# forsaken628/katib

Hardware: AMD Instinct MI355X
Metric: darts_cifar10_search_wall_clock_s (lower is better)
Workload: dtype fp32; 1 GPU; model=darts-cnn-cifar10 supernet (b5: C=4, L=2, N=3, stem x1, 6 primitives + none), global_batch=128, per_gpu_batch=128, parallelism=dp1, epochs=2, steps_per_epoch=196, ops=hip, hip_graph=True, sync_bn=False, hessian=concurrent

## Files before the change

### katib_amd/csrc/hip/darts_bind.cpp

```cpp
#include <torch/extension.h>
#include <c10/hip/HIPStream.h>

#include "darts_ops.h"
#include "darts_plane_layout.h"

using namespace katib_hip;
using at::Tensor;
using OptT = c10::optional<Tensor>;

namespace {

hipStream_t cur_stream() { return c10::hip::getCurrentHIPStream().stream(); }

void check_f32(const Tensor& t, const char* name) {
  TORCH_CHECK(t.is_cuda(), name, " must be a GPU tensor");
  TORCH_CHECK(t.scalar_type() == at::kFloat, name, " must be float32");
  TORCH_CHECK(t.is_contiguous(), name, " must be contiguous");
}

constexpr at::ScalarType kZType = kZbf16 ? at::kBFloat16 : at::kFloat;

void check_z(const Tensor& t, const char* name) {
  TORCH_CHECK(t.is_cuda(), name, " must be a GPU tensor");
  TORCH_CHECK(t.scalar_type() == kZType, name, " must be ", kZbf16 ? "bfloat16" : "float32",
              " (the per-op intermediates' storage type of this build)");
  TORCH_CHECK(t.is_contiguous(), name, " must be contiguous");
}

zt* zptr(const Tensor& t) { return reinterpret_cast<zt*>(t.data_ptr()); }

template <typename T>
T* ptr_or_null(const OptT& t) {
  return t.has_value() && t->defined() ? t->data_ptr<T>() : nullptr;
}

BNRef make_bn(const py::tuple& b, int C) {
  BNRef r{};
  TORCH_CHECK(b.size() == 8, "bn tuple has 8 fields");
  OptT sums = b[0].cast<OptT>(), rm = b[1].cast<OptT>(), rv = b[2].cast<OptT>();
  r.rep = b[6].cast<int>();
  r.rstride = b[7].cast<int>();
  TORCH_CHECK(r.rep >= 1 && r.rep <= kRep && r.rstride >= 2 * C, "bn replica layout");
  if (sums.has_value() && sums->defined()) {
    TORCH_CHECK(sums->scalar_type() == at::kDouble && sums->is_contiguous() &&
                    sums->numel() >= (int64_t)(r.rep - 1) * r.rstride + 2 * C,
                "bn sums must be f64 with rep x rstride doubles");
  }
  r.sums = ptr_or_null<double>(sums);
  r.rmean = ptr_or_null<float>(rm);
  r.rvar = ptr_or_null<float>(rv);
  r.inv_count = b[3].cast<float>();
  r.eval = b[4].cast<bool>() ? 1 : 0;
  r.eps = b[5].cast<float>();
  r.C = C;
  TORCH_CHECK(r.eval ? (r.rmean && r.rvar) : (r.sums != nullptr), "bn reference lacks its statistics");
  return r;
}

int64_t storage_doubles_after(const Tensor& t) {
  return (int64_t)(t.storage().nbytes() / sizeof(double)) - t.storage_offset();
}

int64_t gs_numel(const py::tuple& t) {
  return t[1].cast<Tensor>().numel();
}

GradSrc make_gs(const py::tuple& t, int C) {
  GradSrc g{};
  TORCH_CHECK(t.size() == 9, "grad-source tuple has 9 fields");
  Tensor gt = t[0].cast<Tensor>(), zt = t[1].cast<Tensor>();
  check_f32(gt, "g");
  check_z(zt, "z");
  g.g = gt.data_ptr<float>();
  g.z = zptr(zt);
  OptT s1 = t[2].cast<OptT>(), s2 = t[3].cast<OptT>();
  g.S1 = ptr_or_null<double>(s1);
  g.S2 = ptr_or_null<double>(s2);
  g.bn = make_bn(t[4].cast<py::tuple>(), C);
  g.eval = g.bn.eval;
  TORCH_CHECK(g.eval || (g.S1 && g.S2), "training-mode BN backward needs S1/S2 reductions");
  OptT w = t[5].cast<OptT>();
  g.w = ptr_or_null<float>(w);
  g.widx = t[6].cast<int>();
  g.rep = t[7].cast<int>();
  g.rstride = t[8].cast<int>();
  TORCH_CHECK(g.rep >= 1 && g.rep <= kRep, "replicas");
  if (!g.eval) {
    for (int k = 2; k <= 3; ++k) {
      Tensor sv = *t[k].cast<OptT>();
      TORCH_CHECK(sv.scalar_type() == at::kDouble &&
                      storage_doubles_after(sv) >= (int64_t)(g.rep - 1) * g.rstride + C,
                  "S1/S2 replicas exceed their buffer");
    }
  }
  return g;
}

struct CtrRing {
  unsigned* base = nullptr;
  int size = 0;
  int cursor = 0;
};
CtrRing g_ring[64];
bool g_selffold = false;

void set_selffold(bool on) { g_selffold = on; }

int cur_device() {
  int d = 0;
  TORCH_CHECK(hipGetDevice(&d) == hipSuccess, "hipGetDevice");
  return d;
}

void set_fold_counters(Tensor t) {
  TORCH_CHECK(t.is_cuda() && t.scalar_type() == at::kInt && t.is_contiguous() && t.numel() >= 4 * kFoldCtrSlot,
              "fold counters: contiguous int32 GPU tensor of >= 4 launch slots");
  const int d = t.get_device();
  TORCH_CHECK(d >= 0 && d < 64, "device index");
  g_ring[d] = CtrRing{reinterpret_cast<unsigned*>(t.data_ptr<int>()), (int)(t.numel() / kFoldCtrSlot), 0};
}

bool selffold_ready() { return g_selffold && g_ring[cur_device()].base != nullptr; }

void tail_begin(FoldTail& t) {
  t.nseg = 0;
  t.ctr = nullptr;
  if (!g_selffold) return;
  CtrRing& r = g_ring[cur_device()];
  if (!r.base) return;
  t.ctr = r.base + (size_t)r.cursor * kFoldCtrSlot;
  r.cursor = (r.cursor + 1) % r.size;
}

void tail_add(FoldTail& t, double* p, int n, int rs) {
  if (!t.ctr || !p) return;
  for (int s = 0; s < t.nseg; ++s)
    if (t.p[s] == p) {
      t.n[s] = std::max(t.n[s], n);
      return;
    }
  TORCH_CHECK(t.nseg < kTailSeg, "self-fold: too many reduction segments in one launch");
  t.p[t.nseg] = p;
  t.n[t.nseg] = n;
  t.rs[t.nseg] = rs;
  ++t.nseg;
}

void tail_close(FoldTail& t) {
  if (t.nseg == 0) t.ctr = nullptr;
}

int pick_chunk(int C, int per_channel_floats, int fixed_floats) {
  const int budget = 16384 - fixed_floats;
  int ch = C;
  while (ch > 1 && ch * per_channel_floats > budget) ch = (ch + 1) / 2;
  return std::max(ch, 1);
}

template <typename Bt>
void check_batch(const std::vector<py::tuple>& calls) {
  TORCH_CHECK(!calls.empty() && (int)calls.size() <= Bt::kCap, "batch of 1..", Bt::kCap, " edges");
}

#define SAME_SHAPE(b, fld) TORCH_CHECK(b.e[i].fld == b.e[0].fld, "edges in a batch must share " #fld)

static bool fill_dwpw(const py::tuple& t, DwPwFwdArgs& a, int64_t K, int64_t dil, int64_t S, int64_t pad, int nentries,
                      bool use_mfma) {
  Tensor x = t[0].cast<Tensor>(), dw = t[1].cast<Tensor>(), pw = t[2].cast<Tensor>();
  auto inbn = t[3].cast<c10::optional<py::tuple>>();
  Tensor d = t[4].cast<Tensor>(), z = t[5].cast<Tensor>();
  OptT stats = t[6].cast<OptT>();
  const bool has_inbn = t[3].cast<c10::optional<py::tuple>>().has_value();
  if (has_inbn) check_z(x, "x (previous stage z)");
  else check_f32(x, "x");
  check_f32(dw, "dw"); check_f32(pw, "pw"); check_z(d, "d"); check_z(z, "z");
  TORCH_CHECK(x.dim() == 4, "x must be NCHW");
  TORCH_CHECK((K == 3 || K == 5) && (dil == 1 || dil == 2) && (S == 1 || S == 2), "K in {3,5}, dil, S in {1,2}");
  const int N = x.size(0), C = x.size(1), H = x.size(2), W = x.size(3);
  const int Ho = z.size(2), Wo = z.size(3);
  TORCH_CHECK(dw.numel() == C * K * K && pw.numel() == C * C, "weight shapes");
  TORCH_CHECK(z.size(0) == N && z.size(1) == C && d.sizes() == z.sizes(), "output shapes");
  TORCH_CHECK(C == 4 || C == 8 || C == 16 || (64 % Wo == 0 && Ho % (64 / Wo) == 0),
              "tile constraint: 64 % Wo == 0 and Ho % (64/Wo) == 0");
  TORCH_CHECK(C <= kMaxC, "C too large");
  TORCH_CHECK(Ho == (H + 2 * pad - dil * (K - 1) - 1) / S + 1, "output height mismatch");
  a.x = x.data_ptr(); a.dw = dw.data_ptr<float>(); a.pw = pw.data_ptr<float>();
  a.d = zptr(d); a.z = zptr(z); a.stats = ptr_or_null<double>(stats);
  if (a.stats) TORCH_CHECK(stats->scalar_type() == at::kDouble && stats->numel() >= kRep * 2 * C, "stats f64 [kRep][2C]");
  a.N = N; a.C = C; a.H = H; a.W = W; a.Ho = Ho; a.Wo = Wo; a.pad = pad;
  const int TR = 64 / Wo;
  const int IR = (TR - 1) * S + (K - 1) * dil + 1, IW = (Wo - 1) * S + (K - 1) * dil + 1;
  a.chunk = pick_chunk(C, IR * IW, C * 64 + 4 * C);
  if (C == 4 || C == 8 || C == 16) {
    int nb = std::max(1, std::min(Ho / 4, 2048 / std::max(N * nentries, 1)));
    auto band_bytes = [&](int b) {
      const int BR = (Ho + b - 1) / b;
      return (size_t)C * ((BR - 1) * S + (K - 1) * dil + 1) * plane_pitch(W + 2 * pad, S) * sizeof(float);
    };
    while (band_bytes(nb) > 65536 && nb < Ho) ++nb;
    a.chunk = nb;
  }
  a.use_mfma = (use_mfma && C % 16 == 0) ? 1 : 0;
  const bool prebn = inbn.has_value();
  if (prebn) a.inbn = make_bn(*inbn, C);
  a.variant = (((K == 5) * 4 + (dil == 2) * 2 + (S == 2)) * 4) + (prebn ? 2 : 0);
  return prebn;
}

void dwpw_fwd(std::vector<py::tuple> calls, int64_t K, int64_t dil, int64_t S, int64_t pad, bool use_mfma) {
  check_batch<DwPwFwdBatch>(calls);
  DwPwFwdBatch bt{};
  bt.n = calls.size();
  bool prebn = false;
  for (int i = 0; i < bt.n; ++i) {
    const bool pb = fill_dwpw(calls[i], bt.e[i], K, dil, S, pad, bt.n, use_mfma);
    if (i == 0) prebn = pb;
    TORCH_CHECK(pb == prebn, "edges in a batch must agree on the input BN");
    SAME_SHAPE(bt, N); SAME_SHAPE(bt, C); SAME_SHAPE(bt, H); SAME_SHAPE(bt, W);
  }
  tail_begin(bt.tail);
  for (int i = 0; i < bt.n; ++i) tail_add(bt.tail, bt.e[i].stats, 2 * bt.e[i].C, 2 * bt.e[i].C);
  tail_close(bt.tail);
  launch_dwpw_fwd(bt, K, dil, S, prebn, cur_stream());
}

static void fill_dwpw_multi(const std::vector<py::tuple>& calls, DwPwMultiBatch& bt, int64_t* kk, int64_t* dd,
                            int64_t* ss, int64_t* pp, bool* pre) {
  TORCH_CHECK(!calls.empty() && (int)calls.size() <= DwPwMultiBatch::kCap, "1..", DwPwMultiBatch::kCap, " entries");
  bt.n = calls.size();
  for (int i = 0; i < bt.n; ++i) {
    const py::tuple& t = calls[i];
    TORCH_CHECK(t.size() == 11, "dwpw_fwd_multi entry: (x, dw, pw, inbn, d, z, stats, K, dil, S, pad)");
    kk[i] = t[7].cast<int64_t>(); dd[i] = t[8].cast<int64_t>(); ss[i] = t[9].cast<int64_t>(); pp[i] = t[10].cast<int64_t>();
    pre[i] = fill_dwpw(t, bt.e[i], kk[i], dd[i], ss[i], pp[i], bt.n, true);
    SAME_SHAPE(bt, N); SAME_SHAPE(bt, C); SAME_SHAPE(bt, Ho); SAME_SHAPE(bt, Wo);
  }
  tail_begin(bt.tail);
  for (int i = 0; i < bt.n; ++i) tail_add(bt.tail, bt.e[i].stats, 2 * bt.e[i].C, 2 * bt.e[i].C);
  tail_close(bt.tail);
}

void dwpw_fwd_multi(std::vector<py::tuple> calls) {
  DwPwMultiBatch bt{};
  int64_t kk[DwPwMultiBatch::kCap], dd[DwPwMultiBatch::kCap], ss[DwPwMultiBatch::kCap], pp[DwPwMultiBatch::kCap];
  bool pre[DwPwMultiBatch::kCap];
  fill_dwpw_multi(calls, bt, kk, dd, ss, pp, pre);
  if (launch_dwpw_multi(bt, cur_stream())) return;
  for (int i = 0; i < bt.n; ++i) {
    DwPwFwdBatch one{};
    one.n = 1;
    one.tail = bt.tail;
    fill_dwpw(calls[i], one.e[0], kk[i], dd[i], ss[i], pp[i], 1, true);
    launch_dwpw_fwd(one, kk[i], dd[i], ss[i], pre[i], cur_stream());
  }
}

void pw_fwd(std::vector<py::tuple> calls, int64_t S) {
  check_batch<PwFwdBatch>(calls);
  PwFwdBatch bt{};
  bt.n = calls.size();
  for (int i = 0; i < bt.n; ++i) {
    const py::tuple& t = calls[i];
    Tensor x = t[0].cast<Tensor>(), pw = t[1].cast<Tensor>(), z = t[2].cast<Tensor>();
    OptT stats = t[3].cast<OptT>();
    const int co_off = t[4].cast<int>(), off = t[5].cast<int>();
    check_f32(x, "x"); check_f32(pw, "pw"); check_z(z, "z");
    const bool nm = x.dim() == 5;
    const int xnodes = nm ? x.size(0) : 1;
    const int N = nm ? x.size(1) : x.size(0), Cin = nm ? x.size(0) * x.size(2) : x.size(1);
    const int H = x.size(nm ? 3 : 2), W = x.size(nm ? 4 : 3);
    const int Cout = pw.size(0), Ho = z.size(2), Wo = z.size(3);
    TORCH_CHECK(pw.size(1) == Cin && co_off + Cout <= z.size(1) && z.size(0) == N, "pw shapes");
    TORCH_CHECK((Ho * Wo) % 64 == 0, "Ho*Wo must be a multiple of 64");
    TORCH_CHECK(Cin <= kMaxC && Cout <= kMaxC, "channels");
    PwFwdArgs& a = bt.e[i];
    a.x = x.data_ptr<float>(); a.pw = pw.data_ptr<float>(); a.z = zptr(z);
    a.stats = ptr_or_null<double>(stats);
    if (a.stats)
      TORCH_CHECK(stats->scalar_type() == at::kDouble && stats->numel() >= kRep * 2 * z.size(1), "stats [kRep][2Ctot]");
    a.N = N; a.Cin = Cin; a.Cout = Cout; a.CoutTotal = z.size(1); a.co_off = co_off;
    a.H = H; a.W = W; a.Ho = Ho; a.Wo = Wo; a.S = S; a.off = off; a.relu = 1; a.xnodes = xnodes;
    SAME_SHAPE(bt, N); SAME_SHAPE(bt, Cin); SAME_SHAPE(bt, Cout); SAME_SHAPE(bt, Ho); SAME_SHAPE(bt, Wo);
  }
  tail_begin(bt.tail);
  for (int i = 0; i < bt.n; ++i) tail_add(bt.tail, bt.e[i].stats, 2 * bt.e[i].CoutTotal, 2 * bt.e[i].CoutTotal);
  tail_close(bt.tail);
  launch_pw_fwd(bt, cur_stream());
}

static void fill_pool_fwd(const std::vector<py::tuple>& calls, int64_t S_all, PoolFwdBatch& bt) {
  check_batch<PoolFwdBatch>(calls);
  bt.n = calls.size();
  for (int i = 0; i < bt.n; ++i) {
    const py::tuple& t = calls[i];
    const int64_t S = S_all > 0 ? S_all : t[6].cast<int64_t>();
    TORCH_CHECK(S == 1 || S == 2, "pool stride must be 1 or 2");
    bt.e[i].S = (int)S;
    Tensor x = t[0].cast<Tensor>(), zavg = t[1].cast<Tensor>(), zmax = t[2].cast<Tensor>();
    OptT sa = t[3].cast<OptT>(), sm = t[4].cast<OptT>(), amax = t[5].cast<OptT>();
    check_f32(x, "x"); check_z(zavg, "zavg"); check_z(zmax, "zmax");
    PoolFwdArgs& a = bt.e[i];
    if (amax.has_value() && amax->defined()) {
      TORCH_CHECK(amax->scalar_type() == at::kByte && amax->numel() == zmax.numel(), "amax must be uint8 like zmax");
      a.amax = amax->data_ptr<uint8_t>();
    }
    a.x = x.data_ptr<float>(); a.zavg = zptr(zavg); a.zmax = zptr(zmax);
    a.stats_avg = ptr_or_null<double>(sa); a.stats_max = ptr_or_null<double>(sm);
    if (a.stats_avg) TORCH_CHECK(sa->scalar_type() == at::kDouble && sa->numel() >= kRep * 2 * x.size(1), "stats");
    if (a.stats_max) TORCH_CHECK(sm->scalar_type() == at::kDouble && sm->numel() >= kRep * 2 * x.size(1), "stats");
    a.N = x.size(0); a.C = x.size(1); a.H = x.size(2); a.W = x.size(3); a.Ho = zavg.size(2); a.Wo = zavg.size(3);
    TORCH_CHECK(a.Ho == (a.H - 1) / S + 1 && zmax.sizes() == zavg.sizes(), "pool shapes");
    SAME_SHAPE(bt, N); SAME_SHAPE(bt, C);
    if (S_all > 0) { SAME_SHAPE(bt, H); SAME_SHAPE(bt, W); }
  }
  tail_begin(bt.tail);
  for (int i = 0; i < bt.n; ++i) {
    tail_add(bt.tail, bt.e[i].stats_avg, 2 * bt.e[i].C, 2 * bt.e[i].C);
    tail_add(bt.tail, bt.e[i].stats_max, 2 * bt.e[i].C, 2 * bt.e[i].C);
  }
  tail_close(bt.tail);
}

static void pool_fwd_impl(std::vector<py::tuple> calls, int64_t S_all) {
  PoolFwdBatch bt{};
  fill_pool_fwd(calls, S_all, bt);
  if (S_all > 0) launch_pool_fwd(bt, S_all, cur_stream());
  else launch_pool_fwd_multi(bt, cur_stream());
}

void pool_fwd(std::vector<py::tuple> calls, int64_t S) { pool_fwd_impl(calls, S); }
void pool_fwd_multi(std::vector<py::tuple> calls) { pool_fwd_impl(calls, -1); }

void dwpw_pool_fwd_multi(std::vector<py::tuple> dcalls, std::vector<py::tuple> pcalls) {
  DwPwMultiBatch bt{};
  int64_t kk[DwPwMultiBatch::kCap], dd[DwPwMultiBatch::kCap], ss[DwPwMultiBatch::kCap], pp[DwPwMultiBatch::kCap];
  bool pre[DwPwMultiBatch::kCap];
  fill_dwpw_multi(dcalls, bt, kk, dd, ss, pp, pre);
  PoolFwdBatch pb{};
  fill_pool_fwd(pcalls, -1, pb);
  if (launch_dwpw_pool_multi(bt, pb, cur_stream())) return;
  dwpw_fwd_multi(dcalls);
  launch_pool_fwd_multi(pb, cur_stream());
}

void combine_fwd(std::vector<py::tuple> calls, OptT gamma, OptT beta, Tensor out, double momentum,
                 bool update_running, bool accumulate) {
  check_f32(out, "out");
  check_batch<CombineFwdBatch>(calls);
  CombineFwdBatch bt{};
  bt.n = calls.size();
  const int C = out.size(1);
  TORCH_CHECK(C <= kMaxC, "C too large");
  TORCH_CHECK((int64_t)2 * bt.n * kMaxOps * C * 4 <= 65536, "combine LDS budget exceeded");
  for (int e = 0; e < bt.n; ++e) {
    const py::tuple& t = calls[e];
    auto zs = t[0].cast<std::vector<Tensor>>();
    auto bns = t[1].cast<std::vector<py::tuple>>();
    auto widx = t[2].cast<std::vector<int64_t>>();
    OptT w = t[3].cast<OptT>();
    const int id_idx = t[4].cast<int>();
    OptT xid = t[5].cast<OptT>();
    auto upd = t[6].cast<std::vector<py::tuple>>();
    TORCH_CHECK(zs.size() == bns.size() && zs.size() == widx.size() && (int)zs.size() <= kMaxOps, "ops");
    CombineFwdArgs& a = bt.e[e];
    a.N = out.size(0); a.C = C; a.HW = out.size(2) * out.size(3);
    a.nops = zs.size();
    for (size_t k = 0; k < zs.size(); ++k) {
      check_z(zs[k], "z");
      TORCH_CHECK(zs[k].sizes() == out.sizes(), "combine input shape");
      a.z[k] = zptr(zs[k]);
      a.bn[k] = make_bn(bns[k], C);
      a.widx[k] = widx[k];
    }
    TORCH_CHECK((int)upd.size() <= kMaxUpd, "too many update-only BN layers");
    a.nupd = upd.size();
    for (size_t k = 0; k < upd.size(); ++k) a.upd[k] = make_bn(upd[k], C);
    a.w = ptr_or_null<float>(w); a.id_idx = id_idx; a.xid = ptr_or_null<float>(xid);
    if (a.xid) {
      check_f32(*xid, "xid");
      TORCH_CHECK(xid->sizes() == out.sizes(), "identity shape");
    }
    a.gamma = ptr_or_null<float>(gamma); a.beta = ptr_or_null<float>(beta);
    a.out = out.data_ptr<float>(); a.momentum = momentum; a.update_running = update_running;
    a.accumulate = accumulate;
  }
  launch_combine_fwd(bt, cur_stream());
}

void combine_bwd_reduce(std::vector<py::tuple> calls) {
  check_batch<CombineBwdBatch>(calls);
  CombineBwdBatch bt{};
  bt.n = calls.size();
  for (int i = 0; i < bt.n; ++i) {
    const py::tuple& t = calls[i];
    Tensor dout = t[0].cast<Tensor>();
    auto zs = t[1].cast<std::vector<Tensor>>();
    auto bns = t[2].cast<std::vector<py::tuple>>();
    OptT xid = t[3].cast<OptT>();
    Tensor red = t[4].cast<Tensor>();
    auto widx = t[5].cast<std::vector<int64_t>>();
    const int id_idx = t[6].cast<int>();
    OptT gw = t[7].cast<OptT>();
    check_f32(dout, "dout");
    TORCH_CHECK(red.scalar_type() == at::kDouble, "red must be f64");
    CombineBwdArgs& a = bt.e[i];
    a.N = dout.size(0); a.C = dout.size(1); a.HW = dout.size(2) * dout.size(3);
    a.nops = zs.size();
    a.rstride = (a.nops + 1) * a.C + 1;
    TORCH_CHECK(a.nops <= kMaxOps && red.numel() >= (int64_t)kRep * a.rstride, "red size [kRep][(nops+1)C+1]");
    for (int k = 0; k < a.nops; ++k) {
      TORCH_CHECK(zs[k].sizes() == dout.sizes(), "z shape");
      check_z(zs[k], "z");
      a.z[k] = zptr(zs[k]);
      a.bn[k] = make_bn(bns[k], a.C);
    }
    a.dout = dout.data_ptr<float>(); a.xid = ptr_or_null<float>(xid); a.red = red.data_ptr<double>();
    a.gw = ptr_or_null<double>(gw); a.id_idx = id_idx;
    if (a.gw) {
      TORCH_CHECK(gw->scalar_type() == at::kDouble && gw->numel() % kRep == 0, "gw must be f64 [kRep][nw]");
      a.gwstride = gw->numel() / kRep;
      TORCH_CHECK((int)widx.size() == a.nops, "widx per op");
      for (int k = 0; k < a.nops; ++k) {
        TORCH_CHECK(widx[k] >= 0 && widx[k] < a.gwstride, "widx out of range");
        a.widx[k] = widx[k];
      }
      TORCH_CHECK(id_idx < a.gwstride, "id_idx out of range");
    }
    SAME_SHAPE(bt, N); SAME_SHAPE(bt, C); SAME_SHAPE(bt, HW);
  }
  tail_begin(bt.tail);
  for (int i = 0; i < bt.n; ++i) {
    tail_add(bt.tail, bt.e[i].red, bt.e[i].rstride, bt.e[i].rstride);
    tail_add(bt.tail, bt.e[i].gw, bt.e[i].gwstride, bt.e[i].gwstride);
  }
  tail_close(bt.tail);
  launch_combine_bwd_reduce(bt, cur_stream());
}

void check_grad_sink(const OptT& gW, int64_t numel, int64_t gstride) {
  if (!gW.has_value() || !gW->defined()) return;
  TORCH_CHECK(gW->scalar_type() == at::kFloat && gW->is_contiguous() && gW->numel() == numel, "gW shape");
  TORCH_CHECK(gstride == 0 || (gstride >= numel && (int64_t)(gW->storage().nbytes() / sizeof(float)) -
                                                           gW->storage_offset() >= (kRep - 1) * gstride + numel),
              "gW replicas exceed their buffer");
}

void pw_bwd(std::vector<py::tuple> calls, int64_t S, int64_t mode, bool need_dx) {
  check_batch<PwBwdBatch>(calls);
  PwBwdBatch bt{};
  bt.n = calls.size();
  for (int i = 0; i < bt.n; ++i) {
    const py::tuple& t = calls[i];
    py::tuple gs = t[0].cast<py::tuple>();
    Tensor pw = t[1].cast<Tensor>();
    OptT ain = t[2].cast<OptT>();
    Tensor x = t[3].cast<Tensor>();
    OptT dd = t[4].cast<OptT>(), gx = t[5].cast<OptT>(), gW = t[6].cast<OptT>();
    const int co_off = t[7].cast<int>(), off = t[8].cast<int>();
    const int64_t gstride = t[9].cast<int64_t>();
    const bool overwrite = t.size() > 10 && t[10].cast<bool>();
    check_f32(pw, "pw");
    if (mode != 0) check_f32(x, "x");
    PwBwdArgs& a = bt.e[i];
    a.overwrite = overwrite;
    TORCH_CHECK(!overwrite || (mode == 1 && S == 1 && off == 0), "gx overwrite needs the stride-1 full-coverage form");
    const int Cout = pw.size(0), Cin = pw.size(1);
    Tensor g = gs[0].cast<Tensor>();
    a.N = g.size(0); a.CoutTotal = g.size(1); a.Ho = g.size(2); a.Wo = g.size(3);
    a.gs = make_gs(gs, a.CoutTotal);
    a.Cin = Cin; a.Cout = Cout; a.co_off = co_off; a.S = S; a.off = off; a.mode = mode;
    a.need_dx = need_dx;
    const bool nm = mode != 0 && x.dim() == 5;
    a.xnodes = nm ? x.size(0) : 1;
    a.H = x.size(nm ? 3 : 2); a.W = x.size(nm ? 4 : 3);
    if (mode != 0) {
      TORCH_CHECK(x.numel() == (int64_t)a.N * Cin * a.H * a.W && (!nm || x.size(1) == a.N),
                  "pw_bwd: x must be [N][Cin][H][W] or node-major [nodes][N][Cin/nodes][H][W]");
      if (gx.has_value() && gx->defined()) TORCH_CHECK(gx->sizes() == x.sizes(), "pw_bwd: gx must have the shape of x");
    }
    TORCH_CHECK(Cin * Cout <= 8192, "pw_bwd supports Cin*Cout <= 8192");
    TORCH_CHECK((a.Ho * a.Wo) % 64 == 0, "Ho*Wo % 64");
    a.pw = pw.data_ptr<float>(); a.x = mode != 0 ? x.data_ptr<float>() : nullptr;
    if (ain.has_value() && ain->defined()) check_z(*ain, "ain (depthwise output d)");
    a.ain = ain.has_value() && ain->defined() ? zptr(*ain) : nullptr;
    a.dd = ptr_or_null<float>(dd); a.gx = ptr_or_null<float>(gx);
    a.gW = ptr_or_null<float>(gW);
    if (mode == 0) {
      TORCH_CHECK(a.ain && (!need_dx || a.dd), "mode 0 needs ain (and dd)");
    } else {
      TORCH_CHECK(!need_dx || a.gx, "mode 1 needs gx");
    }
    check_grad_sink(gW, (int64_t)Cin * Cout, gstride);
    a.gstride = gstride;
    SAME_SHAPE(bt, N); SAME_SHAPE(bt, Cin); SAME_SHAPE(bt, Cout); SAME_SHAPE(bt, Ho); SAME_SHAPE(bt, Wo);
  }
  launch_pw_bwd(bt, cur_stream());
}

void dw_bwd_fill(std::vector<py::tuple>& calls, DwBwdBatch& bt, const int64_t* Ks, const int64_t* dils,
                 const int64_t* Ss, bool& prebn);

void dw_bwd(std::vector<py::tuple> calls, int64_t K, int64_t dil, int64_t S, int64_t pad) {
  check_batch<DwBwdBatch>(calls);
  DwBwdBatch bt{};
  int64_t Ks[DwBwdBatch::kCap], Ds[DwBwdBatch::kCap], Ss[DwBwdBatch::kCap];
  for (int i = 0; i < DwBwdBatch::kCap; ++i) Ks[i] = K, Ds[i] = dil, Ss[i] = S;
  TORCH_CHECK(pad == (K - 1) / 2 * dil, "dw_bwd padding must be 'same'");
  bool prebn = false;
  dw_bwd_fill(calls, bt, Ks, Ds, Ss, prebn);
  tail_close(bt.tail);
  launch_dw_bwd(bt, K, dil, S, prebn, cur_stream());
}

void dw_bwd_multi(std::vector<py::tuple> calls) {
  check_batch<DwBwdBatch>(calls);
  DwBwdBatch bt{};
  int64_t Ks[DwBwdBatch::kCap], Ds[DwBwdBatch::kCap], Ss[DwBwdBatch::kCap];
  for (size_t i = 0; i < calls.size(); ++i) {
    TORCH_CHECK(calls[i].size() == 10 || calls[i].size() == 12,
                "dw_bwd_multi entry: (x, inbn, dw, dd, gout, gW, red, gstride, overwrite, K[, dil, S])");
    Ks[i] = calls[i][9].cast<int64_t>();
    Ds[i] = calls[i].size() == 12 ? calls[i][10].cast<int64_t>() : 1;
    Ss[i] = calls[i].size() == 12 ? calls[i][11].cast<int64_t>() : 1;
    TORCH_CHECK((Ks[i] == 3 || Ks[i] == 5) && (Ds[i] == 1 || Ds[i] == 2) && (Ss[i] == 1 || Ss[i] == 2),
                "K in {3, 5}, dil and S in {1, 2}");
  }
  bool prebn = false;
  dw_bwd_fill(calls, bt, Ks, Ds, Ss, prebn);
  for (int i = 0; i < bt.n; ++i) {
    TORCH_CHECK(prebn || bt.e[i].overwrite, "dw_bwd_multi: input-gradient entries must own (overwrite) their output");
    TORCH_CHECK(!prebn || (Ds[i] == 1 && Ss[i] == 1), "dw_bwd_multi: input-BN entries are stride-1 separable stages");
    bt.e[i].variant = dw_bwd_variant((int)Ks[i], (int)Ds[i], (int)Ss[i], prebn);
  }
  for (int i = 0; i < bt.n; ++i)
    for (int j = i + 1; j < bt.n; ++j) TORCH_CHECK(bt.e[i].gout != bt.e[j].gout, "dw_bwd_multi entries share an output");
  tail_close(bt.tail);
  if (launch_dw_bwd_multi(bt, cur_stream())) return;
  for (int v = 0; v < 16; ++v) {
    DwBwdBatch one{};
    one.tail = bt.tail;
    for (int i = 0; i < bt.n; ++i)
      if (bt.e[i].variant == v) one.e[one.n++] = bt.e[i];
    if (one.n) launch_dw_bwd(one, dw_variant_k(v), dw_variant_dil(v), dw_variant_s(v), prebn, cur_stream());
  }
}

void dw_bwd_fill(std::vector<py::tuple>& calls, DwBwdBatch& bt, const int64_t* Ks, const int64_t* dils,
                 const int64_t* Ss, bool& prebn) {
  bt.n = calls.size();
  bool has_gw = false;
  for (int i = 0; i < bt.n; ++i) {
    const py::tuple& t = calls[i];
    const int64_t K = Ks[i], dil = dils[i], S = Ss[i], pad = (K - 1) / 2 * dil;
    Tensor x = t[0].cast<Tensor>();
    auto inbn = t[1].cast<c10::optional<py::tuple>>();
    Tensor dw = t[2].cast<Tensor>(), dd = t[3].cast<Tensor>(), gout = t[4].cast<Tensor>();
    OptT gW = t[5].cast<OptT>(), red = t[6].cast<OptT>();
    const int64_t gstride = t[7].cast<int64_t>();
    const bool overwrite = t[8].cast<bool>();
    if (inbn.has_value()) check_z(x, "x (stage-1 z)");
    else check_f32(x, "x");
    check_f32(dw, "dw"); check_f32(dd, "dd"); check_f32(gout, "gout");
    DwBwdArgs& a = bt.e[i];
    a.N = x.size(0); a.C = x.size(1); a.H = x.size(2); a.W = x.size(3); a.Ho = dd.size(2); a.Wo = dd.size(3);
    TORCH_CHECK(a.H == a.Ho * S && a.W == a.Wo * S, "dw_bwd needs H == Ho*S");
    TORCH_CHECK(gout.sizes() == x.sizes(), "gout shape");
    TORCH_CHECK(dw.numel() == a.C * K * K && dd.size(1) == a.C, "dw_bwd weight / grad shapes");
    a.x = x.data_ptr(); a.dw = dw.data_ptr<float>(); a.dd = dd.data_ptr<float>();
    a.gout = gout.data_ptr<float>(); a.gW = ptr_or_null<float>(gW); a.red = ptr_or_null<double>(red);
    const bool plane = (a.C == 4 || a.C == 8 || (a.C % 16 == 0 && a.C <= kMaxC)) && a.Wo % 4 == 0 &&
                       (((uintptr_t)a.x | (uintptr_t)a.dd | (uintptr_t)a.gout) & 15) == 0;
    TORCH_CHECK(plane || (64 % a.Wo == 0 && a.Ho % (64 / a.Wo) == 0), "tile constraint");
    check_grad_sink(gW, (int64_t)a.C * K * K, gstride);
    a.gstride = gstride;
    a.overwrite = overwrite;
    if (a.red) TORCH_CHECK(red->scalar_type() == at::kDouble && red->numel() >= kRep * 2 * a.C, "red [kRep][2C]");
    a.pad = pad;
    if (i == 0) {
      prebn = inbn.has_value();
      has_gw = a.gW != nullptr;
    }
    TORCH_CHECK(inbn.has_value() == prebn, "edges in a batch must agree on the input BN");
    TORCH_CHECK((a.gW != nullptr) == has_gw, "edges in a batch must agree on weight-gradient sinks");
    TORCH_CHECK(!(prebn && overwrite), "overwrite applies to the input-gradient (non-BN) form");
    const int TR = 64 / a.Wo, r = (K - 1) / 2 * dil, h = (r + S - 1) / S, OR = TR + 2 * h;
    const int IR = (TR - 1) * S + (K - 1) * dil + 1, IW = (a.Wo - 1) * S + (K - 1) * dil + 1;
    a.chunk = pick_chunk(a.C, OR * a.Wo + IR * IW, 4 * a.C + (a.gW ? a.C * (int)(K * K) : 0));
    if (prebn) a.inbn = make_bn(*inbn, a.C);
    SAME_SHAPE(bt, N); SAME_SHAPE(bt, C); SAME_SHAPE(bt, Ho); SAME_SHAPE(bt, Wo);
  }
  tail_begin(bt.tail);
  if (prebn)
    for (int i = 0; i < bt.n; ++i) tail_add(bt.tail, bt.e[i].red, 2 * bt.e[i].C, 2 * bt.e[i].C);
}

static void pool_bwd_impl(std::vector<py::tuple> calls, int64_t S_all) {
  check_batch<PoolBwdBatch>(calls);
  PoolBwdBatch bt{};
  bt.n = calls.size();
  for (int i = 0; i < bt.n; ++i) {
    const py::tuple& t = calls[i];
    const int64_t S = S_all > 0 ? S_all : t[9].cast<int64_t>();
    TORCH_CHECK(S == 1 || S == 2, "pool stride must be 1 or 2");
    bt.e[i].S = (int)S;
    auto ga = t[0].cast<c10::optional<py::tuple>>(), gm = t[1].cast<c10::optional<py::tuple>>();
    Tensor x = t[2].cast<Tensor>();
    OptT dout_id = t[3].cast<OptT>(), w = t[4].cast<OptT>();
    const int id_idx = t[5].cast<int>();
    Tensor gx = t[6].cast<Tensor>();
    OptT amax = t[7].cast<OptT>();
    check_f32(x, "x"); check_f32(gx, "gx");
    PoolBwdArgs& a = bt.e[i];
    a.N = x.size(0); a.C = x.size(1); a.H = x.size(2); a.W = x.size(3);
    a.Ho = (a.H - 1) / S + 1; a.Wo = (a.W - 1) / S + 1;
    TORCH_CHECK(a.Ho * a.Wo <= 8192, "pool_bwd stages one output plane in LDS (Ho*Wo <= 8192)");
    TORCH_CHECK(gx.sizes() == x.sizes(), "gx shape");
    TORCH_CHECK(!gm.has_value() || (amax.has_value() && amax->defined() && amax->scalar_type() == at::kByte &&
                                    amax->numel() == (int64_t)a.N * a.C * a.Ho * a.Wo),
                "max-pool backward needs the uint8 argmax from pool_fwd");
    if (amax.has_value() && amax->defined()) a.amax = amax->data_ptr<uint8_t>();
    if (ga.has_value()) a.ga = make_gs(*ga, a.C);
    if (gm.has_value()) a.gm = make_gs(*gm, a.C);
    a.x = x.data_ptr<float>(); a.dout_id = ptr_or_null<float>(dout_id); a.w = ptr_or_null<float>(w);
    if (a.dout_id) TORCH_CHECK(dout_id->sizes() == x.sizes(), "identity gradient shape");
    a.id_idx = id_idx; a.gx = gx.data_ptr<float>();
    a.overwrite = t[8].cast<bool>();
    if (S_all <= 0 && t.size() > 10) {
      auto ex = t[10].cast<std::vector<Tensor>>();
      TORCH_CHECK(ex.size() <= 4, "pool_bwd: at most 4 extra gradient parts");
      a.nextra = ex.size();
      for (size_t j = 0; j < ex.size(); ++j) {
        check_f32(ex[j], "extra");
        TORCH_CHECK(ex[j].sizes() == gx.sizes(), "extra gradient part shape");
        TORCH_CHECK(ex[j].data_ptr() != gx.data_ptr(), "extra part aliases gx");
        a.extra[j] = ex[j].data_ptr<float>();
      }
    }
    SAME_SHAPE(bt, N); SAME_SHAPE(bt, C);
    if (S_all > 0) { SAME_SHAPE(bt, H); SAME_SHAPE(bt, W); }
  }
  for (int i = 0; i < bt.n; ++i)
    for (int j = i + 1; j < bt.n; ++j) TORCH_CHECK(bt.e[i].gx != bt.e[j].gx, "pool_bwd entries share a gx buffer");
  if (S_all > 0) launch_pool_bwd(bt, S_all, cur_stream());
  else launch_pool_bwd_multi(bt, cur_stream());
}

void pool_bwd(std::vector<py::tuple> calls, int64_t S) { pool_bwd_impl(calls, S); }

bool edge_bwd(std::vector<py::tuple> calls) {
  check_batch<EdgeBwdBatch>(calls);
  EdgeBwdBatch bt{};
  bt.n = calls.size();
  const int Ks[4] = {3, 5, 3, 5};
  for (int i = 0; i < bt.n; ++i) {
    const py::tuple& t = calls[i];
    TORCH_CHECK(t.size() == 11, "edge_bwd entry: (x, gx, overwrite, convs, ga, gm, amax, dout_id, w, id_idx, S)");
    Tensor x = t[0].cast<Tensor>(), gx = t[1].cast<Tensor>();
    check_f32(x, "x"); check_f32(gx, "gx");
    TORCH_CHECK(x.dim() == 4 && gx.sizes() == x.sizes(), "gx shape");
    EdgeBwdArgs& a = bt.e[i];
    a.x = x.data_ptr<float>(); a.gx = gx.data_ptr<float>(); a.overwrite = t[2].cast<bool>();
    a.S = t[10].cast<int>();
    TORCH_CHECK(a.S == 1 || a.S == 2, "stride");
    a.N = x.size(0); a.C = x.size(1); a.H = x.size(2); a.W = x.size(3);
    a.Ho = (a.H - 1) / a.S + 1; a.Wo = (a.W - 1) / a.S + 1;
    auto convs = t[3].cast<std::vector<py::object>>();
    TORCH_CHECK(convs.size() == 4, "4 conv slots");
    for (int v = 0; v < 4; ++v) {
      if (convs[v].is_none()) continue;
      py::tuple c = convs[v].cast<py::tuple>();
      Tensor dw = c[0].cast<Tensor>(), dd = c[1].cast<Tensor>();
      OptT gW = c[2].cast<OptT>();
      const int64_t gstride = c[3].cast<int64_t>();
      check_f32(dw, "dw"); check_f32(dd, "dd");
      TORCH_CHECK(dw.numel() == a.C * Ks[v] * Ks[v], "dw shape");
      TORCH_CHECK(dd.dim() == 4 && dd.size(0) == a.N && dd.size(1) == a.C && dd.size(2) == a.Ho && dd.size(3) == a.Wo,
                  "dd shape");
      check_grad_sink(gW, (int64_t)a.C * Ks[v] * Ks[v], gstride);
      a.dw[v] = dw.data_ptr<float>(); a.dd[v] = dd.data_ptr<float>(); a.gW[v] = ptr_or_null<float>(gW);
      a.gstride[v] = gstride;
      a.conv_mask |= 1 << v;
    }
    auto ga = t[4].cast<c10::optional<py::tuple>>(), gm = t[5].cast<c10::optional<py::tuple>>();
    OptT amax = t[6].cast<OptT>(), dout_id = t[7].cast<OptT>(), w = t[8].cast<OptT>();
    if (ga.has_value()) {
      a.ga = make_gs(*ga, a.C);
      TORCH_CHECK(gs_numel(*ga) == (int64_t)a.N * a.C * a.Ho * a.Wo, "avg-pool gradient source shape");
    }
    if (gm.has_value()) {
      a.gm = make_gs(*gm, a.C);
      TORCH_CHECK(gs_numel(*gm) == (int64_t)a.N * a.C * a.Ho * a.Wo, "max-pool gradient source shape");
      TORCH_CHECK(amax.has_value() && amax->defined() && amax->scalar_type() == at::kByte &&
                      amax->numel() == (int64_t)a.N * a.C * a.Ho * a.Wo,
                  "max-pool backward needs the uint8 argmax from pool_fwd");
      a.amax = amax->data_ptr<uint8_t>();
    }
    a.dout_id = ptr_or_null<float>(dout_id); a.w = ptr_or_null<float>(w); a.id_idx = t[9].cast<int>();
    if (a.dout_id) {
      check_f32(*dout_id, "dout_id");
      TORCH_CHECK(dout_id->sizes() == x.sizes() && a.S == 1, "identity gradient shape");
    }
    SAME_SHAPE(bt, N); SAME_SHAPE(bt, C);
  }
  for (int i = 0; i < bt.n; ++i)
    for (int j = i + 1; j < bt.n; ++j) TORCH_CHECK(bt.e[i].gx != bt.e[j].gx, "edge_bwd entries share a gx buffer");
  return launch_edge_bwd(bt, cur_stream());
}
void pool_bwd_multi(std::vector<py::tuple> calls) { pool_bwd_impl(calls, -1); }

void fold_rows(Tensor buf) {
  check_f32(buf, "buf");
  TORCH_CHECK(buf.dim() == 2, "buf must be [rows][n]");
  FoldArgs a{};
  a.buf = buf.data_ptr<float>();
  a.rows = buf.size(0);
  a.n = buf.size(1);
  launch_fold_rows(a, cur_stream());
}

void fold_f64(std::vector<py::tuple> segs) {
  TORCH_CHECK(!segs.empty() && (int)segs.size() <= kMaxSeg, "1..kMaxSeg segments");
  FoldF64Args a{};
  a.nseg = segs.size();
  for (int k = 0; k < a.nseg; ++k) {
    Tensor t = segs[k][0].cast<Tensor>();
    int n = segs[k][1].cast<int>(), rs = segs[k][2].cast<int>();
    TORCH_CHECK(t.is_cuda() && t.scalar_type() == at::kDouble && t.is_contiguous(), "fold segment must be f64");
    TORCH_CHECK(n >= 1 && rs >= n && t.numel() >= (int64_t)(kRep - 1) * rs + n, "fold segment size");
    a.p[k] = t.data_ptr<double>();
    a.n[k] = n;
    a.rstride[k] = rs;
    a.total += n;
  }
  launch_fold_f64(a, cur_stream());
}

}

void register_xgmi(py::module& m);
void register_conv(py::module& m);
void register_transformer(py::module& m);
void register_batchnorm(py::module& m);
void register_mlp(py::module& m);
void register_stem(py::module& m);
void register_enas(py::module& m);
void register_dwconv(py::module& m);
void register_darts_optim(py::module& m);
void register_darts_head(py::module& m);
void register_resnet(py::module& m);
void register_augment(py::module& m);

PYBIND11_MODULE(TORCH_EXTENSION_NAME, m) {
  m.doc() = "katib_amd HIP kernels for gfx950 (DARTS edge ops, implicit-GEMM conv, transformer, xGMI all-reduce)";
  m.def("dwpw_fwd", &dwpw_fwd);
  m.def("pw_fwd", &pw_fwd);
  m.def("pool_fwd", &pool_fwd);
  m.def("combine_fwd", &combine_fwd);
  m.def("combine_bwd_reduce", &combine_bwd_reduce);
  m.def("pw_bwd", &pw_bwd);
  m.def("dw_bwd", &dw_bwd);
  m.def("dw_bwd_multi", &dw_bwd_multi, "separable second-stage depthwise backward of mixed kernel size in one launch");
  m.def("pool_bwd", &pool_bwd);
  m.def("dwpw_fwd_multi", &dwpw_fwd_multi, "mixed (K, dil, S) dw-pw entries of one node stage in one launch");
  m.def("pool_fwd_multi", &pool_fwd_multi, "stride-1 and stride-2 pools in one launch");
  m.def("dwpw_pool_fwd_multi", &dwpw_pool_fwd_multi, "a node's stage-1 dw-pw entries and its pools in one launch");
  m.def("pool_bwd_multi", &pool_bwd_multi, "stride-1 and stride-2 pool backward in one launch");
  m.def("edge_bwd", &edge_bwd, "whole input gradient of a node's edges (convs, pools, identity) in one launch");
  m.def("set_max_blocks", &set_max_blocks);
  m.def("stamps_arm", [](int kind, int call, torch::Tensor buf) {
    TORCH_CHECK(!buf.defined() || kind == 0 || (buf.is_cuda() && buf.scalar_type() == torch::kInt64 &&
                                               buf.is_contiguous() && buf.numel() >= 65536 * 8),
                "stamps_arm: int64 CUDA buffer of >= 65536 * 8 entries");
    stamps_arm(kind, call, kind == 0 ? nullptr : reinterpret_cast<unsigned long long*>(buf.data_ptr<int64_t>()));
  }, "diagnostic build: phase-stamp the call-th launch of kind (StampKind) into buf[wg * 8 + phase]");
  m.def("stamps_compiled", &stamps_compiled);
  m.def("fold_rows", &fold_rows);
  m.def("fold_f64", &fold_f64);
  m.def("set_fold_counters", &set_fold_counters, "register the current device's self-fold counter ring (int32, zeroed)");
  m.def("selffold_ready", &selffold_ready, "launches on the current device fold their own f64 replicas");
  m.def("set_selffold", &set_selffold, "turn self-folding launches on / off (default off: measured slower)");
  m.attr("REP") = kRep;
  m.attr("ZBF16") = kZbf16;
  m.def("max_blocks", &max_blocks);
  register_xgmi(m);
  register_conv(m);
  register_transformer(m);
  register_batchnorm(m);
  register_enas(m);
  register_dwconv(m);
  register_mlp(m);
  register_stem(m);
  register_darts_optim(m);
  register_darts_head(m);
  register_resnet(m);
  register_augment(m);
}
```

### katib_amd/csrc/hip/darts_ops.h

```cpp
#pragma once
#include <hip/hip_runtime.h>
#include <hip/hip_bf16.h>

namespace katib_hip {

#ifdef KATIB_DARTS_ZBF16
typedef __hip_bfloat16 zt;
constexpr bool kZbf16 = true;
#else
typedef float zt;
constexpr bool kZbf16 = false;
#endif
typedef float zf4 __attribute__((ext_vector_type(4)));

__device__ __forceinline__ float z2f(float v) { return v; }
__device__ __forceinline__ float z2f(__hip_bfloat16 v) { return __bfloat162float(v); }
__device__ __forceinline__ void zput(float* p, float v) { *p = v; }
__device__ __forceinline__ void zput(__hip_bfloat16* p, float v) { *p = __float2bfloat16(v); }
__device__ __forceinline__ zf4 zld4(const float* p) { return *reinterpret_cast<const zf4*>(p); }
__device__ __forceinline__ zf4 zld4(const __hip_bfloat16* p) {
  const uint2 u = *reinterpret_cast<const uint2*>(p);
  return zf4{__uint_as_float(u.x << 16), __uint_as_float(u.x & 0xffff0000u), __uint_as_float(u.y << 16),
             __uint_as_float(u.y & 0xffff0000u)};
}
__device__ __forceinline__ void zst4(float* p, zf4 v) { *reinterpret_cast<zf4*>(p) = v; }
__device__ __forceinline__ void zst4(__hip_bfloat16* p, zf4 v) {
  __hip_bfloat16 b[4] = {__float2bfloat16(v.x), __float2bfloat16(v.y), __float2bfloat16(v.z), __float2bfloat16(v.w)};
  *reinterpret_cast<uint2*>(p) = *reinterpret_cast<const uint2*>(b);
}

__host__ __device__ __forceinline__ size_t plane_off(int n, int c, int N, int C, int nodes, size_t HW) {
  if (nodes <= 1) return ((size_t)n * C + c) * HW;
  const int Cn = C / nodes, k = c / Cn;
  return (((size_t)k * N + n) * Cn + (c - k * Cn)) * HW;
}

constexpr int kMaxOps = 8;
constexpr int kMaxUpd = 4;
constexpr int kMaxC = 256;
#ifndef KATIB_HIP_REP
#define KATIB_HIP_REP 32
#endif
constexpr int kRep = KATIB_HIP_REP;

struct BNRef {
  const double* sums;
  float* rmean;
  float* rvar;
  float inv_count;
  float eps;
  int eval;
  int C;
  int rep;
  int rstride;
};

struct GradSrc {
  const float* g;
  const zt* z;
  const double* S1;
  const double* S2;
  BNRef bn;
  const float* w;
  int widx;
  int eval;
  int rep;
  int rstride;
};

struct DwPwFwdArgs {
  const void* x;
  BNRef inbn; const float* dw; const float* pw;
  zt* d; zt* z; double* stats;
  int N, C, H, W, Ho, Wo, pad, chunk, use_mfma;
  int variant;
  int nblk;
  int vout = 0;
};

struct PwFwdArgs {
  const void* x;
  const float* pw; zt* z; double* stats;
  int N, Cin, Cout, CoutTotal, co_off, H, W, Ho, Wo, S, off;
  int relu;
  int xnodes;
};

struct PoolFwdArgs {
  const float* x; zt* zavg; zt* zmax; double* stats_avg; double* stats_max; unsigned char* amax;
  int N, C, H, W, Ho, Wo;
  int S, nblk;
};

struct CombineFwdArgs {
  const zt* z[kMaxOps]; BNRef bn[kMaxOps]; int widx[kMaxOps]; int nops;
  BNRef upd[kMaxUpd]; int nupd;
  const float* w; int id_idx; const float* xid; const float* gamma; const float* beta;
  float* out; int N, C, HW; float momentum; int update_running; int accumulate;
};

struct CombineBwdArgs {
  const float* dout; const zt* z[kMaxOps]; BNRef bn[kMaxOps]; int nops;
  const float* xid; double* red; int N, C, HW;
  double* gw; int widx[kMaxOps]; int id_idx;
  int rstride, gwstride;
};

struct PwBwdArgs {
  GradSrc gs; const float* pw; const zt* ain; const float* x; float* dd; float* gx; float* gW;
  int gstride;
  int N, Cin, Cout, CoutTotal, co_off, H, W, Ho, Wo, S, off, mode, need_dx;
  int overwrite;
  int xnodes;
};

struct DwBwdArgs {
  const void* x;
  BNRef inbn; const float* dw; const float* dd; float* gout; float* gW; double* red;
  int gstride;
  int N, C, H, W, Ho, Wo, pad, chunk;
  int overwrite;
  int variant, nbands, nblk;
  int vin = 0;
  int blk0 = 0;
};
constexpr int dw_bwd_variant(int K, int dil, int S, bool prebn) {
  return (((K == 5) * 4 + (dil == 2) * 2 + (S == 2)) << 1) | (prebn ? 1 : 0);
}
constexpr int dw_variant_k(int v) { return (v >> 3) & 1 ? 5 : 3; }
constexpr int dw_variant_dil(int v) { return (v >> 2) & 1 ? 2 : 1; }
constexpr int dw_variant_s(int v) { return (v >> 1) & 1 ? 2 : 1; }
constexpr bool dw_variant_prebn(int v) { return v & 1; }

struct FoldArgs {
  float* buf; int n; int rows;
};

constexpr int kMaxSeg = 128;
struct FoldF64Args {
  double* p[kMaxSeg]; int n[kMaxSeg]; int rstride[kMaxSeg]; int nseg; int total;
};

struct PoolBwdArgs {
  GradSrc ga; GradSrc gm; const float* x; const float* dout_id; const float* w; int id_idx; float* gx;
  const unsigned char* amax;
  const float* extra[4]; int nextra;
  int overwrite;
  int N, C, H, W, Ho, Wo;
  int S;
};

constexpr int kTailSeg = 16;
constexpr int kFoldShards = 32;
constexpr int kFoldCtrStride = 32;
constexpr int kFoldCtrSlot = (1 + kFoldShards) * kFoldCtrStride;
struct FoldTail {
  unsigned* ctr;
  int nseg;
  double* p[kTailSeg];
  int n[kTailSeg];
  int rs[kTailSeg];
};

template <typename A, int M>
struct Batch {
  A e[M];
  int n;
  FoldTail tail;
  static constexpr int kCap = M;
};
using DwPwFwdBatch = Batch<DwPwFwdArgs, 16>;
using CombineFwdBatch = Batch<CombineFwdArgs, 4>;
using PwFwdBatch = Batch<PwFwdArgs, 32>;
using PoolFwdBatch = Batch<PoolFwdArgs, 16>;
using CombineBwdBatch = Batch<CombineBwdArgs, 8>;
using PwBwdBatch = Batch<PwBwdArgs, 32>;
using DwBwdBatch = Batch<DwBwdArgs, 40>;
using PoolBwdBatch = Batch<PoolBwdArgs, 16>;
using DwPwMultiBatch = Batch<DwPwFwdArgs, 40>;

struct EdgeBwdArgs {
  const float* x; float* gx; int overwrite;
  const float* dw[4]; const float* dd[4]; float* gW[4]; int gstride[4]; int conv_mask;
  GradSrc ga; GradSrc gm; const unsigned char* amax;
  const float* dout_id; const float* w; int id_idx;
  int N, C, H, W, Ho, Wo, S, nb, nblk;
};
using EdgeBwdBatch = Batch<EdgeBwdArgs, 4>;
constexpr size_t kKernargMax = 24576;
static_assert(sizeof(EdgeBwdBatch) <= kKernargMax, "edge_bwd batch exceeds the kernarg budget");
static_assert(sizeof(DwPwFwdBatch) <= kKernargMax && sizeof(CombineFwdBatch) <= kKernargMax &&
                  sizeof(PwFwdBatch) <= kKernargMax && sizeof(PoolFwdBatch) <= kKernargMax &&
                  sizeof(CombineBwdBatch) <= kKernargMax && sizeof(PwBwdBatch) <= kKernargMax &&
                  sizeof(DwBwdBatch) <= kKernargMax && sizeof(PoolBwdBatch) <= kKernargMax &&
                  sizeof(DwPwMultiBatch) <= kKernargMax,
              "kernel argument batches exceed the kernarg budget");

void launch_dwpw_fwd(const DwPwFwdBatch& b, int K, int dil, int S, bool prebn, hipStream_t st);
void launch_dw_bwd(const DwBwdBatch& b, int K, int dil, int S, bool prebn, hipStream_t st);
bool launch_dw_bwd_multi(DwBwdBatch b, hipStream_t st);
void launch_pw_fwd(const PwFwdBatch& b, hipStream_t st);
void launch_pool_fwd(const PoolFwdBatch& b, int S, hipStream_t st);
void launch_pool_bwd(const PoolBwdBatch& b, int S, hipStream_t st);
bool launch_dwpw_multi(DwPwMultiBatch b, hipStream_t st);
void launch_pool_fwd_multi(PoolFwdBatch b, hipStream_t st);
struct PoolFwdEntries {
  PoolFwdArgs e[PoolFwdBatch::kCap];
  int n;
};
static_assert(sizeof(DwPwMultiBatch) + sizeof(PoolFwdEntries) <= kKernargMax, "kernarg budget");
bool launch_dwpw_pool_multi(DwPwMultiBatch b, const PoolFwdBatch& pb, hipStream_t st);
void launch_pool_bwd_multi(const PoolBwdBatch& b, hipStream_t st);
void launch_combine_fwd(const CombineFwdBatch& b, hipStream_t st);
bool launch_edge_bwd(EdgeBwdBatch b, hipStream_t st);
void launch_combine_bwd_reduce(const CombineBwdBatch& b, hipStream_t st);
void launch_pw_bwd(const PwBwdBatch& b, hipStream_t st);
int max_blocks();
void launch_fold_rows(const FoldArgs& a, hipStream_t st);
void launch_fold_f64(const FoldF64Args& a, hipStream_t st);
void set_max_blocks(int n);
void stamps_arm(int kind, int call, unsigned long long* buf);
bool stamps_compiled();

}
```

### katib_amd/csrc/hip/darts_ops_fwd.hip

```cpp
#include "darts_ops_fwd_k.h"

namespace katib_hip {


template <int K, int DIL, int S, int C>
static void launch_dwpw_plane_t(const DwPwFwdBatch& b, bool prebn, hipStream_t st) {
  const DwPwFwdArgs& a = b.e[0];
  const int nb = a.chunk, BR = (a.Ho + nb - 1) / nb;
  const size_t lds = sizeof(float) * (plane_head_floats(C) + C * ((BR - 1) * S + (K - 1) * DIL + 1) * plane_pitch(a.W + 2 * a.pad, S));
  dim3 grid(a.N * nb, b.n);
  bool vec = a.W % 4 == 0;
  for (int i = 0; i < b.n; ++i) vec &= ((uintptr_t)b.e[i].x & 15) == 0;
  if (vec) {
    if (prebn) hipLaunchKernelGGL((dwpw_plane_kernel<K, DIL, S, true, C, true>), grid, dim3(256), lds, st, b);
    else hipLaunchKernelGGL((dwpw_plane_kernel<K, DIL, S, false, C, true>), grid, dim3(256), lds, st, b);
  } else {
    if (prebn) hipLaunchKernelGGL((dwpw_plane_kernel<K, DIL, S, true, C, false>), grid, dim3(256), lds, st, b);
    else hipLaunchKernelGGL((dwpw_plane_kernel<K, DIL, S, false, C, false>), grid, dim3(256), lds, st, b);
  }
}

static bool plane_ok(const DwPwFwdArgs& a) { return a.C == 4 || a.C == 8 || a.C == 16; }

template <int CI, int CO>
static bool try_pw_fwd_wave(const PwFwdBatch& b, hipStream_t st);

template <int K, int DIL, int S, int CG>
static bool try_dwpw_split_g(const DwPwFwdBatch& b, bool prebn, hipStream_t st, bool split16);

template <int K, int DIL, int S>
static bool try_dwpw_split(const DwPwFwdBatch& b, bool prebn, hipStream_t st) {
  const DwPwFwdArgs& a = b.e[0];
  constexpr bool split16 = true;
  constexpr int grp = 8;
  if (grp == 4) return try_dwpw_split_g<K, DIL, S, 4>(b, prebn, st, split16);
  if (grp == 8) return try_dwpw_split_g<K, DIL, S, 8>(b, prebn, st, split16);
  return try_dwpw_split_g<K, DIL, S, 16>(b, prebn, st, split16);
}

template <int K, int DIL, int S, int CG>
static bool try_dwpw_split_g(const DwPwFwdBatch& b, bool prebn, hipStream_t st, bool split16) {
  const DwPwFwdArgs& a = b.e[0];
  if (a.C % 16 != 0 || a.C > 64 || (a.C == 16 && !split16) ||
      (a.Ho * a.Wo) % 64 != 0 || a.W % 4 != 0)
    return false;
  for (int i = 0; i < b.n; ++i)
    if (((uintptr_t)b.e[i].x | (uintptr_t)b.e[i].d | (uintptr_t)b.e[i].z) & 15) return false;
  const int G = a.C / CG;
  int nb = std::max(1, std::min(a.Ho / 4, 2048 / std::max(a.N * b.n * G, 1)));
  auto band_bytes = [&](int v) {
    const int BR = (a.Ho + v - 1) / v;
    return ((size_t)plane_head_floats(CG) + (size_t)CG * ((BR - 1) * S + (K - 1) * DIL + 1) * plane_pitch(a.W + 2 * a.pad, S)) * sizeof(float);
  };
  while (band_bytes(nb) > 65536 && nb < a.Ho) ++nb;
  DwPwFwdBatch db = b;
  db.tail.ctr = nullptr;
  for (int i = 0; i < b.n; ++i) db.e[i].chunk = nb;
  dim3 grid(a.N * nb * G, b.n);
  const size_t lds = band_bytes(nb);
  if (prebn) hipLaunchKernelGGL((dwpw_plane_kernel<K, DIL, S, true, CG, true, false>), grid, dim3(256), lds, st, db);
  else hipLaunchKernelGGL((dwpw_plane_kernel<K, DIL, S, false, CG, true, false>), grid, dim3(256), lds, st, db);
  PwFwdBatch pb{};
  pb.n = b.n;
  pb.tail = b.tail;
  for (int i = 0; i < b.n; ++i) {
    const DwPwFwdArgs& e = b.e[i];
    PwFwdArgs& p = pb.e[i];
    p.x = e.d; p.pw = e.pw; p.z = e.z; p.stats = e.stats;
    p.N = e.N; p.Cin = e.C; p.Cout = e.C; p.CoutTotal = e.C; p.co_off = 0;
    p.H = e.Ho; p.W = e.Wo; p.Ho = e.Ho; p.Wo = e.Wo; p.S = 1; p.off = 0; p.relu = 0;
  }
  if (try_pw_fwd_wave<16, 16>(pb, st) || try_pw_fwd_wave<32, 32>(pb, st) || try_pw_fwd_wave<64, 64>(pb, st))
    return true;
  launch_pw_fwd(pb, st);
  return true;
}

template <int K, int DIL, int S>
static void launch_dwpw_fwd_t(const DwPwFwdBatch& b, bool prebn, hipStream_t st) {
  const DwPwFwdArgs& a = b.e[0];
  if (try_dwpw_split<K, DIL, S>(b, prebn, st)) return;
  if (plane_ok(a)) {
    if (a.C == 4) return launch_dwpw_plane_t<K, DIL, S, 4>(b, prebn, st);
    if (a.C == 8) return launch_dwpw_plane_t<K, DIL, S, 8>(b, prebn, st);
    return launch_dwpw_plane_t<K, DIL, S, 16>(b, prebn, st);
  }
  const int TR = 64 / a.Wo;
  const int IR = (TR - 1) * S + (K - 1) * DIL + 1;
  const int IW = (a.Wo - 1) * S + (K - 1) * DIL + 1;
  size_t lds = sizeof(float) * (a.C * 64 + a.chunk * IR * IW + 4 * a.C);
  dim3 grid(per_edge_blocks(a.N * (a.Ho / TR), b.n), b.n);
  if (prebn) hipLaunchKernelGGL((dwpw_fwd_kernel<K, DIL, S, true>), grid, dim3(256), lds, st, b);
  else hipLaunchKernelGGL((dwpw_fwd_kernel<K, DIL, S, false>), grid, dim3(256), lds, st, b);
}

void launch_dwpw_fwd(const DwPwFwdBatch& b, int K, int dil, int S, bool prebn, hipStream_t st) {
#define DISPATCH(KK, DD, SS) \
  if (K == KK && dil == DD && S == SS) return launch_dwpw_fwd_t<KK, DD, SS>(b, prebn, st);
  DISPATCH(3, 1, 1) DISPATCH(3, 1, 2) DISPATCH(5, 1, 1) DISPATCH(5, 1, 2)
  DISPATCH(3, 2, 1) DISPATCH(3, 2, 2) DISPATCH(5, 2, 1) DISPATCH(5, 2, 2)
#undef DISPATCH
}


static bool dwpw_multi_prep(DwPwMultiBatch& b, bool& fused, int& maxblk, size_t& lds) {
  const int C = b.e[0].C, N = b.e[0].N;
  constexpr bool split16 = true;
  fused = C == 4 || C == 8 || (C == 16 && !split16);
  const bool split = !fused && C % 16 == 0 && C <= 64;
  if (!fused && !split) return false;
  const int CG = fused ? C : 8, G = C / CG;
  maxblk = 0;
  lds = 0;
  for (int i = 0; i < b.n; ++i) {
    DwPwFwdArgs& a = b.e[i];
    if (a.C != C || a.N != N) return false;
    const int code = a.variant >> 2;
    const int K = (code & 4) ? 5 : 3, DIL = (code & 2) ? 2 : 1, S = (code & 1) ? 2 : 1;
    const bool aligned = ((((uintptr_t)a.x) | (uintptr_t)a.d | (uintptr_t)a.z) & 15) == 0;
    if (split && (!aligned || (a.Ho * a.Wo) % 64 != 0 || a.W % 4 != 0)) return false;
    int nb = std::max(1, std::min(a.Ho / 4, 512 / std::max(N * b.n * G, 1)));
    auto band_bytes = [&](int v) {
      const int BR = (a.Ho + v - 1) / v;
      return ((size_t)plane_head_floats(CG) + (size_t)CG * ((BR - 1) * S + (K - 1) * DIL + 1) * plane_pitch(a.W + 2 * a.pad, S)) * sizeof(float);
    };
    while (band_bytes(nb) > 65536 && nb < a.Ho) ++nb;
    a.chunk = nb;
    a.nblk = N * nb * G;
    const bool vec = a.W % 4 == 0 && (((uintptr_t)a.x) & 15) == 0;
    a.variant = (a.variant & ~1) | (vec ? 1 : 0);
    a.vout = (vec_mask() >> (CG == 4 ? 0 : 1)) & 1;
    maxblk = std::max(maxblk, a.nblk);
    lds = std::max(lds, band_bytes(nb));
  }
  return true;
}

bool launch_dwpw_multi(DwPwMultiBatch b, hipStream_t st) {
  if (b.n < 1) return true;
  const int C = b.e[0].C;
  bool fused;
  int maxblk;
  size_t lds;
  if (!dwpw_multi_prep(b, fused, maxblk, lds)) return false;
  const dim3 grid(maxblk, b.n);
  if (fused) {
    if (C == 4) launch_dwpw_plane_multi_t<4>(true, grid, lds, st, b);
    else if (C == 8) launch_dwpw_plane_multi_t<8>(true, grid, lds, st, b);
    else launch_dwpw_plane_multi_t<16>(true, grid, lds, st, b);
    return true;
  }
  {
    DwPwMultiBatch db = b;
    db.tail.ctr = nullptr;
    launch_dwpw_plane_multi_t<8>(false, grid, lds, st, db);
  }
  PwFwdBatch pb{};
  pb.n = b.n;
  pb.tail = b.tail;
  for (int i = 0; i < b.n; ++i) {
    const DwPwFwdArgs& e = b.e[i];
    PwFwdArgs& p = pb.e[i];
    p.x = e.d; p.pw = e.pw; p.z = e.z; p.stats = e.stats;
    p.N = e.N; p.Cin = e.C; p.Cout = e.C; p.CoutTotal = e.C; p.co_off = 0;
    p.H = e.Ho; p.W = e.Wo; p.Ho = e.Ho; p.Wo = e.Wo; p.S = 1; p.off = 0; p.relu = 0;
  }
  bool same_hw = true;
  for (int i = 1; i < b.n; ++i) same_hw &= b.e[i].Ho == b.e[0].Ho && b.e[i].Wo == b.e[0].Wo;
  if (same_hw && (try_pw_fwd_wave<16, 16>(pb, st) || try_pw_fwd_wave<32, 32>(pb, st) || try_pw_fwd_wave<64, 64>(pb, st)))
    return true;
  for (int i = 0; i < b.n; ++i) {
    PwFwdBatch one{};
    one.n = 1;
    one.tail = pb.tail;
    one.e[0] = pb.e[i];
    if (!(try_pw_fwd_wave<16, 16>(one, st) || try_pw_fwd_wave<32, 32>(one, st) || try_pw_fwd_wave<64, 64>(one, st)))
      launch_pw_fwd(one, st);
  }
  return true;
}

static bool pool_fwd_prep(PoolFwdArgs* e, int n, int& maxblk, size_t& lds) {
  bool v4 = true;
  auto al = [](const void* p, uintptr_t m) { return p == nullptr || (reinterpret_cast<uintptr_t>(p) & (m - 1)) == 0; };
  maxblk = 0;
  lds = 0;
  for (int i = 0; i < n; ++i) {
    PoolFwdArgs& a = e[i];
    a.nblk = a.C * channel_groups(a.N, a.C, n);
    maxblk = std::max(maxblk, a.nblk);
    v4 = v4 && a.W % 4 == 0 && a.Wo % 4 == 0 && (a.S == 1 || a.W == 2 * a.Wo) && al(a.x, 16) &&
         al(a.zavg, 4 * sizeof(zt)) && al(a.zmax, 4 * sizeof(zt)) && al(a.amax, 4);
  }
  return v4;
}

void launch_pool_fwd_multi(PoolFwdBatch b, hipStream_t st) {
  int maxblk;
  size_t lds;
  if (pool_fwd_prep(b.e, b.n, maxblk, lds))
    hipLaunchKernelGGL(pool_fwd_multi_kernel<true>, dim3(maxblk, b.n), dim3(256), lds, st, b);
  else hipLaunchKernelGGL(pool_fwd_multi_kernel<false>, dim3(maxblk, b.n), dim3(256), 0, st, b);
}

bool launch_dwpw_pool_multi(DwPwMultiBatch b, const PoolFwdBatch& pb, hipStream_t st) {
  constexpr bool off = false;
  if (off || b.n < 1 || pb.n < 1 || b.tail.ctr || pb.tail.ctr || b.n + pb.n > 65535) return false;
  const int C = b.e[0].C;
  bool fused;
  int maxblk;
  size_t lds;
  if (!dwpw_multi_prep(b, fused, maxblk, lds) || !fused || (C != 4 && C != 8)) return false;
  PoolFwdEntries pe{};
  pe.n = pb.n;
  for (int i = 0; i < pb.n; ++i) pe.e[i] = pb.e[i];
  int pblk;
  size_t plds;
  if (!pool_fwd_prep(pe.e, pe.n, pblk, plds)) return false;
  const dim3 grid(std::max(maxblk, pblk), b.n + pb.n);
  lds = std::max(lds, plds);
  if (C == 4) launch_dwpw_pool_t<4>(grid, lds, st, b, pe);
  else launch_dwpw_pool_t<8>(grid, lds, st, b, pe);
  return true;
}

template <int CI, int CO>
static bool try_pw_fwd_wave(const PwFwdBatch& b, hipStream_t st) {
  const PwFwdArgs& a = b.e[0];
  constexpr int BO = CO / 16;
  if (a.Cin != CI || a.Cout != CO || (a.Ho * a.Wo) % 64 != 0) return false;
  for (int e = 0; e < b.n; ++e) {
    const PwFwdArgs& x = b.e[e];
    const bool flat = !x.relu || (x.S == 1 && x.off == 0 && x.H == x.Ho && x.W == x.Wo);
    if ((((uintptr_t)x.z) | (flat ? (uintptr_t)x.x : 0)) & 15) return false;
  }
  const int chunks = a.N * a.Ho * a.Wo / 64;
  int ns = 1;
  while (BO % (2 * ns) == 0 && chunks * ns * b.n < 4096) ns *= 2;
  const int per_edge = std::max(1, std::min((chunks * ns + 3) / 4, max_blocks() / std::max(b.n, 1)));
  const dim3 grid(per_edge, b.n);
  if (ns == 1) hipLaunchKernelGGL((pw_fwd_wave_kernel<CI, CO, 1>), grid, dim3(256), 0, st, b);
  else if constexpr (BO % 2 == 0) {
    if (ns == 2) hipLaunchKernelGGL((pw_fwd_wave_kernel<CI, CO, 2>), grid, dim3(256), 0, st, b);
    else if constexpr (BO % 4 == 0) hipLaunchKernelGGL((pw_fwd_wave_kernel<CI, CO, 4>), grid, dim3(256), 0, st, b);
  }
  return true;
}

void launch_pw_fwd(const PwFwdBatch& b, hipStream_t st) {
  const PwFwdArgs& a = b.e[0];
  if (try_pw_fwd_wave<48, 16>(b, st) || try_pw_fwd_wave<48, 32>(b, st) || try_pw_fwd_wave<64, 32>(b, st) ||
      try_pw_fwd_wave<32, 16>(b, st) || try_pw_fwd_wave<16, 16>(b, st) || try_pw_fwd_wave<32, 32>(b, st) ||
      try_pw_fwd_wave<64, 64>(b, st) || try_pw_fwd_wave<128, 64>(b, st))
    return;
  size_t lds = sizeof(float) * (a.Cin * 64 + 2 * a.Cout);
  dim3 grid(per_edge_blocks(a.N * a.Ho * a.Wo / 64, b.n), b.n);
  hipLaunchKernelGGL(pw_fwd_kernel, grid, dim3(256), lds, st, b);
}

void launch_pool_fwd(const PoolFwdBatch& b, int S, hipStream_t st) {
  const PoolFwdArgs& a = b.e[0];
  dim3 grid(a.C * channel_groups(a.N, a.C, b.n), b.n);
  if (S == 1) hipLaunchKernelGGL(pool_fwd_kernel<1>, grid, dim3(256), 0, st, b);
  else hipLaunchKernelGGL(pool_fwd_kernel<2>, grid, dim3(256), 0, st, b);
}

}
```

### katib_amd/csrc/hip/darts_ops_fwd_k.h

```cpp
#pragma once
#include "darts_ops_dev.h"

namespace katib_hip {

template <int K, int DIL, int S, bool PREBN>
__global__ void __launch_bounds__(256) dwpw_fwd_kernel(DwPwFwdBatch bt) {
  const DwPwFwdArgs& a = bt.e[blockIdx.y];
  constexpr int P = 64;
  const int C = a.C, H = a.H, W = a.W, Ho = a.Ho, Wo = a.Wo;
  const int TR = P / Wo;
  const int tiles = Ho / TR;
  const int ntiles = a.N * tiles;
  const int pad = a.pad;
  const int IR = (TR - 1) * S + (K - 1) * DIL + 1;
  const int IW = (Wo - 1) * S + (K - 1) * DIL + 1;
  extern __shared__ __attribute__((aligned(16))) float smem[];
  float* sD = smem;
  float* sIn = smem + C * P;
  float* sMean = sIn + a.chunk * IR * IW;
  float* sInv = sMean + C;
  float* sStat = sInv + C;
  const int tid = threadIdx.x;
  const int wave = tid >> 6, lane = tid & 63;
  for (int c = tid; c < C; c += 256) {
    if (PREBN) bn_coeffs(a.inbn, c, sMean[c], sInv[c]);
    sStat[c] = 0.f;
    sStat[C + c] = 0.f;
  }
  __syncthreads();
  for (int t = blockIdx.x; t < ntiles; t += gridDim.x) {
    const int n = t / tiles, oy0 = (t % tiles) * TR;
    const int iy0 = oy0 * S - pad, ix0 = -pad;
    const size_t xin = (size_t)n * C * H * W;
    for (int c0 = 0; c0 < C; c0 += a.chunk) {
      const int cn = min(a.chunk, C - c0);
      const int tot = cn * IR * IW;
      #pragma unroll 4
      for (int i = tid; i < tot; i += 256) {
        int cc = i / (IR * IW), r = (i / IW) % IR, q = i % IW;
        int iy = iy0 + r, ix = ix0 + q, c = c0 + cc;
        float v = 0.f;
        if (iy >= 0 && iy < H && ix >= 0 && ix < W) {
          v = xval<PREBN>(a.x, xin + ((size_t)c * H + iy) * W + ix);
          if (PREBN) v = (v - sMean[c]) * sInv[c];
          v = fmaxf(v, 0.f);
        }
        sIn[i] = v;
      }
      __syncthreads();
      for (int i = tid; i < cn * P; i += 256) {
        const int cc = __builtin_amdgcn_readfirstlane(i / P);
        const int p = i % P;
        const int c = c0 + cc;
        int ty = p / Wo, tx = p % Wo;
        const float* wk = a.dw + c * K * K;
        const float* src = sIn + (cc * IR + ty * S) * IW + tx * S;
        float acc = 0.f;
#pragma unroll
        for (int ky = 0; ky < K; ++ky)
#pragma unroll
          for (int kx = 0; kx < K; ++kx) acc += wk[ky * K + kx] * src[ky * DIL * IW + kx * DIL];
        sD[c * P + p] = acc;
        zput(a.d + (((size_t)n * C + c) * Ho + oy0 + ty) * Wo + tx, acc);
      }
      __syncthreads();
    }
    if (a.use_mfma) {
      typedef float f4 __attribute__((ext_vector_type(4)));
      for (int cob = wave * 16; cob < C; cob += 64) {
        f4 acc[4] = {{0, 0, 0, 0}, {0, 0, 0, 0}, {0, 0, 0, 0}, {0, 0, 0, 0}};
        for (int k0 = 0; k0 < C; k0 += 4) {
          float av = a.pw[(cob + (lane & 15)) * C + k0 + (lane >> 4)];
#pragma unroll
          for (int pb = 0; pb < 4; ++pb) {
            float bv = sD[(k0 + (lane >> 4)) * P + pb * 16 + (lane & 15)];
            acc[pb] = __builtin_amdgcn_mfma_f32_16x16x4f32(av, bv, acc[pb], 0, 0, 0);
          }
        }
#pragma unroll
        for (int r = 0; r < 4; ++r) {
          int co = cob + (lane >> 4) * 4 + r;
          float s = 0.f, s2 = 0.f;
#pragma unroll
          for (int pb = 0; pb < 4; ++pb) {
            int p = pb * 16 + (lane & 15);
            float v = acc[pb][r];
            zput(a.z + (((size_t)n * C + co) * Ho + oy0 + p / Wo) * Wo + p % Wo, v);
            s += v;
            s2 += v * v;
          }
#pragma unroll
          for (int o = 8; o > 0; o >>= 1) {
            s += __shfl_xor(s, o, 64);
            s2 += __shfl_xor(s2, o, 64);
          }
          if ((lane & 15) == 0) {
            sStat[co] += s;
            sStat[C + co] += s2;
          }
        }
      }
    } else {
      for (int co = wave; co < C; co += 4) {
        const int cou = __builtin_amdgcn_readfirstlane(co);
        const float* wrow = a.pw + cou * C;
        float v = 0.f;
        for (int ci = 0; ci < C; ++ci) v += wrow[ci] * sD[ci * P + lane];
        zput(a.z + (((size_t)n * C + cou) * Ho + oy0 + lane / Wo) * Wo + lane % Wo, v);
        float s = wave_sum(v), s2 = wave_sum(v * v);
        if (lane == 0) {
          sStat[cou] += s;
          sStat[C + cou] += s2;
        }
      }
    }
    __syncthreads();
  }
  if (a.stats)
    for (int i = tid; i < 2 * C; i += 256) atomicAdd(a.stats + rep_slot() * 2 * C + i, (double)sStat[i]);
  if (bt.tail.ctr) fold_tail(bt.tail);
}

template <int K, int DIL, int S, bool PREBN, int C, bool VEC, bool PW>
__device__ __forceinline__ void dwpw_plane_body(const DwPwFwdArgs& a, const int bx) {
  constexpr int KK = K * K;
  const int H = a.H, W = a.W, Ho = a.Ho, Wo = a.Wo, pad = a.pad;
  const int nb = a.chunk, BR = (Ho + nb - 1) / nb;
  const int G = PW ? 1 : a.C / C, c0 = PW ? 0 : (bx % G) * C, nbx = PW ? bx : bx / G;
  const int n = nbx / nb, band = nbx - n * nb;
  const int oy0 = band * BR, oy1 = min(Ho, oy0 + BR);
  const int HP = (BR - 1) * S + (K - 1) * DIL + 1, WP = plane_pitch(W + 2 * pad, S), PL = HP * WP;
  const int iyb = oy0 * S - pad;
  extern __shared__ __attribute__((aligned(16))) float smem[];
  float* sWt = smem;
  float* sPw = smem + C * 25;
  float* sIn = smem + plane_head_floats(C);
  __shared__ float sMean[C], sInv[C], sStat[2 * C];
  const int tid = threadIdx.x, lane = tid & 63, wave = tid >> 6;
  KSTAMP(0);
  for (int i = tid; i < C * KK; i += 256) sWt[i] = a.dw[c0 * KK + i];
  if (PW)
    for (int i = tid; i < C * C; i += 256) sPw[i] = a.pw[i];
  if (PREBN) bn_coeffs_coop(a.inbn, c0, C, sMean, sInv);
  if (tid < C) {
    sStat[tid] = 0.f;
    sStat[C + tid] = 0.f;
  }
  if (PREBN) __syncthreads();
  KSTAMP(1);
  const size_t xin = ((size_t)n * a.C + c0) * H * W;
  if (VEC) {
    const int va = max(iyb, 0), vb = min(iyb + HP, H), q4 = (vb - va) * W / 4;
#pragma unroll 4
    for (int i = tid; i < C * q4; i += 256) {
      const int c = i / q4, o = (i - c * q4) * 4, r = o / W, ix = o - r * W;
      float4 v = xval4<PREBN>(a.x, xin + ((size_t)c * H + va) * W + o);
      if (PREBN) {
        const float m = sMean[c], iv = sInv[c];
        v.x = (v.x - m) * iv;
        v.y = (v.y - m) * iv;
        v.z = (v.z - m) * iv;
        v.w = (v.w - m) * iv;
      }
      float* d = sIn + (c * HP + va - iyb + r) * WP + pad + ix;
      d[0] = fmaxf(v.x, 0.f);
      d[1] = fmaxf(v.y, 0.f);
      d[2] = fmaxf(v.z, 0.f);
      d[3] = fmaxf(v.w, 0.f);
    }
    for (int i = tid; i < C * HP; i += 256) {
      const int iy = iyb + i % HP;
      float* d = sIn + i * WP;
      if (iy < 0 || iy >= H) {
        for (int q = 0; q < WP; ++q) d[q] = 0.f;
      } else {
        for (int q = 0; q < pad; ++q) d[q] = d[pad + W + q] = 0.f;
      }
    }
  } else {
#pragma unroll 4
    for (int row = wave; row < C * HP; row += 4) {
      const int c = row / HP, r = row - c * HP, iy = iyb + r;
      const bool rok = iy >= 0 && iy < H;
      const size_t src = xin + ((size_t)c * H + (rok ? iy : 0)) * W;
      for (int q = lane; q < WP; q += 64) {
        const int ix = q - pad;
        float v = 0.f;
        if (rok && ix >= 0 && ix < W) {
          v = xval<PREBN>(a.x, src + ix);
          if (PREBN) v = (v - sMean[c]) * sInv[c];
          v = fmaxf(v, 0.f);
        }
        sIn[row * WP + q] = v;
      }
    }
  }
  __syncthreads();
  KSTAMP(2);
  float st1[C], st2[C];
#pragma unroll
  for (int c = 0; c < C; ++c) st1[c] = st2[c] = 0.f;
  const int HWo = Ho * Wo;
  zt* dn = a.d + ((size_t)n * a.C + c0) * HWo;
  zt* zn = a.z + (size_t)n * C * HWo;
  const bool vout = VEC && Wo % 4 == 0 && a.vout;
  if (vout) {
    constexpr int SPAN = 3 * S + (K - 1) * DIL + 1, NQ = (SPAN + 3) / 4;
    const bool tiled = S == 1 && (Wo & 7) == 0;
    const int nrowo = oy1 - oy0, npair = Wo >> 3, nrb = (nrowo + kCellRows - 1) / kCellRows;
    const int nit = tiled ? nrb * npair : nrowo * Wo / 4;
    for (int j = tiled ? 4 * wave + tile_cell(lane) : tid; j < nit; j += tiled ? kBlockCells : 256) {
      int p = oy0 * Wo + 4 * j;
      if (tiled) {
        const TileItem it = tile_item(j, lane, nrb, npair);
        if (it.row >= nrowo) continue;
        p = (oy0 + it.row) * Wo + 4 * it.quad;
      }
      const int oy = p / Wo, ox0 = p - oy * Wo;
      zf4 d[C];
#pragma unroll
      for (int c = 0; c < C; ++c) {
        const float* src = sIn + c * PL + ((oy - oy0) * S) * WP + ox0 * S;
        KEEP_WEIGHT_READS_LOCAL();
        const float* wk = sWt + c * KK;
        zf4 acc = {0.f, 0.f, 0.f, 0.f};
#pragma unroll
        for (int ky = 0; ky < K; ++ky) {
          float v[4 * NQ];
#pragma unroll
          for (int q = 0; q < NQ; ++q) {
            const float4 t = *reinterpret_cast<const float4*>(src + ky * DIL * WP + 4 * q);
            v[4 * q] = t.x;
            v[4 * q + 1] = t.y;
            v[4 * q + 2] = t.z;
            v[4 * q + 3] = t.w;
          }
#pragma unroll
          for (int kx = 0; kx < K; ++kx) {
            const float w = wk[ky * K + kx];
            acc.x += w * v[kx * DIL];
            acc.y += w * v[kx * DIL + S];
            acc.z += w * v[kx * DIL + 2 * S];
            acc.w += w * v[kx * DIL + 3 * S];
          }
        }
        d[c] = acc;
        zst4(dn + (size_t)c * HWo + p, acc);
      }
      if (!PW) continue;
#pragma unroll
      for (int co = 0; co < C; ++co) {
        KEEP_WEIGHT_READS_LOCAL();
        zf4 z = {0.f, 0.f, 0.f, 0.f};
#pragma unroll
        for (int ci = 0; ci < C; ++ci) z += sPw[co * C + ci] * d[ci];
        zst4(zn + (size_t)co * HWo + p, z);
        st1[co] += (z.x + z.y) + (z.z + z.w);
        st2[co] += (z.x * z.x + z.y * z.y) + (z.z * z.z + z.w * z.w);
      }
    }
  }
  for (int p = oy0 * Wo + tid; p < (vout ? 0 : oy1 * Wo); p += 256) {
    const int oy = p / Wo, ox = p - oy * Wo;
    float d[C];
#pragma unroll
    for (int c = 0; c < C; ++c) {
      const float* src = sIn + c * PL + ((oy - oy0) * S) * WP + ox * S;
      KEEP_WEIGHT_READS_LOCAL();
        const float* wk = sWt + c * KK;
      float acc = 0.f;
#pragma unroll
      for (int ky = 0; ky < K; ++ky)
#pragma unroll
        for (int kx = 0; kx < K; ++kx) acc += wk[ky * K + kx] * src[ky * DIL * WP + kx * DIL];
      d[c] = acc;
      zput(dn + (size_t)c * HWo + p, acc);
    }
    if (!PW) continue;
#pragma unroll
    for (int co = 0; co < C; ++co) {
      KEEP_WEIGHT_READS_LOCAL();
      float z = 0.f;
#pragma unroll
      for (int ci = 0; ci < C; ++ci) z += sPw[co * C + ci] * d[ci];
      zput(zn + (size_t)co * HWo + p, z);
      st1[co] += z;
      st2[co] += z * z;
    }
  }
  KSTAMP(3);
  if (!PW || !a.stats) return;
  {
    float st[2 * C];
#pragma unroll
    for (int c = 0; c < C; ++c) st[c] = st1[c], st[C + c] = st2[c];
    const float v = wave_reduce_scatter<2 * C>(st);
    if ((lane & (32 / C - 1)) == 0) atomicAdd(sStat + wave_scatter_index<2 * C>(lane), v);
  }
  __syncthreads();
  if (tid < 2 * C) atomicAdd(a.stats + (bx % kRep) * 2 * C + tid, (double)sStat[tid]);
  KSTAMP(4);
}
template <int K, int DIL, int S, bool PREBN, int C, bool VEC, bool PW = true>
__global__ void __launch_bounds__(256) dwpw_plane_kernel(DwPwFwdBatch bt) {
  dwpw_plane_body<K, DIL, S, PREBN, C, VEC, PW>(bt.e[blockIdx.y], blockIdx.x);
  if (bt.tail.ctr) fold_tail(bt.tail);
}

#define DWPW_CASE(KK, DD, SS)                                                                      \
  case ((KK == 5) * 4 + (DD == 2) * 2 + (SS == 2)) * 4 + 0: dwpw_plane_body<KK, DD, SS, false, C, false, PW>(a, bx); break; \
  case ((KK == 5) * 4 + (DD == 2) * 2 + (SS == 2)) * 4 + 1: dwpw_plane_body<KK, DD, SS, false, C, true, PW>(a, bx); break;  \
  case ((KK == 5) * 4 + (DD == 2) * 2 + (SS == 2)) * 4 + 2: dwpw_plane_body<KK, DD, SS, true, C, false, PW>(a, bx); break;  \
  case ((KK == 5) * 4 + (DD == 2) * 2 + (SS == 2)) * 4 + 3: dwpw_plane_body<KK, DD, SS, true, C, true, PW>(a, bx); break;
template <int C, bool PW>
__global__ void __launch_bounds__(256) dwpw_plane_multi_kernel(DwPwMultiBatch bt) {
  const DwPwFwdArgs a = bt.e[blockIdx.y];
  const int bx = blockIdx.x;
  if (bx < a.nblk) {
    switch (a.variant) {
      DWPW_CASE(3, 1, 1) DWPW_CASE(3, 1, 2) DWPW_CASE(5, 1, 1) DWPW_CASE(5, 1, 2)
      DWPW_CASE(3, 2, 1) DWPW_CASE(3, 2, 2) DWPW_CASE(5, 2, 1) DWPW_CASE(5, 2, 2)
      default: break;
    }
  }
  if (bt.tail.ctr) fold_tail(bt.tail);
}



template <int CI, int CO, int NS = 1>
__global__ void __launch_bounds__(256) pw_fwd_wave_kernel(PwFwdBatch bt) {
  static_assert(CI % 16 == 0 && CO % 16 == 0 && CI <= 128 && CO <= 64 && (CO / 16) % NS == 0, "16-channel blocks");
  constexpr int BO = CO / 16 / NS, KS = CI / 4;
  typedef float f4 __attribute__((ext_vector_type(4)));
  const PwFwdArgs& a = bt.e[blockIdx.y];
  const int HWo = a.Ho * a.Wo, Wo = a.Wo;
  const int nchunks = a.N * HWo / 64;
  __shared__ float sStat[2 * CO];
  const int tid = threadIdx.x, wave = tid >> 6, lane = tid & 63, c16 = lane & 15, q = lane >> 4;
  for (int i = tid; i < 2 * CO; i += 256) sStat[i] = 0.f;
  __syncthreads();
  const int grp = (blockIdx.x * 4 + wave) % NS, cb0 = grp * BO * 16;
  float wA[BO][KS];
#pragma unroll
  for (int bo = 0; bo < BO; ++bo)
#pragma unroll
    for (int k = 0; k < KS; ++k) wA[bo][k] = a.pw[(cb0 + bo * 16 + c16) * CI + 4 * k + q];
  const bool flat = !a.relu || (a.S == 1 && a.off == 0 && a.H == a.Ho && a.W == a.Wo);
  const bool fr2 = a.S == 2 && a.H == 2 * a.Ho && a.W == 2 * a.Wo && a.W % 4 == 0 && a.off <= 1 &&
                   ((uintptr_t)a.x & 15) == 0;
  f4 s1[BO], s2[BO];
#pragma unroll
  for (int bo = 0; bo < BO; ++bo) s1[bo] = s2[bo] = f4{0.f, 0.f, 0.f, 0.f};
  for (int w = blockIdx.x * 4 + wave; w < nchunks * NS; w += gridDim.x * 4) {
    const int pix0 = (w / NS) * 64, n = pix0 / HWo, prem = pix0 - n * HWo;
    const int pp = prem + 4 * c16;
    f4 acc[BO][4];
#pragma unroll
    for (int bo = 0; bo < BO; ++bo)
#pragma unroll
      for (int t = 0; t < 4; ++t) acc[bo][t] = f4{0.f, 0.f, 0.f, 0.f};
#pragma unroll
    for (int k = 0; k < KS; ++k) {
      const int ci = 4 * k + q;
      f4 v;
      if (flat) {
        if (a.relu) {
          const size_t o = plane_off(n, ci, a.N, CI, a.xnodes, HWo) + pp;
          v = *reinterpret_cast<const f4*>(static_cast<const float*>(a.x) + o);
          v = f4{fmaxf(v.x, 0.f), fmaxf(v.y, 0.f), fmaxf(v.z, 0.f), fmaxf(v.w, 0.f)};
        } else {
          v = zld4(static_cast<const zt*>(a.x) + ((size_t)n * CI + ci) * HWo + pp);
        }
      } else if (fr2) {
        const float* plane = static_cast<const float*>(a.x) + plane_off(n, ci, a.N, CI, a.xnodes, (size_t)a.H * a.W);
        float v0, v1, v2, v3;
        fr2_pair(plane, a.W, Wo, a.off, pp, v0, v1);
        fr2_pair(plane, a.W, Wo, a.off, pp + 2, v2, v3);
        v = f4{v0, v1, v2, v3};
      } else {
#pragma unroll
        for (int t = 0; t < 4; ++t) {
          const int p = pp + t, oy = p / Wo, ox = p - oy * Wo, iy = oy * a.S + a.off, ix = ox * a.S + a.off;
          v[t] = (iy < a.H && ix < a.W)
                     ? fmaxf(static_cast<const float*>(a.x)[plane_off(n, ci, a.N, CI, a.xnodes, (size_t)a.H * a.W) +
                                                             (size_t)iy * a.W + ix], 0.f)
                     : 0.f;
        }
      }
#pragma unroll
      for (int bo = 0; bo < BO; ++bo)
#pragma unroll
        for (int t = 0; t < 4; ++t) acc[bo][t] = __builtin_amdgcn_mfma_f32_16x16x4f32(wA[bo][k], v[t], acc[bo][t], 0, 0, 0);
    }
#pragma unroll
    for (int bo = 0; bo < BO; ++bo)
#pragma unroll
      for (int r = 0; r < 4; ++r) {
        const f4 z = f4{acc[bo][0][r], acc[bo][1][r], acc[bo][2][r], acc[bo][3][r]};
        zst4(a.z + ((size_t)n * a.CoutTotal + a.co_off + cb0 + bo * 16 + 4 * q + r) * HWo + pp, z);
        s1[bo][r] += (z.x + z.y) + (z.z + z.w);
        s2[bo][r] += (z.x * z.x + z.y * z.y) + (z.z * z.z + z.w * z.w);
      }
  }
  if (a.stats) {
#pragma unroll
  for (int bo = 0; bo < BO; ++bo)
#pragma unroll
    for (int r = 0; r < 4; ++r) {
      float u = s1[bo][r], w = s2[bo][r];
#pragma unroll
      for (int o = 8; o > 0; o >>= 1) {
        u += __shfl_xor(u, o, 64);
        w += __shfl_xor(w, o, 64);
      }
      if (c16 == 0) {
        atomicAdd(sStat + cb0 + bo * 16 + 4 * q + r, u);
        atomicAdd(sStat + CO + cb0 + bo * 16 + 4 * q + r, w);
      }
    }
  __syncthreads();
  for (int i = tid; i < 2 * CO; i += 256) {
    const int hi = i >= CO;
    atomicAdd(a.stats + rep_slot() * 2 * a.CoutTotal + hi * a.CoutTotal + a.co_off + (i - hi * CO), (double)sStat[i]);
  }
  }
  if (bt.tail.ctr) fold_tail(bt.tail);
}

static __global__ void __launch_bounds__(256) pw_fwd_kernel(PwFwdBatch bt) {
  const PwFwdArgs& a = bt.e[blockIdx.y];
  constexpr int P = 64;
  const int Cin = a.Cin, Cout = a.Cout, H = a.H, W = a.W, Ho = a.Ho, Wo = a.Wo;
  const int HWo = Ho * Wo;
  const int ntiles = a.N * HWo / P;
  extern __shared__ __attribute__((aligned(16))) float smem[];
  float* sX = smem;
  float* sStat = sX + Cin * P;
  const int tid = threadIdx.x, wave = tid >> 6, lane = tid & 63;
  for (int i = tid; i < 2 * Cout; i += 256) sStat[i] = 0.f;
  for (int t = blockIdx.x; t < ntiles; t += gridDim.x) {
    const int pix0 = t * P;
    const int n = pix0 / HWo, prem = pix0 % HWo;
    #pragma unroll 4
    for (int i = tid; i < Cin * P; i += 256) {
      int ci = i / P, p = i % P;
      int pp = prem + p, oy = pp / Wo, ox = pp % Wo;
      int iy = oy * a.S + a.off, ix = ox * a.S + a.off;
      float v = 0.f;
      if (iy < H && ix < W) {
        const size_t xi = a.relu ? plane_off(n, ci, a.N, Cin, a.xnodes, (size_t)H * W) + (size_t)iy * W + ix
                                 : (((size_t)n * Cin + ci) * H + iy) * W + ix;
        v = a.relu ? fmaxf(static_cast<const float*>(a.x)[xi], 0.f) : z2f(static_cast<const zt*>(a.x)[xi]);
      }
      sX[i] = v;
    }
    __syncthreads();
    for (int co = wave; co < Cout; co += 4) {
      const int cou = __builtin_amdgcn_readfirstlane(co);
      const float* wrow = a.pw + cou * Cin;
      float v = 0.f;
      for (int ci = 0; ci < Cin; ++ci) v += wrow[ci] * sX[ci * P + lane];
      zput(a.z + ((size_t)n * a.CoutTotal + a.co_off + cou) * HWo + prem + lane, v);
      float s = wave_sum(v), s2 = wave_sum(v * v);
      if (lane == 0) {
        sStat[cou] += s;
        sStat[Cout + cou] += s2;
      }
    }
    __syncthreads();
  }
  if (a.stats)
    for (int i = tid; i < 2 * Cout; i += 256) {
      int hi = i >= Cout;
      atomicAdd(a.stats + rep_slot() * 2 * a.CoutTotal + hi * a.CoutTotal + a.co_off + (i - hi * Cout),
                (double)sStat[i]);
    }
  if (bt.tail.ctr) fold_tail(bt.tail);
}

template <int S, bool V4 = false>
__device__ __forceinline__ void pool_fwd_body(const PoolFwdArgs& a, const int bx, const int gx) {
  const int C = a.C, H = a.H, W = a.W, Ho = a.Ho, Wo = a.Wo;
  const int c = bx % C, g0 = bx / C, G = gx / C;
  float sa = 0, sa2 = 0, sm = 0, sm2 = 0;
  if constexpr (V4) {
    constexpr int WC = S == 1 ? 6 : 9;
    const int HWo = Ho * Wo;
    for (int n = g0; n < a.N; n += G) {
      const int nc = n * C + c;
      const float* xp = a.x + (size_t)nc * H * W;
      for (int o4 = threadIdx.x * 4; o4 < HWo; o4 += 1024) {
        const int oy = o4 / Wo, ox0 = o4 - oy * Wo, ib = ox0 * S;
        float win[3][WC];
        bool rv[3];
#pragma unroll
        for (int r = 0; r < 3; ++r) {
          const int iy = oy * S - 1 + r;
          rv[r] = iy >= 0 && iy < H;
          const float* row = xp + (size_t)(rv[r] ? iy : 0) * W;
          const float4 m0 = *reinterpret_cast<const float4*>(row + ib);
          win[r][1] = m0.x;
          win[r][2] = m0.y;
          win[r][3] = m0.z;
          win[r][4] = m0.w;
          if (S == 1) {
            win[r][5] = ib + 4 < W ? row[ib + 4] : 0.f;
          } else {
            const float4 m1 = *reinterpret_cast<const float4*>(row + ib + 4);
            win[r][5] = m1.x;
            win[r][6] = m1.y;
            win[r][7] = m1.z;
            win[r][8] = m1.w;
          }
          win[r][0] = ib > 0 ? row[ib - 1] : 0.f;
        }
        const bool lv = ib > 0, hv = S == 2 || ib + 4 < W;
        zf4 av, mv;
        unsigned args = 0;
#pragma unroll
        for (int t = 0; t < 4; ++t) {
          float sum = 0.f, mx = -INFINITY;
          int cnt = 0, arg = 0;
#pragma unroll
          for (int ky = 0; ky < 3; ++ky) {
            if (!rv[ky]) continue;
#pragma unroll
            for (int kx = 0; kx < 3; ++kx) {
              const int wc = t * S + kx;
              if ((wc == 0 && !lv) || (wc == WC - 1 && !hv)) continue;
              const float v = win[ky][wc];
              sum += v;
              cnt++;
              if (v > mx || v != v) {
                mx = v;
                arg = ky * 3 + kx;
              }
            }
          }
          av[t] = sum / (float)cnt;
          mv[t] = mx;
          args |= (unsigned)arg << (8 * t);
        }
        const size_t oo = (size_t)nc * HWo + o4;
        zst4(a.zavg + oo, av);
        zst4(a.zmax + oo, mv);
        if (a.amax) *reinterpret_cast<unsigned*>(a.amax + oo) = args;
        sa += (av.x + av.y) + (av.z + av.w);
        sa2 += (av.x * av.x + av.y * av.y) + (av.z * av.z + av.w * av.w);
        sm += (mv.x + mv.y) + (mv.z + mv.w);
        sm2 += (mv.x * mv.x + mv.y * mv.y) + (mv.z * mv.z + mv.w * mv.w);
      }
    }
  }
  for (int n = V4 ? a.N : g0; n < a.N; n += G) {
    const int nc = n * C + c;
    const float* xp = a.x + (size_t)nc * H * W;
    for (int o = threadIdx.x; o < Ho * Wo; o += 256) {
      int oy = o / Wo, ox = o % Wo;
      float sum = 0.f, mx = -INFINITY;
      int cnt = 0, arg = 0;
      for (int ky = 0; ky < 3; ++ky) {
        int iy = oy * S - 1 + ky;
        if (iy < 0 || iy >= H) continue;
        for (int kx = 0; kx < 3; ++kx) {
          int ix = ox * S - 1 + kx;
          if (ix < 0 || ix >= W) continue;
          float v = xp[iy * W + ix];
          sum += v;
          cnt++;
          if (v > mx || v != v) {
            mx = v;
            arg = ky * 3 + kx;
          }
        }
      }
      float av = sum / (float)cnt;
      zput(a.zavg + (size_t)nc * Ho * Wo + o, av);
      zput(a.zmax + (size_t)nc * Ho * Wo + o, mx);
      if (a.amax) a.amax[(size_t)nc * Ho * Wo + o] = (unsigned char)arg;
      sa += av;
      sa2 += av * av;
      sm += mx;
      sm2 += mx * mx;
    }
  }
  if (!a.stats_avg && !a.stats_max) return;
  __shared__ float red[4][4];
  int wave = threadIdx.x >> 6, lane = threadIdx.x & 63;
  {
    float v[4] = {sa, sa2, sm, sm2};
    const float t = wave_reduce_scatter<4>(v);
    if ((lane & 15) == 0) red[wave][wave_scatter_index<4>(lane)] = t;
  }
  __syncthreads();
  if (threadIdx.x < 4) {
    float t = red[0][threadIdx.x] + red[1][threadIdx.x] + red[2][threadIdx.x] + red[3][threadIdx.x];
    double* dst = threadIdx.x < 2 ? a.stats_avg : a.stats_max;
    if (dst) atomicAdd(dst + (bx % kRep) * 2 * C + (threadIdx.x & 1) * C + c, (double)t);
  }
}
template <int S>
__global__ void __launch_bounds__(256) pool_fwd_kernel(PoolFwdBatch bt) {
  pool_fwd_body<S>(bt.e[blockIdx.y], blockIdx.x, gridDim.x);
  if (bt.tail.ctr) fold_tail(bt.tail);
}

template <bool V4>
__global__ void __launch_bounds__(256) pool_fwd_multi_kernel(PoolFwdBatch bt) {
  const PoolFwdArgs a = bt.e[blockIdx.y];
  if ((int)blockIdx.x < a.nblk) {
    if (a.S == 1) pool_fwd_body<1, V4>(a, blockIdx.x, a.nblk);
    else pool_fwd_body<2, V4>(a, blockIdx.x, a.nblk);
  }
  if (bt.tail.ctr) fold_tail(bt.tail);
}


template <int C, bool PV4>
__global__ void __launch_bounds__(256) dwpw_pool_multi_kernel(DwPwMultiBatch bt, PoolFwdEntries pe) {
  constexpr bool PW = true;
  const int bx = blockIdx.x;
  if ((int)blockIdx.y < bt.n) {
    const DwPwFwdArgs a = bt.e[blockIdx.y];
    if (bx < a.nblk) {
      switch (a.variant) {
        DWPW_CASE(3, 1, 1) DWPW_CASE(3, 1, 2) DWPW_CASE(5, 1, 1) DWPW_CASE(5, 1, 2)
        DWPW_CASE(3, 2, 1) DWPW_CASE(3, 2, 2) DWPW_CASE(5, 2, 1) DWPW_CASE(5, 2, 2)
        default: break;
      }
    }
  } else {
    const PoolFwdArgs a = pe.e[blockIdx.y - bt.n];
    if (bx < a.nblk) {
      if (a.S == 1) pool_fwd_body<1, PV4>(a, bx, a.nblk);
      else pool_fwd_body<2, PV4>(a, bx, a.nblk);
    }
  }
}
#undef DWPW_CASE


template <int C>
void launch_dwpw_plane_multi_t(bool pw, dim3 grid, size_t lds, hipStream_t st, const DwPwMultiBatch& b);
template <int C>
void launch_dwpw_pool_t(dim3 grid, size_t lds, hipStream_t st, const DwPwMultiBatch& b, const PoolFwdEntries& pe);
template <>
void launch_dwpw_plane_multi_t<4>(bool pw, dim3 grid, size_t lds, hipStream_t st, const DwPwMultiBatch& b);
template <>
void launch_dwpw_plane_multi_t<8>(bool pw, dim3 grid, size_t lds, hipStream_t st, const DwPwMultiBatch& b);
template <>
void launch_dwpw_plane_multi_t<16>(bool pw, dim3 grid, size_t lds, hipStream_t st, const DwPwMultiBatch& b);
template <>
void launch_dwpw_pool_t<4>(dim3 grid, size_t lds, hipStream_t st, const DwPwMultiBatch& b, const PoolFwdEntries& pe);
template <>
void launch_dwpw_pool_t<8>(dim3 grid, size_t lds, hipStream_t st, const DwPwMultiBatch& b, const PoolFwdEntries& pe);

}
```

### katib_amd/csrc/hip/darts_ops_pwb.hip

```cpp
#include "darts_ops_dev.h"

namespace katib_hip {


template <bool MFMA, int MBLK = 4>
__global__ void __launch_bounds__(256) pw_bwd_kernel(PwBwdBatch bt) {
  const PwBwdArgs& a = bt.e[blockIdx.y];
  constexpr int P = 64, PS = P + 1;
  const int Cin = a.Cin, Cout = a.Cout, Ho = a.Ho, Wo = a.Wo, HWo = Ho * Wo;
  const int ntiles = a.N * HWo / P;
  extern __shared__ __attribute__((aligned(16))) float smem[];
  float* sDz = smem;
  float* sA = sDz + Cout * PS;
  float* sMean = sA + Cin * PS;
  float* sInv = sMean + Cout;
  float* sM1 = sInv + Cout;
  float* sM2 = sM1 + Cout;
  float* sW = sM2 + Cout;
  const int tid = threadIdx.x, wave = tid >> 6, lane = tid & 63;
  const float wv = (tid == 0 && a.gs.w) ? a.gs.w[a.gs.widx] : 1.f;
  bn_gs_coop(a.gs, a.co_off, Cout, sMean, sInv, sM1, sM2);
  if (tid == 0) sW[0] = wv;
  __syncthreads();
  const float wk = sW[0];
  typedef float f4 __attribute__((ext_vector_type(4)));
  constexpr int MAXJ = 32;
  float gacc[MFMA ? 1 : MAXJ];
  f4 macc[MFMA ? MBLK : 1];
#pragma unroll
  for (int j = 0; j < (MFMA ? 1 : MAXJ); ++j) gacc[j] = 0.f;
#pragma unroll
  for (int j = 0; j < (MFMA ? MBLK : 1); ++j) macc[j] = f4{0, 0, 0, 0};
  const int npairs = Cout * Cin;
  const int nbi = Cin / 16, nblk = (Cout / 16) * nbi;
  for (int t = blockIdx.x; t < ntiles; t += gridDim.x) {
    const int pix0 = t * P, n = pix0 / HWo, prem = pix0 % HWo;
    #pragma unroll 4
    for (int i = tid; i < Cout * P; i += 256) {
      int co = i / P, p = i % P;
      size_t gi = ((size_t)n * a.CoutTotal + a.co_off + co) * HWo + prem + p;
      sDz[co * PS + p] = bn_bwd_val(a.gs, gi, sMean[co], sInv[co], wk, sM1[co], sM2[co]);
    }
    #pragma unroll 4
    for (int i = tid; i < Cin * P; i += 256) {
      int ci = i / P, p = i % P;
      int pp = prem + p;
      float v;
      if (a.mode == 0) {
        v = z2f(a.ain[((size_t)n * Cin + ci) * HWo + pp]);
      } else {
        int oy = pp / Wo, ox = pp % Wo, iy = oy * a.S + a.off, ix = ox * a.S + a.off;
        v = (iy < a.H && ix < a.W)
                ? fmaxf(a.x[plane_off(n, ci, a.N, Cin, a.xnodes, (size_t)a.H * a.W) + (size_t)iy * a.W + ix], 0.f)
                : 0.f;
      }
      sA[ci * PS + p] = v;
    }
    __syncthreads();
    if (a.gW) {
      if (MFMA) {
#pragma unroll
        for (int j = 0; j < MBLK; ++j) {
          int b = wave + 4 * j;
          if (b < nblk) {
            int cob = (b / nbi) * 16, cib = (b % nbi) * 16;
            for (int p0 = 0; p0 < P; p0 += 4) {
              float av = sDz[(cob + (lane & 15)) * PS + p0 + (lane >> 4)];
              float bv = sA[(cib + (lane & 15)) * PS + p0 + (lane >> 4)];
              macc[j] = __builtin_amdgcn_mfma_f32_16x16x4f32(av, bv, macc[j], 0, 0, 0);
            }
          }
        }
      } else {
#pragma unroll
        for (int j = 0; j < MAXJ; ++j) {
          int pr = tid + 256 * j;
          if (pr < npairs) {
            int co = pr / Cin, ci = pr % Cin;
            float s = 0.f;
            for (int p = 0; p < P; ++p) s += sDz[co * PS + p] * sA[ci * PS + p];
            gacc[j] += s;
          }
        }
      }
    }
    if (a.need_dx) {
      if (MFMA) {
        for (int cib = wave * 16; cib < Cin; cib += 64) {
          f4 acc[4] = {{0, 0, 0, 0}, {0, 0, 0, 0}, {0, 0, 0, 0}, {0, 0, 0, 0}};
          for (int k0 = 0; k0 < Cout; k0 += 4) {
            float av = a.pw[(k0 + (lane >> 4)) * Cin + cib + (lane & 15)];
#pragma unroll
            for (int pb = 0; pb < 4; ++pb) {
              float bv = sDz[(k0 + (lane >> 4)) * PS + pb * 16 + (lane & 15)];
              acc[pb] = __builtin_amdgcn_mfma_f32_16x16x4f32(av, bv, acc[pb], 0, 0, 0);
            }
          }
#pragma unroll
          for (int r = 0; r < 4; ++r) {
            int ci = cib + (lane >> 4) * 4 + r;
#pragma unroll
            for (int pb = 0; pb < 4; ++pb) {
              int pp = prem + pb * 16 + (lane & 15);
              float v = acc[pb][r];
              if (a.mode == 0) {
                a.dd[((size_t)n * Cin + ci) * HWo + pp] = v;
              } else {
                int oy = pp / Wo, ox = pp % Wo, iy = oy * a.S + a.off, ix = ox * a.S + a.off;
                if (iy < a.H && ix < a.W) {
                  size_t xi = plane_off(n, ci, a.N, Cin, a.xnodes, (size_t)a.H * a.W) + (size_t)iy * a.W + ix;
                  if (a.overwrite) a.gx[xi] = a.x[xi] > 0.f ? v : 0.f;
                  else if (a.x[xi] > 0.f) a.gx[xi] += v;
                }
              }
            }
          }
        }
      } else {
        for (int ci = wave; ci < Cin; ci += 4) {
          const int ciu = __builtin_amdgcn_readfirstlane(ci);
          float v = 0.f;
          for (int co = 0; co < Cout; ++co) v += a.pw[co * Cin + ciu] * sDz[co * PS + lane];
          int pp = prem + lane;
          if (a.mode == 0) {
            a.dd[((size_t)n * Cin + ciu) * HWo + pp] = v;
          } else {
            int oy = pp / Wo, ox = pp % Wo, iy = oy * a.S + a.off, ix = ox * a.S + a.off;
            if (iy < a.H && ix < a.W) {
              size_t xi = plane_off(n, ciu, a.N, Cin, a.xnodes, (size_t)a.H * a.W) + (size_t)iy * a.W + ix;
              if (a.overwrite) a.gx[xi] = a.x[xi] > 0.f ? v : 0.f;
              else if (a.x[xi] > 0.f) a.gx[xi] += v;
            }
          }
        }
      }
    }
    __syncthreads();
  }
  if (a.gW) {
    float* gW = a.gW + (size_t)rep_slot() * a.gstride;
    if (MFMA) {
#pragma unroll
      for (int j = 0; j < MBLK; ++j) {
        int b = wave + 4 * j;
        if (b < nblk) {
          int cob = (b / nbi) * 16, cib = (b % nbi) * 16;
#pragma unroll
          for (int r = 0; r < 4; ++r)
            atomicAdd(gW + (cob + (lane >> 4) * 4 + r) * Cin + cib + (lane & 15), macc[j][r]);
        }
      }
    } else {
#pragma unroll
      for (int j = 0; j < MAXJ; ++j) {
        int pr = tid + 256 * j;
        if (pr < npairs) atomicAdd(gW + pr, gacc[j]);
      }
    }
  }
}

template <int CI, int CO, bool V4>
__global__ void __launch_bounds__(256) pw_bwd_px_kernel(PwBwdBatch bt) {
  const PwBwdArgs& a = bt.e[blockIdx.y];
  const int HWo = a.Ho * a.Wo, Wo = a.Wo;
  const int total = a.N * HWo;
  __shared__ float sC[4 * CO + 1];
  __shared__ float sGW[CI * CO];
  const int tid = threadIdx.x, lane = tid & 63;
  const float wv = (tid == 0 && a.gs.w) ? a.gs.w[a.gs.widx] : 1.f;
  bn_gs_coop(a.gs, a.co_off, CO, sC, sC + CO, sC + 2 * CO, sC + 3 * CO);
  if (tid == 0) sC[4 * CO] = wv;
  for (int i = tid; i < CI * CO; i += 256) sGW[i] = 0.f;
  __syncthreads();
  float mean[CO], inv[CO], m1[CO], m2[CO];
#pragma unroll
  for (int c = 0; c < CO; ++c) {
    mean[c] = sC[c];
    inv[c] = sC[CO + c];
    m1[c] = sC[2 * CO + c];
    m2[c] = sC[3 * CO + c];
  }
  const float wk = sC[4 * CO];
  float wpw[CI * CO];
#pragma unroll
  for (int i = 0; i < CI * CO; ++i) wpw[i] = a.pw[i];
  float gacc[CI * CO];
#pragma unroll
  for (int i = 0; i < CI * CO; ++i) gacc[i] = 0.f;
  const bool want_w = a.gW != nullptr;
  if (V4) {
    typedef float f4 __attribute__((ext_vector_type(4)));
    for (int t = blockIdx.x * 256 + tid; t < total / 4; t += gridDim.x * 256) {
      const int p = t * 4, n = p / HWo, pp = p - n * HWo;
      f4 dz[CO], av[CI];
#pragma unroll
      for (int c = 0; c < CO; ++c) {
        const size_t gi = ((size_t)n * a.CoutTotal + a.co_off + c) * HWo + pp;
        const f4 zz = zld4(a.gs.z + gi), gg = *reinterpret_cast<const f4*>(a.gs.g + gi);
        dz[c] = wk * inv[c] * (gg - m1[c] - ((zz - mean[c]) * inv[c]) * m2[c]);
      }
#pragma unroll
      for (int c = 0; c < CI; ++c) {
        const size_t o = a.mode == 0 ? ((size_t)n * CI + c) * HWo + pp : plane_off(n, c, a.N, CI, a.xnodes, HWo) + pp;
        av[c] = a.mode == 0 ? zld4(a.ain + o) : *reinterpret_cast<const f4*>(a.x + o);
        if (a.mode != 0) {
          av[c].x = fmaxf(av[c].x, 0.f);
          av[c].y = fmaxf(av[c].y, 0.f);
          av[c].z = fmaxf(av[c].z, 0.f);
          av[c].w = fmaxf(av[c].w, 0.f);
        }
      }
      if (want_w) {
#pragma unroll
        for (int co = 0; co < CO; ++co)
#pragma unroll
          for (int ci = 0; ci < CI; ++ci) {
            const f4 t2 = dz[co] * av[ci];
            gacc[co * CI + ci] += (t2.x + t2.y) + (t2.z + t2.w);
          }
      }
      if (a.need_dx) {
#pragma unroll
        for (int ci = 0; ci < CI; ++ci) {
          f4 v = {0.f, 0.f, 0.f, 0.f};
#pragma unroll
          for (int co = 0; co < CO; ++co) v += wpw[co * CI + ci] * dz[co];
          const size_t o = a.mode == 0 ? ((size_t)n * CI + ci) * HWo + pp : plane_off(n, ci, a.N, CI, a.xnodes, HWo) + pp;
          if (a.mode == 0) {
            *reinterpret_cast<f4*>(a.dd + o) = v;
          } else {
            f4 m;
            m.x = av[ci].x > 0.f ? v.x : 0.f;
            m.y = av[ci].y > 0.f ? v.y : 0.f;
            m.z = av[ci].z > 0.f ? v.z : 0.f;
            m.w = av[ci].w > 0.f ? v.w : 0.f;
            f4* g = reinterpret_cast<f4*>(a.gx + o);
            *g = a.overwrite ? m : *g + m;
          }
        }
      }
    }
  }
  for (int p = blockIdx.x * 256 + tid; p < (V4 ? 0 : total); p += gridDim.x * 256) {
    const int n = p / HWo, pp = p - n * HWo;
    float dz[CO], av[CI];
#pragma unroll
    for (int c = 0; c < CO; ++c)
      dz[c] = bn_bwd_val(a.gs, ((size_t)n * a.CoutTotal + a.co_off + c) * HWo + pp, mean[c], inv[c], wk, m1[c], m2[c]);
    size_t xi0 = 0;
    bool inb = true;
    if (a.mode == 0) {
#pragma unroll
      for (int c = 0; c < CI; ++c) av[c] = z2f(a.ain[((size_t)n * CI + c) * HWo + pp]);
    } else {
      const int oy = pp / Wo, ox = pp - oy * Wo, iy = oy * a.S + a.off, ix = ox * a.S + a.off;
      inb = iy < a.H && ix < a.W;
      xi0 = inb ? (size_t)iy * a.W + ix : 0;
      float raw[CI];
#pragma unroll
      for (int c = 0; c < CI; ++c) raw[c] = a.x[plane_off(n, c, a.N, CI, a.xnodes, (size_t)a.H * a.W) + xi0];
#pragma unroll
      for (int c = 0; c < CI; ++c) av[c] = inb ? fmaxf(raw[c], 0.f) : 0.f;
    }
    if (want_w) {
#pragma unroll
      for (int co = 0; co < CO; ++co)
#pragma unroll
        for (int ci = 0; ci < CI; ++ci) gacc[co * CI + ci] += dz[co] * av[ci];
    }
    if (a.need_dx) {
#pragma unroll
      for (int ci = 0; ci < CI; ++ci) {
        float v = 0.f;
#pragma unroll
        for (int co = 0; co < CO; ++co) v += wpw[co * CI + ci] * dz[co];
        if (a.mode == 0) {
          a.dd[((size_t)n * CI + ci) * HWo + pp] = v;
        } else if (a.overwrite) {
          a.gx[plane_off(n, ci, a.N, CI, a.xnodes, (size_t)a.H * a.W) + xi0] = av[ci] > 0.f ? v : 0.f;
        } else if (inb && av[ci] > 0.f) {
          a.gx[plane_off(n, ci, a.N, CI, a.xnodes, (size_t)a.H * a.W) + xi0] += v;
        }
      }
    }
  }
  if (!want_w) return;
  wave_sums_to_lds<CI * CO>(gacc, sGW, lane);
  __syncthreads();
  float* gW = a.gW + (size_t)rep_slot() * a.gstride;
  for (int i = tid; i < CI * CO; i += 256) atomicAdd(gW + i, sGW[i]);
}


template <int CI, int CO, int NS = 1>
__global__ void __launch_bounds__(256) pw_bwd_wave_kernel(PwBwdBatch bt) {
  static_assert(CI % 16 == 0 && CO % 16 == 0 && CI <= 128 && CO <= 64 && (CI / 16) % NS == 0, "16-channel blocks");
  constexpr int BO = CO / 16, BI = CI / 16 / NS, RS = 64 + 4;
  typedef float f4 __attribute__((ext_vector_type(4)));
  const PwBwdArgs& a = bt.e[blockIdx.y];
  const int HWo = a.Ho * a.Wo, Wo = a.Wo;
  const int nchunks = a.N * HWo / 64;
  extern __shared__ __attribute__((aligned(16))) float smem[];
  __shared__ float sC[4 * CO + 1];
  const int tid = threadIdx.x, wave = tid >> 6, lane = tid & 63;
  const int c16 = lane & 15, q = lane >> 4;
  const float wv = (tid == 0 && a.gs.w) ? a.gs.w[a.gs.widx] : 1.f;
  bn_gs_coop(a.gs, a.co_off, CO, sC, sC + CO, sC + 2 * CO, sC + 3 * CO);
  if (tid == 0) sC[4 * CO] = wv;
  __syncthreads();
  const float wk = sC[4 * CO];
  float mean[BO], inv[BO], m1[BO], m2[BO];
#pragma unroll
  for (int bo = 0; bo < BO; ++bo) {
    const int c = bo * 16 + c16;
    mean[bo] = sC[c];
    inv[bo] = sC[CO + c];
    m1[bo] = sC[2 * CO + c];
    m2[bo] = sC[3 * CO + c];
  }
  const bool want_w = a.gW != nullptr;
  const bool flat = a.mode == 0 || (a.S == 1 && a.off == 0 && a.H == a.Ho && a.W == a.Wo);
  const bool fr2 = a.mode != 0 && a.S == 2 && a.H == 2 * a.Ho && a.W == 2 * a.Wo && a.W % 4 == 0 && a.off <= 1 &&
                   ((uintptr_t)a.x & 15) == 0;
  float* sT = smem + wave * CO * RS;
  const int ci0 = ((blockIdx.x * 4 + wave) % NS) * BI * 16;
  f4 macc[BO][BI];
#pragma unroll
  for (int bo = 0; bo < BO; ++bo)
#pragma unroll
    for (int bi = 0; bi < BI; ++bi) macc[bo][bi] = f4{0.f, 0.f, 0.f, 0.f};
  for (int w = blockIdx.x * 4 + wave; w < nchunks * NS; w += gridDim.x * 4) {
    const int pix0 = (w / NS) * 64, n = pix0 / HWo, prem = pix0 - n * HWo;
    const int pq = prem + q * 16;
    float dz[BO][16];
#pragma unroll
    for (int bo = 0; bo < BO; ++bo) {
      const size_t gi = ((size_t)n * a.CoutTotal + a.co_off + bo * 16 + c16) * HWo + pq;
#pragma unroll
      for (int t = 0; t < 4; ++t) {
        const f4 zz = zld4(a.gs.z + gi + 4 * t);
        const f4 gg = *reinterpret_cast<const f4*>(a.gs.g + gi + 4 * t);
        const f4 v = wk * inv[bo] * (gg - m1[bo] - ((zz - mean[bo]) * inv[bo]) * m2[bo]);
        dz[bo][4 * t] = v.x;
        dz[bo][4 * t + 1] = v.y;
        dz[bo][4 * t + 2] = v.z;
        dz[bo][4 * t + 3] = v.w;
      }
    }
    if (want_w) {
      float av[BI][16];
#pragma unroll
      for (int bi = 0; bi < BI; ++bi) {
        const int ci = ci0 + bi * 16 + c16;
        if (flat) {
          const size_t so = a.mode == 0 ? ((size_t)n * CI + ci) * HWo + pq : plane_off(n, ci, a.N, CI, a.xnodes, HWo) + pq;
#pragma unroll
          for (int t = 0; t < 4; ++t) {
            f4 v = a.mode == 0 ? zld4(a.ain + so + 4 * t) : *reinterpret_cast<const f4*>(a.x + so + 4 * t);
            if (a.mode != 0) v = f4{fmaxf(v.x, 0.f), fmaxf(v.y, 0.f), fmaxf(v.z, 0.f), fmaxf(v.w, 0.f)};
            av[bi][4 * t] = v.x;
            av[bi][4 * t + 1] = v.y;
            av[bi][4 * t + 2] = v.z;
            av[bi][4 * t + 3] = v.w;
          }
        } else if (fr2) {
          const float* plane = a.x + plane_off(n, ci, a.N, CI, a.xnodes, (size_t)a.H * a.W);
#pragma unroll
          for (int j = 0; j < 16; j += 2) fr2_pair(plane, a.W, Wo, a.off, pq + j, av[bi][j], av[bi][j + 1]);
        } else {
#pragma unroll
          for (int j = 0; j < 16; ++j) {
            const int pp = pq + j, oy = pp / Wo, ox = pp - oy * Wo, iy = oy * a.S + a.off, ix = ox * a.S + a.off;
            av[bi][j] = (iy < a.H && ix < a.W)
                            ? fmaxf(a.x[plane_off(n, ci, a.N, CI, a.xnodes, (size_t)a.H * a.W) + (size_t)iy * a.W + ix], 0.f)
                            : 0.f;
          }
        }
      }
#pragma unroll
      for (int j = 0; j < 16; ++j)
#pragma unroll
        for (int bo = 0; bo < BO; ++bo)
#pragma unroll
          for (int bi = 0; bi < BI; ++bi)
            macc[bo][bi] = __builtin_amdgcn_mfma_f32_16x16x4f32(dz[bo][j], av[bi][j], macc[bo][bi], 0, 0, 0);
    }
    if (!a.need_dx) continue;
    wave_lds_sync();
#pragma unroll
    for (int bo = 0; bo < BO; ++bo)
#pragma unroll
      for (int t = 0; t < 4; ++t)
        *reinterpret_cast<f4*>(sT + (bo * 16 + c16) * RS + q * 16 + 4 * t) =
            f4{dz[bo][4 * t], dz[bo][4 * t + 1], dz[bo][4 * t + 2], dz[bo][4 * t + 3]};
    wave_lds_sync();
#pragma unroll
    for (int bi = 0; bi < BI; ++bi) {
      f4 acc[4] = {{0, 0, 0, 0}, {0, 0, 0, 0}, {0, 0, 0, 0}, {0, 0, 0, 0}};
#pragma unroll
      for (int k0 = 0; k0 < CO; k0 += 4) {
        const float av = a.pw[(k0 + q) * CI + ci0 + bi * 16 + c16];
#pragma unroll
        for (int pb = 0; pb < 4; ++pb)
          acc[pb] = __builtin_amdgcn_mfma_f32_16x16x4f32(av, sT[(k0 + q) * RS + pb * 16 + c16], acc[pb], 0, 0, 0);
      }
#pragma unroll
      for (int r = 0; r < 4; ++r) {
        const int ci = ci0 + bi * 16 + q * 4 + r;
#pragma unroll
        for (int pb = 0; pb < 4; ++pb) {
          const int pp = prem + pb * 16 + c16;
          const float v = acc[pb][r];
          if (a.mode == 0) {
            a.dd[((size_t)n * CI + ci) * HWo + pp] = v;
          } else {
            const int oy = pp / Wo, ox = pp - oy * Wo, iy = oy * a.S + a.off, ix = ox * a.S + a.off;
            if (iy < a.H && ix < a.W) {
              const size_t xi = plane_off(n, ci, a.N, CI, a.xnodes, (size_t)a.H * a.W) + (size_t)iy * a.W + ix;
              if (a.overwrite) a.gx[xi] = a.x[xi] > 0.f ? v : 0.f;
              else if (a.x[xi] > 0.f) a.gx[xi] += v;
            }
          }
        }
      }
    }
  }
  if (!want_w) return;
  __syncthreads();
  float* sG = smem;
  for (int i = tid; i < CO * CI; i += 256) sG[i] = 0.f;
  __syncthreads();
#pragma unroll
  for (int bo = 0; bo < BO; ++bo)
#pragma unroll
    for (int bi = 0; bi < BI; ++bi)
#pragma unroll
      for (int r = 0; r < 4; ++r) atomicAdd(sG + (bo * 16 + q * 4 + r) * CI + ci0 + bi * 16 + c16, macc[bo][bi][r]);
  __syncthreads();
  float* gW = a.gW + (size_t)rep_slot() * a.gstride;
  for (int i = tid; i < CO * CI; i += 256) atomicAdd(gW + i, sG[i]);
}

template <int CI, int CO>
static bool try_pw_bwd_px(const PwBwdBatch& b, hipStream_t st) {
  const PwBwdArgs& a = b.e[0];
  if (a.Cin != CI || a.Cout != CO) return false;
  const int total = a.N * a.Ho * a.Wo;
  const int per_edge = std::max(1, std::min((total + 255) / 256, max_blocks() / std::max(2 * b.n, 1)));
  hipLaunchKernelGGL((pw_bwd_px_kernel<CI, CO, false>), dim3(per_edge, b.n), dim3(256), 0, st, b);
  return true;
}

template <int CI, int CO>
static bool try_pw_bwd_wave(const PwBwdBatch& b, hipStream_t st) {
  const PwBwdArgs& a = b.e[0];
  if (a.Cin != CI || a.Cout != CO || (a.Ho * a.Wo) % 64 != 0) return false;
  for (int e = 0; e < b.n; ++e) {
    const PwBwdArgs& x = b.e[e];
    const bool flat = x.mode == 0 || (x.S == 1 && x.off == 0 && x.H == x.Ho && x.W == x.Wo);
    const uintptr_t bits = (uintptr_t)x.gs.z | (uintptr_t)x.gs.g | (flat ? (x.mode == 0 ? (uintptr_t)x.ain : (uintptr_t)x.x) : (uintptr_t)0);
    if (bits & 15) return false;
  }
  constexpr int BI = CI / 16;
  const int chunks = a.N * a.Ho * a.Wo / 64;
  int ns = 1;
  while (BI % (2 * ns) == 0 && chunks * ns * b.n < 4096) ns *= 2;
  const int per_edge = std::max(1, std::min((chunks * ns + 3) / 4, max_blocks() / std::max(b.n, 1)));
  const size_t lds = sizeof(float) * 4 * CO * (64 + 4);
  const dim3 grid(per_edge, b.n);
  if (ns == 1) hipLaunchKernelGGL((pw_bwd_wave_kernel<CI, CO, 1>), grid, dim3(256), lds, st, b);
  else if constexpr (BI % 2 == 0) {
    if (ns == 2) hipLaunchKernelGGL((pw_bwd_wave_kernel<CI, CO, 2>), grid, dim3(256), lds, st, b);
    else if constexpr (BI % 4 == 0) hipLaunchKernelGGL((pw_bwd_wave_kernel<CI, CO, 4>), grid, dim3(256), lds, st, b);
  }
  return true;
}

void launch_pw_bwd(const PwBwdBatch& b, hipStream_t st) {
  const PwBwdArgs& a = b.e[0];
  if (try_pw_bwd_px<4, 4>(b, st) || try_pw_bwd_px<8, 8>(b, st) || try_pw_bwd_px<4, 8>(b, st) ||
      try_pw_bwd_px<8, 4>(b, st) || try_pw_bwd_px<12, 8>(b, st) || try_pw_bwd_px<2, 2>(b, st) ||
      try_pw_bwd_px<4, 2>(b, st) || try_pw_bwd_px<2, 4>(b, st))
    return;
  if (try_pw_bwd_wave<16, 16>(b, st) || try_pw_bwd_wave<32, 32>(b, st) || try_pw_bwd_wave<64, 64>(b, st) ||
      try_pw_bwd_wave<48, 16>(b, st) || try_pw_bwd_wave<48, 32>(b, st) || try_pw_bwd_wave<64, 32>(b, st) ||
      try_pw_bwd_wave<32, 16>(b, st) || try_pw_bwd_wave<128, 64>(b, st))
    return;
  int ntiles = a.N * a.Ho * a.Wo / 64;
  dim3 grid(per_edge_blocks(ntiles, b.n), b.n);
  size_t lds = sizeof(float) * (a.Cout * 65 + a.Cin * 65 + 4 * a.Cout + 4);
  const int nblk = (a.Cin % 16 == 0 && a.Cout % 16 == 0) ? (a.Cin / 16) * (a.Cout / 16) : 1 << 30;
  if (nblk <= 16) hipLaunchKernelGGL((pw_bwd_kernel<true, 4>), grid, dim3(256), lds, st, b);
  else if (nblk <= 32) hipLaunchKernelGGL((pw_bwd_kernel<true, 8>), grid, dim3(256), lds, st, b);
  else hipLaunchKernelGGL((pw_bwd_kernel<false>), grid, dim3(256), lds, st, b);
}


}
```

### katib_amd/ops/hip_darts.py

```python

from __future__ import annotations

import contextlib
import importlib
import weakref
from collections import defaultdict
from typing import Dict, List, Optional, Sequence, Tuple

import torch

from .. import _hipload

try:
    _K = _hipload.hipkern()
except ImportError as e:
    raise ImportError("katib_amd._hipkern is not built (run __graft_entry__.build()): %s" % e)

F64 = torch.float64
REP = int(_K.REP)
ZDT = torch.bfloat16 if bool(getattr(_K, "ZBF16", False)) else torch.float32
FOLD = True
_R = 1 if FOLD else REP
SELFFOLD = False
_CTR: Dict[int, torch.Tensor] = {}


def set_selffold(on: bool):
    global SELFFOLD
    if on and _SYNC is not None:
        raise RuntimeError("self-folding producers cannot run under SyncBN (see _check_sync_fold_mode)")
    SELFFOLD = bool(on)
    _K.set_selffold(SELFFOLD)
_CTR_SIZE = 64 * 33 * 32


def _selffold(dev) -> bool:
    if not FOLD or not SELFFOLD:
        return False
    idx = dev.index if dev.index is not None else torch.cuda.current_device()
    if idx not in _CTR:
        if torch.cuda.is_current_stream_capturing():
            return bool(_K.selffold_ready())
        t = torch.zeros(_CTR_SIZE, dtype=torch.int32, device=torch.device("cuda", idx))
        _K.set_fold_counters(t)
        _CTR[idx] = t
    return bool(_K.selffold_ready())


_SYNC = None


def _check_sync_fold_mode():
    if not FOLD:
        raise RuntimeError("SyncBN needs the fold launches (hip_darts.FOLD): the cross-rank BN sum "
                           "happens inside them")
    if SELFFOLD:
        raise RuntimeError("SyncBN is incompatible with self-folding producers (hip_darts.SELFFOLD): "
                           "their replicas would never be summed over the ranks")


class SyncBN:

    def __init__(self, comm):
        _check_sync_fold_mode()
        self.comm, self.world = comm, comm.world_size
        self.ws = None
        if comm.xgmi is not None:
            from ..parallel import xgmi

            ar = xgmi.create(comm, capacity=1 << 16, blocks=16)
            self.ws = ar.ws if ar is not None else None
        self.rccl_graph = self.ws is None and comm.probe_rccl_capture()
        self.folds = 0

    @property
    def capturable(self) -> bool:
        return self.ws is not None or self.rccl_graph

    @property
    def path(self) -> str:
        return "xgmi-oneshot" if self.ws is not None else ("rccl-graph" if self.rccl_graph else "host")

    def fold(self, segs):
        self.folds += 1
        if self.ws is not None:
            self.ws.fold_sync(list(segs))
            return
        _K.fold_f64([tuple(sg[:3]) for sg in segs])
        self.comm.allreduce_sum_many_([sg[0][:sg[1]] for sg in segs if len(sg) < 4 or sg[3]])


class sync_scope:

    def __init__(self, sync):
        self.sync = sync

    def __enter__(self):
        global _SYNC
        if self.sync is not None:
            _check_sync_fold_mode()
        self.prev, _SYNC = _SYNC, self.sync
        return self

    def __exit__(self, *exc):
        global _SYNC
        _SYNC = self.prev
        return False


def _world() -> int:
    return _SYNC.world if _SYNC is not None else 1


def _fold(segs):
    if _SYNC is not None:
        _SYNC.fold(segs)
    else:
        _K.fold_f64([tuple(sg[:3]) for sg in segs])


def _defer(dev) -> bool:
    return DEFER_FOLD and FOLD and _SYNC is None and not _selffold(dev)


def _fold64(segs, dev=None):
    if FOLD and (dev is None or not _selffold(dev)):
        _fold(segs)
_CAP = {"combine_fwd": 4, "dwpw_fwd": 8, "pw_fwd": 16, "pool_fwd": 8, "combine_bwd_reduce": 4, "pw_bwd": 16,
        "dw_bwd": 20, "pool_bwd": 8}
_REPLICATED: List[Tuple[weakref.ref, int]] = []


class _Arena:

    def __init__(self):
        self.buf: Optional[torch.Tensor] = None
        self.keep: List[torch.Tensor] = []
        self.off = 0
        self.used = 0
        self.need = 0
        self.active = False
        self.pending_zero = False


_ARENA = _Arena()


def arena_begin(device, deferred_zero: bool = False):
    a = _ARENA
    if a.need and (a.buf is None or a.buf.numel() < a.need):
        if a.buf is not None:
            a.keep.append(a.buf)
        a.buf = torch.zeros(a.need, dtype=F64, device=device)
        a.pending_zero = False
    elif a.buf is not None:
        if deferred_zero:
            a.pending_zero = True
        else:
            a.buf.zero_()
    a.off, a.used, a.active = 0, 0, True


def arena_end():
    a = _ARENA
    a.need = max(a.need, a.used)
    a.active = False
    if a.pending_zero:
        a.buf.zero_()
        a.pending_zero = False


def zeros64(n: int, device) -> torch.Tensor:
    a = _ARENA
    if a.active:
        if a.pending_zero and a.buf is not None:
            a.buf.zero_()
            a.pending_zero = False
        step = (n + 31) // 32 * 32
        a.used += step
        if a.buf is not None and a.off + step <= a.buf.numel() and a.buf.device == device:
            t = a.buf[a.off:a.off + n]
            a.off += step
            return t
    return torch.zeros(n, dtype=F64, device=device)


def register_grad_replicas(buf: torch.Tensor):
    if buf.dim() != 2 or buf.shape[0] != REP or not buf.is_contiguous() or buf.dtype != torch.float32:
        raise ValueError("replicated gradient buffer must be contiguous fp32 [%d][n]" % REP)
    _REPLICATED.append((weakref.ref(buf), buf.shape[1]))


def fold(buf: torch.Tensor):
    _K.fold_rows(buf)


def _replica_stride(g: torch.Tensor) -> int:
    ptr = g.data_ptr()
    for ref, n in list(_REPLICATED):
        buf = ref()
        if buf is None:
            _REPLICATED.remove((ref, n))
            continue
        base = buf.data_ptr()
        if base <= ptr and ptr + g.numel() * 4 <= base + n * 4:
            return n
    return 0


def _launch(name: str, calls: List, *args):
    cap = _CAP[name]
    fn = getattr(_K, name)
    for i in range(0, len(calls), cap):
        fn(calls[i:i + cap], *args)


MULTI = True
DEFER_FOLD = True


def _unfolded(bn):
    return bn[:6] + (REP, bn[7])


DWB_MULTI = True
EDGE_BWD = False


JOINT_POOL = False


def _dwpw_multi(entries):
    if not entries:
        return
    if MULTI:
        for i in range(0, len(entries), 20):
            _K.dwpw_fwd_multi(entries[i:i + 20])
        return
    groups = defaultdict(list)
    for e in entries:
        groups[e[7:]].append(e[:7])
    for (K, dil, S, pad), calls in groups.items():
        _launch("dwpw_fwd", calls, K, dil, S, pad, True)


def _pool_multi(entries):
    if not entries:
        return
    if MULTI:
        for i in range(0, len(entries), _CAP["pool_fwd"]):
            _K.pool_fwd_multi(entries[i:i + _CAP["pool_fwd"]])
        return
    groups = defaultdict(list)
    for e in entries:
        groups[e[6]].append(e[:6])
    for S, calls in groups.items():
        _launch("pool_fwd", calls, S)


class EdgeSpec:

    def __init__(self, prims: Sequence[str], stride: int, pnames: List[str], slots: Dict[str, Tuple[int, ...]]):
        self.prims = list(prims)
        self.stride = stride
        self.pnames = pnames
        self.slots = slots
        self.nbn = sum(len(v) for v in slots.values())
        self.pidx = {n: i for i, n in enumerate(pnames)}


def _bn(stats: Optional[torch.Tensor], rm, rv, count: int, training: bool, eps: float, C: int):
    if training:
        return (stats, rm, rv, 1.0 / (count * _world()), False, eps, _R, 2 * C)
    return (None, rm, rv, 1.0 / count, True, eps, 1, 2 * C)


class _Sinks:

    def __init__(self):
        self.temps = []

    def get(self, p: torch.Tensor, key):
        if not p.requires_grad:
            return None, 0
        g = p.grad if p.is_leaf else None
        if g is not None and g.is_contiguous():
            stride = _replica_stride(g)
            if stride:
                return g, stride
        t = torch.zeros(REP, p.numel(), device=p.device, dtype=torch.float32)
        self.temps.append((key, t, g, p))
        return t[0].view_as(p), p.numel()

    def finish(self, grads: List):
        for key, t, g, p in self.temps:
            s = t.sum(0).view_as(p)
            if g is not None:
                g.add_(s)
            else:
                grads[key] = s


class _Edge:

    def __init__(self, i, x, w, spec: EdgeSpec, bn, params):
        self.i, self.x, self.w, self.spec, self.bn = i, x, w, spec, bn
        self.P = dict(zip(spec.pnames, params))
        self.S = spec.stride
        self.refs = []
        self.zs, self.bns, self.widx = {}, {}, []
        self.saved = {}
        self.id_idx, self.xid = -1, None
        self.upd = []
        self.id_done = False


def _node_forward(xs, ws, specs, bns, params_list, training, momentum, eps, out=None, extra_fold=()):
    E = len(specs)
    xs = [t.contiguous() for t in xs]
    _selffold(xs[0].device)
    N, C = xs[0].shape[:2]
    S0 = specs[0].stride
    Ho = (xs[0].shape[2] - 1) // S0 + 1
    Wo = (xs[0].shape[3] - 1) // S0 + 1
    cnt = N * Ho * Wo
    dev = xs[0].device
    slot = REP * 2 * C
    edges, off = [], 0
    for i in range(E):
        edges.append(_Edge(i, xs[i], ws[i], specs[i], bns[i], params_list[i]))
    nslots = sum(e.spec.nbn for e in edges)
    stats = zeros64(max(nslots, 1) * slot, dev) if training else None
    base = 0
    for e in edges:
        e.slot0 = base
        e.refs = [_bn(stats[(base + i) * slot:(base + i + 1) * slot] if training else None, e.bn[i][0],
                      e.bn[i][1], cnt, training, eps, C) for i in range(e.spec.nbn)]
        base += e.spec.nbn

    def st(e, i):
        return stats[(e.slot0 + i) * slot:(e.slot0 + i + 1) * slot] if training else None

    def new():
        return torch.empty(N, C, Ho, Wo, device=dev, dtype=ZDT)

    dw_groups = defaultdict(list)
    pool_groups = defaultdict(list)
    fr_calls = []
    stage1, stage2 = [], []
    for e in edges:
        for k, prim in enumerate(e.spec.prims):
            if prim == "none":
                continue
            sl = e.spec.slots.get(prim, ())
            if prim.startswith("separable_convolution"):
                K = int(prim[-1])
                d1, z1 = new(), new()
                dw_groups[(K, 1, e.S, K // 2)].append(
                    (e.x, e.P[prim + ".0.dw"], e.P[prim + ".0.pw"], None, d1, z1, st(e, sl[0])))
                e.saved[prim] = [d1, z1]
                stage1.append(e.slot0 + sl[0])
                stage2.append(e.slot0 + sl[1])
            elif prim.startswith("dilated_convolution"):
                K = int(prim[-1])
                d, z = new(), new()
                dw_groups[(K, 2, e.S, (K // 2) * 2)].append(
                    (e.x, e.P[prim + ".dw"], e.P[prim + ".pw"], None, d, z, st(e, sl[0])))
                e.zs[k], e.bns[k] = z, e.refs[sl[0]]
                e.saved[prim] = (d, z)
                stage1.append(e.slot0 + sl[0])
            elif prim in ("avg_pooling_3x3", "max_pooling_3x3"):
                if "pool" not in e.saved:
                    za, zm = new(), new()
                    am = torch.empty(N, C, Ho, Wo, dtype=torch.uint8, device=dev)
                    sa = e.spec.slots.get("avg_pooling_3x3")
                    sm = e.spec.slots.get("max_pooling_3x3")
                    pool_groups[e.S].append((e.x, za, zm, st(e, sa[0]) if sa else None,
                                             st(e, sm[0]) if sm else None, am))
                    e.saved["pool"] = (za, zm, am)
                e.zs[k] = e.saved["pool"][0 if prim == "avg_pooling_3x3" else 1]
                e.bns[k] = e.refs[sl[0]]
                stage1.append(e.slot0 + sl[0])
            elif prim == "skip_connection":
                if e.S == 1:
                    e.id_idx, e.xid = k, e.x
                    continue
                z = new()
                fr_calls.append((e.x, e.P[prim + ".conv1"], z, st(e, sl[0]), 0, 0))
                fr_calls.append((e.x, e.P[prim + ".conv2"], z, st(e, sl[0]), C // 2, 1))
                e.zs[k], e.bns[k] = z, e.refs[sl[0]]
                e.saved[prim] = (z,)
                stage1.append(e.slot0 + sl[0])
            else:
                raise ValueError(prim)
            e.widx.append(k)
    dw1 = [(*c, K, dil, S, pad) for (K, dil, S, pad), calls in dw_groups.items() for c in calls]
    pools = [(*c, S) for S, calls in pool_groups.items() for c in calls]
    if JOINT_POOL and MULTI and dw1 and pools and len(dw1) <= 20 and len(pools) <= _CAP["pool_fwd"]:
        _K.dwpw_pool_fwd_multi(dw1, pools)
    else:
        _dwpw_multi(dw1)
        _pool_multi(pools)
    if fr_calls:
        _launch("pw_fwd", fr_calls, 2)
    defer = training and _defer(dev)
    if training and stage1 and not defer:
        _fold64([(stats[i * slot:(i + 1) * slot], 2 * C, 2 * C) for i in sorted(set(stage1))], dev)
    s2_groups = defaultdict(list)
    for e in edges:
        for k, prim in enumerate(e.spec.prims):
            if prim.startswith("separable_convolution"):
                K = int(prim[-1])
                sl = e.spec.slots[prim]
                d1, z1 = e.saved[prim]
                d2, z2 = new(), new()
                inbn = _unfolded(e.refs[sl[0]]) if defer else e.refs[sl[0]]
                s2_groups[K].append((z1, e.P[prim + ".1.dw"], e.P[prim + ".1.pw"], inbn, d2, z2, st(e, sl[1])))
                e.upd.append(e.refs[sl[0]])
                e.zs[k], e.bns[k] = z2, e.refs[sl[1]]
                e.saved[prim] = (d1, z1, d2, z2)
    _dwpw_multi([(*c, K, 1, 1, K // 2) for K, calls in s2_groups.items() for c in calls])
    if training and (stage2 or (defer and stage1) or extra_fold):
        _fold64([(stats[i * slot:(i + 1) * slot], 2 * C, 2 * C)
                 for i in sorted(set(stage2 + (stage1 if defer else [])))] + list(extra_fold), dev)
    if out is None:
        out = torch.empty(N, C, Ho, Wo, device=dev)
    ccalls = []
    for e in edges:
        e.zl = [e.zs[k] for k in e.widx]
        e.bl = [e.bns[k] for k in e.widx]
        ccalls.append((e.zl, e.bl, e.widx, e.w, e.id_idx, e.xid, e.upd if training else []))
    cap = _CAP["combine_fwd"]
    for i in range(0, E, cap):
        _K.combine_fwd(ccalls[i:i + cap], None, None, out, momentum, training, i > 0)
    return out, edges


def _node_backward(edges, training, C, dout, gx_of, take_first, sinks, pkey, cell_gw=None):
    E = len(edges)
    dout = dout.contiguous()
    dev = dout.device

    def sink(e, name):
        return sinks.get(e.P[name], pkey(e, name))

    sizes = []
    for e in edges:
        e.nred = (len(e.zl) + 1) * C + 1
        sizes.append(REP * (e.nred + e.w.numel()))
    buf = zeros64(sum(sizes), dev)
    o = 0
    calls, segs = [], []
    for e, sz in zip(edges, sizes):
        e.red = buf[o:o + REP * e.nred]
        e.gw = buf[o + REP * e.nred:o + sz]
        o += sz
        calls.append((dout, e.zl, e.bl, e.x if e.id_idx >= 0 else None, e.red, e.widx, e.id_idx, e.gw))
        segs += [(e.red, e.nred, e.nred), (e.gw, e.w.numel(), e.w.numel(), False)]
    _launch("combine_bwd_reduce", calls)
    defer = training and _defer(dev)
    nofold = defer and cell_gw is not None and not EDGE_BWD
    if nofold:
        cell_gw.extend(segs[1::2])
    if not _selffold(dev) and not defer:
        _fold(segs if FOLD else segs[1::2])

    r_early = REP if defer else _R
    r_late = REP if nofold else _R

    def src(e, k, z, rep=r_late):
        j = e.widx.index(k)
        return (dout, z, e.red[:C], e.red[(1 + j) * C:(2 + j) * C], e.bl[j], e.w, k, rep, e.nred)

    gxs = [gx_of(e.i) for e in edges]

    dils = [(e, k, p) for e in edges for k, p in enumerate(e.spec.prims) if p.startswith("dilated_convolution")]
    pwd, dd_of = [], {}
    for e, k, prim in dils:
        d, z = e.saved[prim]
        dd = torch.empty(d.shape, device=dev)
        dd_of[(e.i, prim)] = dd
        g, gst = sink(e, prim + ".pw")
        pwd.append((src(e, k, z, r_early), e.P[prim + ".pw"], d, e.x, dd, None, g, 0, 0, gst))
    seps = [(e, k, p) for e in edges for k, p in enumerate(e.spec.prims) if p.startswith("separable_convolution")]
    if not seps and pwd:
        _launch("pw_bwd", pwd, 1, 0, True)
    if not seps and defer and not nofold:
        _fold(segs)
    if seps:
        red1 = zeros64(len(seps) * REP * 2 * C, dev) if training else None
        pw2, dw2 = [], defaultdict(list)
        for n, (e, k, prim) in enumerate(seps):
            K = int(prim[-1])
            d1, z1, d2, z2 = e.saved[prim]
            dd2 = torch.empty(d2.shape, device=dev)
            g, gst = sink(e, prim + ".1.pw")
            pw2.append((src(e, k, z2, r_early), e.P[prim + ".1.pw"], d2, z1, dd2, None, g, 0, 0, gst))
            g1 = torch.empty(z1.shape, device=dev)
            r1 = red1[n * REP * 2 * C:(n + 1) * REP * 2 * C] if training else None
            g, gst = sink(e, prim + ".1.dw")
            dw2[K].append((z1, e.refs[e.spec.slots[prim][0]], e.P[prim + ".1.dw"], dd2, g1, g, r1, gst, False))
            e.saved[prim + "/g1"] = (g1, r1)
        _launch("pw_bwd", pw2 + (pwd if MULTI else []), 1, 0, True)
        if not MULTI and pwd:
            _launch("pw_bwd", pwd, 1, 0, True)
        if MULTI:
            allc = [(*c, K) for K, calls in dw2.items() for c in calls]
            for i in range(0, len(allc), _CAP["dw_bwd"]):
                _K.dw_bwd_multi(allc[i:i + _CAP["dw_bwd"]])
        else:
            for K, calls in dw2.items():
                _launch("dw_bwd", calls, K, 1, 1, K // 2)
        if training and not nofold:
            _fold64([(red1[n * REP * 2 * C:(n + 1) * REP * 2 * C], 2 * C, 2 * C) for n in range(len(seps))]
                    + (segs if defer else []), dev)
        pw1 = []
        for e, k, prim in seps:
            d1, z1, d2, z2 = e.saved[prim]
            g1, r1 = e.saved[prim + "/g1"]
            b1 = e.refs[e.spec.slots[prim][0]]
            gs1 = (g1, z1, r1[:C] if training else None, r1[C:2 * C] if training else None, b1, None, 0, r_late, 2 * C)
            dd1 = torch.empty(d1.shape, device=dev)
            e.saved[prim + "/dd1"] = dd1
            g, gst = sink(e, prim + ".0.pw")
            pw1.append((gs1, e.P[prim + ".0.pw"], d1, e.x, dd1, None, g, 0, 0, gst))
        _launch("pw_bwd", pw1, 1, 0, True)

    first = {e.i: take_first(e.i) for e in edges}

    def tf(i):
        f = first.get(i, False)
        first[i] = False
        return f

    def pool_srcs(e):
        za, zm, am = e.saved["pool"]
        ga = gm = None
        for k, p in enumerate(e.spec.prims):
            if p == "avg_pooling_3x3":
                ga = src(e, k, za)
            elif p == "max_pooling_3x3":
                gm = src(e, k, zm)
        return ga, gm, am

    if EDGE_BWD:
        entries = []
        for e in edges:
            convs = [None] * 4
            for k, prim in enumerate(e.spec.prims):
                if prim.startswith("separable_convolution"):
                    g, gst = sink(e, prim + ".0.dw")
                    convs[0 if prim[-1] == "3" else 1] = (e.P[prim + ".0.dw"], e.saved[prim + "/dd1"], g, gst)
                elif prim.startswith("dilated_convolution"):
                    g, gst = sink(e, prim + ".dw")
                    convs[2 if prim[-1] == "3" else 3] = (e.P[prim + ".dw"], dd_of[(e.i, prim)], g, gst)
            ga, gm, am = pool_srcs(e) if "pool" in e.saved else (None, None, None)
            entries.append((e.x, gxs[e.i], first[e.i], convs, ga, gm, am, dout if e.id_idx >= 0 else None, e.w,
                            e.id_idx, e.S))
        ok = True
        for i in range(0, len(entries), 4):
            ok = ok and bool(_K.edge_bwd(entries[i:i + 4]))
        if ok:
            for e in edges:
                first[e.i] = False
        elif len(entries) > 4:
            raise RuntimeError("edge_bwd accepted part of a node's edges")
    if (not EDGE_BWD or not ok) and MULTI and DWB_MULTI:
        convs, parts = [], defaultdict(list)
        for e, k, prim in seps + dils:
            sep = prim.startswith("separable_convolution")
            K = int(prim[-1])
            t = torch.empty_like(e.x)
            parts[e.i].append(t)
            name = prim + (".0.dw" if sep else ".dw")
            g, gst = sink(e, name)
            dd = e.saved[prim + "/dd1"] if sep else dd_of[(e.i, prim)]
            convs.append((e.x, None, e.P[name], dd, t, g, None, gst, True, K, 1 if sep else 2, e.S))
        for i in range(0, len(convs), _CAP["dw_bwd"]):
            _K.dw_bwd_multi(convs[i:i + _CAP["dw_bwd"]])
        sums = []
        for e in edges:
            ga, gm, am = pool_srcs(e) if "pool" in e.saved else (None, None, None)
            ex = parts.get(e.i, [])
            if ga is None and gm is None and e.id_idx < 0 and not ex:
                continue
            sums.append((ga, gm, e.x, dout if e.id_idx >= 0 else None, e.w, e.id_idx, gxs[e.i], am, tf(e.i), e.S, ex))
            e.id_done = True
        for i in range(0, len(sums), _CAP["pool_bwd"]):
            _K.pool_bwd_multi(sums[i:i + _CAP["pool_bwd"]])
    elif not EDGE_BWD or not ok:
        if seps:
            dw1 = defaultdict(list)
            for e, k, prim in seps:
                K = int(prim[-1])
                g, gst = sink(e, prim + ".0.dw")
                dw1[(K, e.S)].append((e.x, None, e.P[prim + ".0.dw"], e.saved[prim + "/dd1"], gxs[e.i], g, None, gst,
                                      tf(e.i)))
            for (K, S), calls in dw1.items():
                _launch("dw_bwd", calls, K, 1, S, K // 2)
        if dils:
            dwd = defaultdict(list)
            for e, k, prim in dils:
                K = int(prim[-1])
                g, gst = sink(e, prim + ".dw")
                dwd[(K, e.S)].append((e.x, None, e.P[prim + ".dw"], dd_of[(e.i, prim)], gxs[e.i], g, None, gst,
                                      tf(e.i)))
            for (K, S), calls in dwd.items():
                _launch("dw_bwd", calls, K, 2, S, (K // 2) * 2)
        pools = defaultdict(list)
        for e in edges:
            if "pool" not in e.saved:
                continue
            ga, gm, am = pool_srcs(e)
            pools[e.S].append((ga, gm, e.x, dout if e.id_idx >= 0 else None, e.w, e.id_idx, gxs[e.i], am, tf(e.i)))
            e.id_done = True
        if MULTI:
            allp = [(*c, S) for S, calls in pools.items() for c in calls]
            for i in range(0, len(allp), _CAP["pool_bwd"]):
                _K.pool_bwd_multi(allp[i:i + _CAP["pool_bwd"]])
        else:
            for S, calls in pools.items():
                _launch("pool_bwd", calls, S)
        for e in edges:
            if e.id_idx >= 0 and not e.id_done:
                if tf(e.i):
                    torch.mul(dout, e.w[e.id_idx], out=gxs[e.i])
                else:
                    gxs[e.i].add_(dout * e.w[e.id_idx])
    frc = []
    for e in edges:
        if "skip_connection" in e.saved:
            if tf(e.i):
                gxs[e.i].zero_()
            k = e.spec.prims.index("skip_connection")
            (z,) = e.saved["skip_connection"]
            gs = src(e, k, z)
            g, gst = sink(e, "skip_connection.conv1")
            frc.append((gs, e.P["skip_connection.conv1"], None, e.x, None, gxs[e.i], g, 0, 0, gst))
            g, gst = sink(e, "skip_connection.conv2")
            frc.append((gs, e.P["skip_connection.conv2"], None, e.x, None, gxs[e.i], g, C // 2, 1, gst))
    if frc:
        _launch("pw_bwd", frc, 2, 1, True)


class _MixedNode(torch.autograd.Function):
    @staticmethod
    def forward(ctx, meta, *flat):
        specs, bns, training, momentum, eps, nparams = meta
        E = len(specs)
        params, off = [], 2 * E
        for n in nparams:
            params.append(flat[off:off + n])
            off += n
        out, edges = _node_forward(flat[:E], flat[E:2 * E], specs, bns, params, training, momentum, eps)
        ctx.meta = (edges, training, out.shape[1])
        ctx.save_for_backward(*flat)
        return out

    @staticmethod
    def backward(ctx, dout):
        flat = ctx.saved_tensors
        edges, training, C = ctx.meta
        E = len(edges)
        sinks = _Sinks()
        pbase, acc = [], 2 * E
        for e in edges:
            pbase.append(acc)
            acc += len(e.spec.pnames)
        gxs = [torch.empty_like(e.x) for e in edges]
        first = [True] * E

        def take_first(i):
            f = first[i]
            first[i] = False
            return f

        _node_backward(edges, training, C, dout, lambda i: gxs[i], take_first, sinks,
                       lambda e, name: pbase[e.i] + e.spec.pidx[name])
        for i in range(E):
            if first[i]:
                gxs[i].zero_()
        grads = [None] * len(flat)
        for i, e in enumerate(edges):
            grads[i] = gxs[i] if ctx.needs_input_grad[1 + i] else None
            grads[E + i] = e.gw[:e.w.numel()].to(e.w.dtype) if ctx.needs_input_grad[1 + E + i] else None
        sinks.finish(grads)
        return (None, *grads)


def mixed_node(xs: Sequence[torch.Tensor], ws: Sequence[torch.Tensor], specs: Sequence[EdgeSpec],
               bns: Sequence[List[Tuple[torch.Tensor, torch.Tensor]]], params: Sequence[Sequence[torch.Tensor]],
               training: bool, momentum: float = 0.1, eps: float = 1e-5):
    meta = (list(specs), list(bns), training, momentum, eps, [len(p) for p in params])
    flat = list(xs) + list(ws) + [p for ps in params for p in ps]
    return _MixedNode.apply(meta, *flat)


def mixed_edge(x, w, spec: EdgeSpec, bn: List[Tuple[torch.Tensor, torch.Tensor]], params: Sequence[torch.Tensor],
               training: bool, momentum: float = 0.1, eps: float = 1e-5):
    return mixed_node([x], [w], [spec], [bn], [params], training, momentum, eps)


def _dims(x: torch.Tensor):
    if x.dim() == 5:
        return x.shape[1], x.shape[0] * x.shape[2], x.shape[3], x.shape[4]
    return tuple(x.shape)


def _stdconv_forward(x, rm, rv, training, momentum, eps, w1, w2, defer=None):
    x = x.contiguous()
    _selffold(x.device)
    N, Cin, H, W = _dims(x)
    fr = w2 is not None
    Cout = w1.shape[0] * (2 if fr else 1)
    Ho, Wo = (H // 2, W // 2) if fr else (H, W)
    cnt = N * Ho * Wo
    stats = zeros64(REP * 2 * Cout, x.device) if training else None
    z = torch.empty(N, Cout, Ho, Wo, device=x.device, dtype=ZDT)
    if fr:
        _K.pw_fwd([(x, w1, z, stats, 0, 0), (x, w2, z, stats, Cout // 2, 1)], 2)
    else:
        _K.pw_fwd([(x, w1, z, stats, 0, 0)], 1)
    bn = _bn(stats, rm, rv, cnt, training, eps, Cout)
    late = defer is not None and training and _defer(x.device)
    if training and not late:
        _fold64([(stats, 2 * Cout, 2 * Cout)], x.device)
    if late:
        defer.append((stats, 2 * Cout, 2 * Cout))
    out = torch.empty(z.shape, device=x.device)
    _K.combine_fwd([([z], [_unfolded(bn) if late else bn], [0], None, -1, None, [])], None, None, out, momentum,
                   training, False)
    return out, (x, z, w1, w2, bn, fr, Cout, training)


def _stdconv_backward(state, dout, need_x, sinks, keys, gx=None, first=True):
    x, z, w1, w2, bn, fr, Cout, training = state
    dout = dout.contiguous()
    nred = 2 * Cout + 1
    red = zeros64(REP * nred, x.device)
    late = training and _defer(x.device)
    if training:
        _K.combine_bwd_reduce([(dout, [z], [bn], None, red, [0], -1, None)])
        if not late:
            _fold64([(red, nred, nred)], x.device)
    gs = (dout, z, red[:Cout], red[Cout:2 * Cout], bn, None, 0, REP if late else _R, nred)
    g1, s1 = sinks.get(w1, keys[0])
    given = gx is not None
    if fr:
        if need_x and not given:
            gx = torch.zeros_like(x)
        elif need_x and first:
            gx.zero_()
        g2, s2 = sinks.get(w2, keys[1])
        _K.pw_bwd([(gs, w1, None, x, None, gx, g1, 0, 0, s1), (gs, w2, None, x, None, gx, g2, Cout // 2, 1, s2)],
                  2, 1, need_x)
    else:
        if need_x and not given:
            gx = torch.empty_like(x)
        _K.pw_bwd([(gs, w1, None, x, None, gx, g1, 0, 0, s1, first or not given)], 1, 1, need_x)
    return gx if need_x else None


class _StdConvBN(torch.autograd.Function):
    @staticmethod
    def forward(ctx, x, rm, rv, training, momentum, eps, w1, w2):
        out, state = _stdconv_forward(x, rm, rv, training, momentum, eps, w1, w2)
        ctx.state = state
        ctx.save_for_backward(x, w1, *([w2] if w2 is not None else []))
        return out

    @staticmethod
    def backward(ctx, dout):
        sinks = _Sinks()
        grads = [None, None, None]
        gx = _stdconv_backward(ctx.state, dout, ctx.needs_input_grad[0], sinks, (1, 2))
        ctx.state = None
        sinks.finish(grads)
        return gx, None, None, None, None, None, grads[1], grads[2]


class CellSpec:

    def __init__(self, pre0, pre1, nodes, C):
        self.pre0, self.pre1, self.nodes, self.C = pre0, pre1, nodes, C
        self.names = list(pre0[1]) + list(pre1[1])
        for node in nodes:
            for _, pnames, _, _, _ in node:
                self.names += pnames
        self.index = {n: i for i, n in enumerate(self.names)}


def _cell_fwd(spec, s0, s1, wts, P, bn_of, training, momentum, eps):
    late = []

    def pre(x, p):
        kind, pnames, bname = p
        rm, rv = bn_of(bname)
        if kind == "fr":
            return _stdconv_forward(x, rm, rv, training, momentum, eps, P[pnames[0]], P[pnames[1]], late)
        return _stdconv_forward(x, rm, rv, training, momentum, eps, P[pnames[0]], None, late)
    t0, st0 = pre(s0, spec.pre0)
    t1, st1 = pre(s1, spec.pre1)
    states = [t0, t1]
    N, C = t0.shape[0], spec.C
    nn_ = len(spec.nodes)
    S = [e[0].stride for e in spec.nodes[0]]
    Ho = (t0.shape[2] - 1) // max(S) + 1 if S else t0.shape[2]
    Wo = (t0.shape[3] - 1) // max(S) + 1 if S else t0.shape[3]
    O = torch.empty(nn_, N, C, Ho, Wo, device=t0.device)
    node_states = []
    for i, node in enumerate(spec.nodes):
        xs = [states[src] for _, _, _, src, _ in node]
        ws = [wts[row] for _, _, _, _, row in node]
        specs = [es for es, _, _, _, _ in node]
        bns = [[bn_of(b) for b in bnames] for _, _, bnames, _, _ in node]
        plist = [[P[n] for n in pnames] for _, pnames, _, _, _ in node]
        out, edges = _node_forward(xs, ws, specs, bns, plist, training, momentum, eps, out=O[i],
                                   extra_fold=late if i == 0 else ())
        states.append(out)
        node_states.append(edges)
    return O, (spec, training, st0, st1, node_states, states, wts)


def _cell_bwd(state, gO, sinks, pkey, gx0, first0, gx1, first1, need0, need1, alpha_rows=None):
    spec, training, st0, st1, node_states, states, wts = state
    nn_ = len(spec.nodes)
    gS = [None, None] + [gO[i] for i in range(nn_)]
    first = [True, True] + [False] * nn_
    ga_rows = [None] * nn_
    cell_gw = []
    for i in reversed(range(nn_)):
        node = spec.nodes[i]
        edges = node_states[i]
        srcs = [src for _, _, _, src, _ in node]
        for src in srcs:
            if gS[src] is None:
                gS[src] = torch.empty_like(states[src])

        def take_first(k, srcs=srcs):
            f = first[srcs[k]]
            first[srcs[k]] = False
            return f

        _node_backward(edges, training, spec.C, gS[2 + i], lambda k, srcs=srcs: gS[srcs[k]], take_first, sinks,
                       lambda e, name, node=node: pkey(node[e.i][1][e.spec.pidx[name]]), cell_gw)
        if alpha_rows is not None:
            for e, (_, _, _, _, row) in zip(edges, node):
                alpha_rows.append((e.gw, e.w.numel(), wts[row], row))
        else:
            ga_rows[i] = [e.gw[:wts.shape[1]] for e in edges]
    for j in (0, 1):
        if first[j]:
            gS[j] = torch.zeros_like(states[j])
    gs0 = _stdconv_backward(st0, gS[0], need0, sinks, tuple(pkey(n) for n in spec.pre0[1]) + (None,), gx0, first0)
    gs1 = _stdconv_backward(st1, gS[1], need1, sinks, tuple(pkey(n) for n in spec.pre1[1]) + (None,), gx1, first1)
    gw = None
    if alpha_rows is None:
        if cell_gw:
            _K.fold_f64(cell_gw)
        gw = torch.cat([g for rows in ga_rows for g in rows]).view(wts.shape).to(torch.float32)
    return gs0, gs1, gw


class _Cell(torch.autograd.Function):

    @staticmethod
    def forward(ctx, meta, s0, s1, wts, *params):
        spec, bn_of, training, momentum, eps = meta
        P = dict(zip(spec.names, params))
        O, state = _cell_fwd(spec, s0, s1, wts, P, bn_of, training, momentum, eps)
        nn_, N, C, Ho, Wo = O.shape
        y = O.permute(1, 0, 2, 3, 4).reshape(N, nn_ * C, Ho, Wo)
        ctx.cell = state
        ctx.save_for_backward(s0, s1, wts, *params)
        return y

    @staticmethod
    def backward(ctx, dy):
        state = ctx.cell
        ctx.cell = None
        spec = state[0]
        saved = ctx.saved_tensors
        params = saved[3:]
        nn_ = len(spec.nodes)
        N, C = dy.shape[0], spec.C
        Ho, Wo = dy.shape[2], dy.shape[3]
        gO = dy.reshape(N, nn_, C * Ho * Wo).transpose(0, 1).contiguous().view(nn_, N, C, Ho, Wo)
        sinks = _Sinks()
        need = ctx.needs_input_grad
        grads = [None] * (4 + len(params))
        gs0, gs1, gw = _cell_bwd(state, gO, sinks, lambda n: 4 + spec.index[n], None, True, None, True, need[1],
                                 need[2])
        grads[1], grads[2] = gs0, gs1
        if need[3]:
            grads[3] = gw
        sinks.finish(grads)
        return tuple(grads)


def cell_forward(spec: CellSpec, s0, s1, wts, params: Sequence[torch.Tensor], bn_of, training: bool,
                 momentum: float = 0.1, eps: float = 1e-5):
    return _Cell.apply((spec, bn_of, training, momentum, eps), s0, s1, wts, *params)


def relu_conv_bn(x, w, rm, rv, training, momentum=0.1, eps=1e-5):
    return _StdConvBN.apply(x, rm, rv, training, momentum, eps, w, None)


def factorized_reduce_bn(x, w1, w2, rm, rv, training, momentum=0.1, eps=1e-5):
    return _StdConvBN.apply(x, rm, rv, training, momentum, eps, w1, w2)


def supported(x: torch.Tensor, stride: int) -> bool:
    if not x.is_cuda or x.dtype != torch.float32 or x.dim() != 4:
        return False
    N, C, H, W = x.shape
    Ho, Wo = (H - 1) // stride + 1, (W - 1) // stride + 1
    return (C <= 256 and C * C <= 4096 and Wo <= 64 and 64 % Wo == 0 and Ho % (64 // Wo) == 0
            and H == Ho * stride and W == Wo * stride)


class _StemConv(torch.autograd.Function):

    @staticmethod
    def forward(ctx, x, w):
        x, w = x.contiguous(), w.contiguous()
        N, _, H, W = x.shape
        y = torch.empty(N, w.shape[0], H, W, device=x.device, dtype=x.dtype)
        _K.stem_conv_fwd(x, w, y)
        ctx.save_for_backward(x, w)
        return y

    @staticmethod
    def backward(ctx, dy):
        x, w = ctx.saved_tensors
        dy = dy.contiguous()
        gx = gw = None
        if ctx.needs_input_grad[1]:
            chunks = stem_chunks(x, w.shape[0])
            partial = torch.empty(chunks, w.numel(), device=x.device, dtype=torch.float32)
            gw = torch.empty_like(w)
            _K.stem_conv_wgrad(x, dy, partial, gw)
        if ctx.needs_input_grad[0]:
            gx = torch.nn.grad.conv2d_input(x.shape, w, dy, padding=1)
        return gx, gw


def _stem_fwd(x, w, gamma, beta, rm, rv, momentum, eps):
    x, w = x.contiguous(), w.contiguous()
    N, _, H, W = x.shape
    C = w.shape[0]
    stats = zeros64(REP * 2 * C, x.device)
    z = torch.empty(N, C, H, W, device=x.device, dtype=x.dtype)
    _K.stem_conv_fwd_stats(x, w, z, stats)
    _fold([(stats, 2 * C, 2 * C)])
    bn = _bn(stats, rm, rv, N * H * W, True, eps, C)
    out = torch.empty_like(z)
    zs = z if ZDT == z.dtype else z.to(ZDT)
    _K.combine_fwd([([zs], [bn], [0], None, -1, None, [])], gamma, beta, out, momentum, True, False)
    return out, (x, w, gamma, beta, z, zs, bn, eps, stats)


def _stem_bwd(state, dout, sinks, keys, need):
    x, w, gamma, beta, z, zs, bn, eps, stats = state
    dout = dout.contiguous()
    C = w.shape[0]
    nred = 2 * C + 1
    red = zeros64(REP * nred, x.device)
    _K.combine_bwd_reduce([(dout, [zs], [bn], None, red, [0], -1, None)])
    if not _selffold(x.device):
        _fold([(red, nred, nred)])
    gg, _ = sinks.get(gamma, keys[1]) if need[2] else (None, 0)
    gb, _ = sinks.get(beta, keys[2]) if need[3] else (None, 0)
    gw = gx = None
    if need[1] or need[2] or need[3]:
        chunks = stem_chunks(x, C)
        partial = torch.empty(chunks, w.numel(), device=x.device, dtype=torch.float32)
        if need[1]:
            gdst, _ = sinks.get(w, keys[0])
            _K.stem_conv_wgrad_bn(x, dout, z, red, stats, gamma, eps, gg, gb, partial, gdst, _world(), True)
        else:
            _K.stem_conv_wgrad_bn(x, dout, z, red, stats, gamma, eps, gg, gb, partial, torch.empty_like(w), _world())
    if need[0]:
        m = stats[:C] / z[:, 0].numel()
        var = (stats[C:2 * C] / z[:, 0].numel() - m * m).clamp_min(0)
        istd = torch.rsqrt(var.float() + eps).view(1, C, 1, 1)
        zhat = (z - m.float().view(1, C, 1, 1)) * istd
        m1 = (red[:C] / z[:, 0].numel()).float().view(1, C, 1, 1)
        m2 = (red[C:2 * C] / z[:, 0].numel()).float().view(1, C, 1, 1)
        dz = gamma.view(1, C, 1, 1) * istd * (dout - m1 - zhat * m2)
        gx = torch.nn.grad.conv2d_input(x.shape, w, dz, padding=1)
    return gx, gw


class _StemConvBN(torch.autograd.Function):

    @staticmethod
    def forward(ctx, x, w, gamma, beta, rm, rv, momentum, eps):
        out, state = _stem_fwd(x, w, gamma, beta, rm, rv, momentum, eps)
        ctx.stem = state
        return out

    @staticmethod
    def backward(ctx, dout):
        state = ctx.stem
        ctx.stem = None
        need = ctx.needs_input_grad
        grads = [None] * 8
        sinks = _Sinks()
        gx, _ = _stem_bwd(state, dout, sinks, (1, 2, 3), need[:4])
        grads[0] = gx
        sinks.finish(grads)
        return tuple(grads)


def stem_conv_bn(x, w, gamma, beta, rm, rv, momentum=0.1, eps=1e-5):
    return _StemConvBN.apply(x, w, gamma, beta, rm, rv, momentum, eps)


@torch.no_grad()
def stem_bn_eval(z, gamma, beta, rm, rv, eps=1e-5):
    z = z.contiguous()
    N, C, H, W = z.shape
    out = torch.empty(z.shape, device=z.device)
    zs = z if z.dtype == ZDT else z.to(ZDT)
    _K.combine_fwd([([zs], [_bn(None, rm, rv, N * H * W, False, eps, C)], [0], None, -1, None, [])], gamma, beta, out,
                   0.0, False, False)
    return out


def stem_chunks(x: torch.Tensor, cout: int) -> int:
    pixels = x.shape[0] * x.shape[2] * x.shape[3]
    return max(1, min(pixels // 1024, max(16, 1024 // cout)))


def stem_supported(x: torch.Tensor, w: torch.Tensor) -> bool:
    return (x.is_cuda and x.dtype == torch.float32 and w.dtype == torch.float32 and x.dim() == 4
            and x.shape[1] in (1, 3) and tuple(w.shape[1:]) == (x.shape[1], 3, 3) and w.shape[0] <= 64
            and x.numel() < (1 << 31) // 64)


def stem_conv(x: torch.Tensor, w: torch.Tensor) -> torch.Tensor:
    return _StemConv.apply(x, w)


class _Head(torch.autograd.Function):

    @staticmethod
    def forward(ctx, x, w, b, y):
        x = x.contiguous()
        N, C = x.shape[:2]
        K = w.shape[0]
        dev = x.device
        pooled = torch.empty(N, C, device=dev)
        logits = torch.empty(N, K, device=dev)
        dl = torch.empty(N, K, device=dev)
        loss_n = torch.empty(N, device=dev)
        loss = torch.empty((), device=dev)
        _K.head_fwd(x, w, b, y, pooled, logits, dl, loss_n)
        _K.head_loss(loss_n, loss)
        ctx.save_for_backward(dl, pooled, w, b)
        ctx.xshape = x.shape
        ctx.mark_non_differentiable(logits)
        ctx.set_materialize_grads(False)
        return loss, logits

    @staticmethod
    def backward(ctx, gloss, _glogits):
        dl, pooled, w, b = ctx.saved_tensors
        grads = [None, None, None, None]
        if gloss is None:
            return tuple(grads)
        need = ctx.needs_input_grad
        dev = dl.device
        x_like = torch.empty((), device=dev).expand(ctx.xshape)
        dx = torch.empty(ctx.xshape, device=dev) if need[0] else None
        sinks = _Sinks()
        gw, sw = sinks.get(w, 1) if need[1] else (None, 0)
        gb, sb = sinks.get(b, 2) if need[2] else (None, 0)
        _K.head_bwd(x_like, dl, pooled, w, gloss.reshape(()).contiguous().float(), dx, gw, sw, gb, sb)
        grads[0] = dx
        sinks.finish(grads)
        return tuple(grads)


def head_supported(x: torch.Tensor, w: torch.Tensor, y: torch.Tensor) -> bool:
    return (x.is_cuda and x.dim() == 4 and x.dtype == torch.float32 and w.dtype == torch.float32
            and w.dim() == 2 and w.shape[1] == x.shape[1] and x.shape[1] <= 1024 and w.shape[0] <= 64
            and y.dtype == torch.int64 and y.dim() == 1 and y.shape[0] == x.shape[0])


def head_loss(x: torch.Tensor, w: torch.Tensor, b: torch.Tensor, y: torch.Tensor):
    return _Head.apply(x, w, b, y.contiguous())


class NetSpec:

    def __init__(self, stem, cells, reduce, head):
        self.stem, self.cells, self.reduce, self.head = stem, list(cells), list(reduce), head
        names = list(stem[:3])
        for c in self.cells:
            names += c.names
        names += list(head)
        self.names = names
        self.index = {n: i for i, n in enumerate(names)}


def _alpha_grad(entries):
    groups = defaultdict(list)
    for ent in entries:
        groups[ent[3].data_ptr()].append(ent)
    chunk = []
    for rows in groups.values():
        if len(chunk) + len(rows) > 64:
            _K.alpha_grad(chunk, True)
            chunk = []
        chunk += rows
    if chunk:
        _K.alpha_grad(chunk, True)


class _Network(torch.autograd.Function):

    @staticmethod
    def forward(ctx, meta, x, y, an, ar, *params):
        spec, bn_of, training, momentum, eps = meta
        P = dict(zip(spec.names, params))
        dev = x.device
        mats, outs = [an], [torch.empty_like(an)]
        if ar is not None:
            mats.append(ar)
            outs.append(torch.empty_like(ar))
        zero = None
        a = _ARENA
        if training and a.pending_zero and a.buf is not None and a.buf.device == dev:
            zero, a.pending_zero = a.buf, False
        _K.alpha_softmax(mats, outs, zero)
        wn, wr = outs[0], (outs[1] if ar is not None else None)
        conv, gamma, beta, bname = spec.stem
        rm, rv = bn_of(bname)
        if training:
            s, st_stem = _stem_fwd(x, P[conv], P[gamma], P[beta], rm, rv, momentum, eps)
        else:
            s, st_stem = stem_bn_eval(stem_conv(x, P[conv]), P[gamma], P[beta], rm, rv, eps), None
        tensors = [s]
        cells = []
        i0 = i1 = 0
        for cspec, red in zip(spec.cells, spec.reduce):
            O, st = _cell_fwd(cspec, tensors[i0], tensors[i1], wr if red else wn, P, bn_of, training, momentum, eps)
            tensors.append(O)
            cells.append((st, i0, i1, len(tensors) - 1, red))
            i0, i1 = i1, len(tensors) - 1
        feat = tensors[i1]
        hw, hb = spec.head
        N, C = _dims(feat)[:2]
        K = P[hw].shape[0]
        pooled = torch.empty(N, C, device=dev)
        logits = torch.empty(N, K, device=dev)
        dl = torch.empty(N, K, device=dev)
        loss_n = torch.empty(N, device=dev)
        loss = torch.empty((), device=dev)
        _K.head_fwd(feat, P[hw], P[hb], y, pooled, logits, dl, loss_n)
        _K.head_loss(loss_n, loss)
        ctx.net = (spec, P, training, st_stem, cells, tensors, i1, dl, pooled, an, ar)
        ctx.mark_non_differentiable(logits)
        ctx.set_materialize_grads(False)
        return loss, logits

    @staticmethod
    def backward(ctx, gloss, _glogits):
        spec, P, training, st_stem, cells, tensors, last, dl, pooled, an, ar = ctx.net
        ctx.net = None
        grads = [None] * (5 + len(spec.names))
        if gloss is None:
            return tuple(grads)
        need = ctx.needs_input_grad
        sinks = _Sinks()

        def key(n):
            return 5 + spec.index[n]
        g, first = {last: torch.empty_like(tensors[last])}, {last: False}
        hw, hb = spec.head
        gw, sw = sinks.get(P[hw], key(hw)) if need[key(hw)] else (None, 0)
        gb, sb = sinks.get(P[hb], key(hb)) if need[key(hb)] else (None, 0)
        _K.head_bwd(tensors[last], dl, pooled, P[hw], gloss.reshape(()).contiguous().float(), g[last], gw, sw, gb, sb)
        rows = []
        for st, i0, i1, io, red in reversed(cells):
            for i in (i0, i1):
                if i not in g:
                    g[i], first[i] = torch.empty_like(tensors[i]), True
            f0 = first[i0]
            f1 = first[i1] and i1 != i0
            cell_rows = []
            _cell_bwd(st, g[io], sinks, key, g[i0], f0, g[i1], f1, True, True, cell_rows)
            first[i0] = first[i1] = False
            rows += [(r, red) for r in cell_rows]
        dst = {}
        for red, leaf, idx in ((False, an, 3), (True, ar, 4)):
            if leaf is None or not need[idx]:
                continue
            if leaf.is_leaf and leaf.grad is not None and leaf.grad.is_contiguous() and leaf.grad.dtype == torch.float32:
                dst[red] = leaf.grad
            else:
                dst[red] = grads[idx] = torch.zeros_like(leaf)
        ents = [(gw_, rs, wrow, dst[red][row]) for (gw_, rs, wrow, row), red in rows if red in dst]
        if ents:
            _alpha_grad(ents)
        conv, gamma, beta, _ = spec.stem
        if training and st_stem is not None and 0 in g:
            flags = (False, need[key(conv)], need[key(gamma)], need[key(beta)])
            _stem_bwd(st_stem, g[0], sinks, (key(conv), key(gamma), key(beta)), flags)
        sinks.finish(grads)
        return tuple(grads)


_MERGE_CAP = {"dwpw_fwd": 16, "pw_fwd": 32, "pool_fwd": 16, "combine_bwd_reduce": 8, "pw_bwd": 32, "dw_bwd": 40,
              "pool_bwd": 16, "dw_bwd_multi": 40, "dwpw_fwd_multi": 40, "pool_fwd_multi": 16,
              "pool_bwd_multi": 16, "fold_f64": 128, "alpha_grad": 128, "__sync_fold__": 64}
_QUERIES = {"selffold_ready", "max_blocks", "stamps_compiled", "REP", "ZBF16", "OPTIM_MAX_PARTS"}


class _Recorder:

    def __init__(self, real, tape, sync=False):
        self._real, self._tape, self._sync = real, tape, sync

    def __getattr__(self, name):
        attr = getattr(self._real, name)
        if self._sync:
            if name != "fold":
                return attr
            name = "__sync_fold__"
        elif name in _QUERIES or not callable(attr):
            return attr

        def rec(*args, **kw):
            self._tape.append((name, args, kw))
            return None

        return rec


def _same(x, y) -> bool:
    if torch.is_tensor(x) or torch.is_tensor(y):
        return x is y
    if isinstance(x, (list, tuple)) and isinstance(y, (list, tuple)):
        return len(x) == len(y) and all(_same(a, b) for a, b in zip(x, y))
    return x == y


class stacked_passes:

    def __init__(self):
        self.tapes: List[list] = []
        self.stats = {"launches": 0, "merged": 0}

    def __enter__(self):
        return self

    @contextlib.contextmanager
    def pass_(self):
        global _K, _SYNC
        if EDGE_BWD or JOINT_POOL or SELFFOLD:
            yield
            return
        tape: list = []
        self.tapes.append(tape)
        real_k, real_sync = _K, _SYNC
        _K = _Recorder(real_k, tape)
        if real_sync is not None:
            _SYNC = _Recorder(real_sync, tape, sync=True)
        try:
            yield
        finally:
            _K, _SYNC = real_k, real_sync

    def _call(self, name, args, kw):
        self.stats["launches"] += 1
        if name == "__sync_fold__":
            _SYNC.fold(*args, **kw)
        else:
            getattr(_K, name)(*args, **kw)

    def __exit__(self, et, ev, tb):
        if et is not None:
            return False
        tapes = self.tapes
        if not tapes:
            return False
        if len(tapes) != 2 or len(tapes[0]) != len(tapes[1]) or any(a[0] != b[0] for a, b in zip(*tapes)):
            for t in tapes:
                for name, args, kw in t:
                    self._call(name, args, kw)
            return False
        self._replay_merged(tapes)
        return False

    def _replay_merged(self, tapes):
        for (name, aa, ka), (_, ab, kb) in zip(*tapes):
            cap = _MERGE_CAP.get(name)
            if (cap and aa and ab and isinstance(aa[0], list) and isinstance(ab[0], list)
                    and len(aa[0]) + len(ab[0]) <= cap and len(aa) == len(ab) and _same(aa[1:], ab[1:])
                    and _same(sorted(ka.items()), sorted(kb.items()))):
                self.stats["merged"] += 1
                self._call(name, (list(aa[0]) + list(ab[0]),) + tuple(aa[1:]), ka)
            else:
                self._call(name, aa, ka)
                self._call(name, ab, kb)


def network_loss(spec: NetSpec, x, y, params: Sequence[torch.Tensor], an, ar, bn_of, training: bool,
                 momentum: float = 0.1, eps: float = 1e-5):
    return _Network.apply((spec, bn_of, training, momentum, eps), x, y, an, ar, *params)
```

Before: 2.135 s.

## Prune backward to needed gradients and skip storing unused depthwise outputs

```diff
diff --git a/katib_amd/csrc/hip/darts_bind.cpp b/katib_amd/csrc/hip/darts_bind.cpp
--- a/katib_amd/csrc/hip/darts_bind.cpp
+++ b/katib_amd/csrc/hip/darts_bind.cpp
@@ -168,24 +168,28 @@
                       bool use_mfma) {
   Tensor x = t[0].cast<Tensor>(), dw = t[1].cast<Tensor>(), pw = t[2].cast<Tensor>();
   auto inbn = t[3].cast<c10::optional<py::tuple>>();
-  Tensor d = t[4].cast<Tensor>(), z = t[5].cast<Tensor>();
+  OptT d = t[4].cast<OptT>();
+  Tensor z = t[5].cast<Tensor>();
   OptT stats = t[6].cast<OptT>();
+  const bool has_d = d.has_value() && d->defined();
   const bool has_inbn = t[3].cast<c10::optional<py::tuple>>().has_value();
   if (has_inbn) check_z(x, "x (previous stage z)");
   else check_f32(x, "x");
-  check_f32(dw, "dw"); check_f32(pw, "pw"); check_z(d, "d"); check_z(z, "z");
+  check_f32(dw, "dw"); check_f32(pw, "pw"); check_z(z, "z");
+  if (has_d) check_z(*d, "d");
   TORCH_CHECK(x.dim() == 4, "x must be NCHW");
   TORCH_CHECK((K == 3 || K == 5) && (dil == 1 || dil == 2) && (S == 1 || S == 2), "K in {3,5}, dil, S in {1,2}");
   const int N = x.size(0), C = x.size(1), H = x.size(2), W = x.size(3);
   const int Ho = z.size(2), Wo = z.size(3);
   TORCH_CHECK(dw.numel() == C * K * K && pw.numel() == C * C, "weight shapes");
-  TORCH_CHECK(z.size(0) == N && z.size(1) == C && d.sizes() == z.sizes(), "output shapes");
+  TORCH_CHECK(z.size(0) == N && z.size(1) == C && (!has_d || d->sizes() == z.sizes()), "output shapes");
+  TORCH_CHECK(has_d || !dwpw_split_path(C), "dw-pw stages of 16..64 channels (depthwise + pointwise GEMM) need d");
   TORCH_CHECK(C == 4 || C == 8 || C == 16 || (64 % Wo == 0 && Ho % (64 / Wo) == 0),
               "tile constraint: 64 % Wo == 0 and Ho % (64/Wo) == 0");
   TORCH_CHECK(C <= kMaxC, "C too large");
   TORCH_CHECK(Ho == (H + 2 * pad - dil * (K - 1) - 1) / S + 1, "output height mismatch");
   a.x = x.data_ptr(); a.dw = dw.data_ptr<float>(); a.pw = pw.data_ptr<float>();
-  a.d = zptr(d); a.z = zptr(z); a.stats = ptr_or_null<double>(stats);
+  a.d = has_d ? zptr(*d) : nullptr; a.z = zptr(z); a.stats = ptr_or_null<double>(stats);
   if (a.stats) TORCH_CHECK(stats->scalar_type() == at::kDouble && stats->numel() >= kRep * 2 * C, "stats f64 [kRep][2C]");
   a.N = N; a.C = C; a.H = H; a.W = W; a.Ho = Ho; a.Wo = Wo; a.pad = pad;
   const int TR = 64 / Wo;
@@ -486,7 +490,7 @@
     a.dd = ptr_or_null<float>(dd); a.gx = ptr_or_null<float>(gx);
     a.gW = ptr_or_null<float>(gW);
     if (mode == 0) {
-      TORCH_CHECK(a.ain && (!need_dx || a.dd), "mode 0 needs ain (and dd)");
+      TORCH_CHECK((a.ain || !a.gW) && (!need_dx || a.dd), "mode 0 needs ain for a weight gradient (and dd)");
     } else {
       TORCH_CHECK(!need_dx || a.gx, "mode 1 needs gx");
     }
@@ -782,6 +786,7 @@
   m.attr("REP") = kRep;
   m.attr("ZBF16") = kZbf16;
   m.def("max_blocks", &max_blocks);
+  m.def("dwpw_split_path", [](int64_t C) { return dwpw_split_path((int)C); });
   register_xgmi(m);
   register_conv(m);
   register_transformer(m);
diff --git a/katib_amd/csrc/hip/darts_ops.h b/katib_amd/csrc/hip/darts_ops.h
--- a/katib_amd/csrc/hip/darts_ops.h
+++ b/katib_amd/csrc/hip/darts_ops.h
@@ -38,6 +38,7 @@
 constexpr int kMaxOps = 8;
 constexpr int kMaxUpd = 4;
 constexpr int kMaxC = 256;
+constexpr bool dwpw_split_path(int C) { return C % 16 == 0 && C <= 64; }
 #ifndef KATIB_HIP_REP
 #define KATIB_HIP_REP 32
 #endif
diff --git a/katib_amd/csrc/hip/darts_ops_fwd.hip b/katib_amd/csrc/hip/darts_ops_fwd.hip
--- a/katib_amd/csrc/hip/darts_ops_fwd.hip
+++ b/katib_amd/csrc/hip/darts_ops_fwd.hip
@@ -45,7 +45,7 @@
       (a.Ho * a.Wo) % 64 != 0 || a.W % 4 != 0)
     return false;
   for (int i = 0; i < b.n; ++i)
-    if (((uintptr_t)b.e[i].x | (uintptr_t)b.e[i].d | (uintptr_t)b.e[i].z) & 15) return false;
+    if (!b.e[i].d || (((uintptr_t)b.e[i].x | (uintptr_t)b.e[i].d | (uintptr_t)b.e[i].z) & 15)) return false;
   const int G = a.C / CG;
   int nb = std::max(1, std::min(a.Ho / 4, 2048 / std::max(a.N * b.n * G, 1)));
   auto band_bytes = [&](int v) {
@@ -118,7 +118,7 @@
     const int code = a.variant >> 2;
     const int K = (code & 4) ? 5 : 3, DIL = (code & 2) ? 2 : 1, S = (code & 1) ? 2 : 1;
     const bool aligned = ((((uintptr_t)a.x) | (uintptr_t)a.d | (uintptr_t)a.z) & 15) == 0;
-    if (split && (!aligned || (a.Ho * a.Wo) % 64 != 0 || a.W % 4 != 0)) return false;
+    if (split && (!a.d || !aligned || (a.Ho * a.Wo) % 64 != 0 || a.W % 4 != 0)) return false;
     int nb = std::max(1, std::min(a.Ho / 4, 512 / std::max(N * b.n * G, 1)));
     auto band_bytes = [&](int v) {
       const int BR = (a.Ho + v - 1) / v;
diff --git a/katib_amd/csrc/hip/darts_ops_fwd_k.h b/katib_amd/csrc/hip/darts_ops_fwd_k.h
--- a/katib_amd/csrc/hip/darts_ops_fwd_k.h
+++ b/katib_amd/csrc/hip/darts_ops_fwd_k.h
@@ -61,7 +61,7 @@
 #pragma unroll
           for (int kx = 0; kx < K; ++kx) acc += wk[ky * K + kx] * src[ky * DIL * IW + kx * DIL];
         sD[c * P + p] = acc;
-        zput(a.d + (((size_t)n * C + c) * Ho + oy0 + ty) * Wo + tx, acc);
+        if (a.d) zput(a.d + (((size_t)n * C + c) * Ho + oy0 + ty) * Wo + tx, acc);
       }
       __syncthreads();
     }
@@ -203,6 +203,7 @@
   const int HWo = Ho * Wo;
   zt* dn = a.d + ((size_t)n * a.C + c0) * HWo;
   zt* zn = a.z + (size_t)n * C * HWo;
+  const bool put_d = !PW || a.d != nullptr;
   const bool vout = VEC && Wo % 4 == 0 && a.vout;
   if (vout) {
     constexpr int SPAN = 3 * S + (K - 1) * DIL + 1, NQ = (SPAN + 3) / 4;
@@ -245,7 +246,7 @@
           }
         }
         d[c] = acc;
-        zst4(dn + (size_t)c * HWo + p, acc);
+        if (put_d) zst4(dn + (size_t)c * HWo + p, acc);
       }
       if (!PW) continue;
 #pragma unroll
@@ -274,7 +275,7 @@
 #pragma unroll
         for (int kx = 0; kx < K; ++kx) acc += wk[ky * K + kx] * src[ky * DIL * WP + kx * DIL];
       d[c] = acc;
-      zput(dn + (size_t)c * HWo + p, acc);
+      if (put_d) zput(dn + (size_t)c * HWo + p, acc);
     }
     if (!PW) continue;
 #pragma unroll
diff --git a/katib_amd/csrc/hip/darts_ops_pwb.hip b/katib_amd/csrc/hip/darts_ops_pwb.hip
--- a/katib_amd/csrc/hip/darts_ops_pwb.hip
+++ b/katib_amd/csrc/hip/darts_ops_pwb.hip
@@ -47,7 +47,7 @@
       int pp = prem + p;
       float v;
       if (a.mode == 0) {
-        v = z2f(a.ain[((size_t)n * Cin + ci) * HWo + pp]);
+        v = a.gW ? z2f(a.ain[((size_t)n * Cin + ci) * HWo + pp]) : 0.f;
       } else {
         int oy = pp / Wo, ox = pp % Wo, iy = oy * a.S + a.off, ix = ox * a.S + a.off;
         v = (iy < a.H && ix < a.W)
@@ -203,7 +203,9 @@
 #pragma unroll
       for (int c = 0; c < CI; ++c) {
         const size_t o = a.mode == 0 ? ((size_t)n * CI + c) * HWo + pp : plane_off(n, c, a.N, CI, a.xnodes, HWo) + pp;
-        av[c] = a.mode == 0 ? zld4(a.ain + o) : *reinterpret_cast<const f4*>(a.x + o);
+        if (a.mode != 0) av[c] = *reinterpret_cast<const f4*>(a.x + o);
+        else if (want_w) av[c] = zld4(a.ain + o);
+        else av[c] = f4{0.f, 0.f, 0.f, 0.f};
         if (a.mode != 0) {
           av[c].x = fmaxf(av[c].x, 0.f);
           av[c].y = fmaxf(av[c].y, 0.f);
@@ -252,7 +254,7 @@
     bool inb = true;
     if (a.mode == 0) {
 #pragma unroll
-      for (int c = 0; c < CI; ++c) av[c] = z2f(a.ain[((size_t)n * CI + c) * HWo + pp]);
+      for (int c = 0; c < CI; ++c) av[c] = want_w ? z2f(a.ain[((size_t)n * CI + c) * HWo + pp]) : 0.f;
     } else {
       const int oy = pp / Wo, ox = pp - oy * Wo, iy = oy * a.S + a.off, ix = ox * a.S + a.off;
       inb = iy < a.H && ix < a.W;
diff --git a/katib_amd/ops/hip_darts.py b/katib_amd/ops/hip_darts.py
--- a/katib_amd/ops/hip_darts.py
+++ b/katib_amd/ops/hip_darts.py
@@ -113,7 +113,9 @@
 
 
 def _fold(segs):
-    if _SYNC is not None:
+    if not segs:
+        return
+    if _SYNC is not None and any(len(sg) < 4 or sg[3] for sg in segs):
         _SYNC.fold(segs)
     else:
         _K.fold_f64([tuple(sg[:3]) for sg in segs])
@@ -227,6 +229,10 @@
 EDGE_BWD = False
 
 
+NEEDED_GRADS = True
+DROP_D = True
+
+
 JOINT_POOL = False
 
 
@@ -315,7 +321,7 @@
         self.id_done = False
 
 
-def _node_forward(xs, ws, specs, bns, params_list, training, momentum, eps, out=None, extra_fold=()):
+def _node_forward(xs, ws, specs, bns, params_list, training, momentum, eps, out=None, extra_fold=(), grad=True):
     E = len(specs)
     xs = [t.contiguous() for t in xs]
     _selffold(xs[0].device)
@@ -344,6 +350,11 @@
     def new():
         return torch.empty(N, C, Ho, Wo, device=dev, dtype=ZDT)
 
+    keep_d = not DROP_D or bool(_K.dwpw_split_path(C))
+
+    def new_d(pw):
+        return new() if keep_d or (grad and pw.requires_grad) else None
+
     dw_groups = defaultdict(list)
     pool_groups = defaultdict(list)
     fr_calls = []
@@ -355,7 +366,7 @@
             sl = e.spec.slots.get(prim, ())
             if prim.startswith("separable_convolution"):
                 K = int(prim[-1])
-                d1, z1 = new(), new()
+                d1, z1 = new_d(e.P[prim + ".0.pw"]), new()
                 dw_groups[(K, 1, e.S, K // 2)].append(
                     (e.x, e.P[prim + ".0.dw"], e.P[prim + ".0.pw"], None, d1, z1, st(e, sl[0])))
                 e.saved[prim] = [d1, z1]
@@ -363,7 +374,7 @@
                 stage2.append(e.slot0 + sl[1])
             elif prim.startswith("dilated_convolution"):
                 K = int(prim[-1])
-                d, z = new(), new()
+                d, z = new_d(e.P[prim + ".pw"]), new()
                 dw_groups[(K, 2, e.S, (K // 2) * 2)].append(
                     (e.x, e.P[prim + ".dw"], e.P[prim + ".pw"], None, d, z, st(e, sl[0])))
                 e.zs[k], e.bns[k] = z, e.refs[sl[0]]
@@ -413,7 +424,7 @@
                 K = int(prim[-1])
                 sl = e.spec.slots[prim]
                 d1, z1 = e.saved[prim]
-                d2, z2 = new(), new()
+                d2, z2 = new_d(e.P[prim + ".1.pw"]), new()
                 inbn = _unfolded(e.refs[sl[0]]) if defer else e.refs[sl[0]]
                 s2_groups[K].append((z1, e.P[prim + ".1.dw"], e.P[prim + ".1.pw"], inbn, d2, z2, st(e, sl[1])))
                 e.upd.append(e.refs[sl[0]])
@@ -436,34 +447,45 @@
     return out, edges
 
 
-def _node_backward(edges, training, C, dout, gx_of, take_first, sinks, pkey, cell_gw=None):
-    E = len(edges)
+def _node_backward(edges, training, C, dout, gx_of, take_first, sinks, pkey, cell_gw=None, live=None,
+                   alpha_need=True):
     dout = dout.contiguous()
     dev = dout.device
+    if live is None:
+        live = [True] * len(edges)
+    for e in edges:
+        e.gw = None
+    entries = [e for e in edges if alpha_need or live[e.i]]
+    edges = [e for e in edges if live[e.i]]
+    if not entries:
+        return
 
     def sink(e, name):
         return sinks.get(e.P[name], pkey(e, name))
 
     sizes = []
-    for e in edges:
+    for e in entries:
         e.nred = (len(e.zl) + 1) * C + 1
         sizes.append(REP * (e.nred + e.w.numel()))
     buf = zeros64(sum(sizes), dev)
     o = 0
-    calls, segs = [], []
-    for e, sz in zip(edges, sizes):
+    calls, segs, gsegs = [], [], []
+    for e, sz in zip(entries, sizes):
         e.red = buf[o:o + REP * e.nred]
         e.gw = buf[o + REP * e.nred:o + sz]
         o += sz
         calls.append((dout, e.zl, e.bl, e.x if e.id_idx >= 0 else None, e.red, e.widx, e.id_idx, e.gw))
-        segs += [(e.red, e.nred, e.nred), (e.gw, e.w.numel(), e.w.numel(), False)]
+        if live[e.i]:
+            segs.append((e.red, e.nred, e.nred))
+        gsegs.append((e.gw, e.w.numel(), e.w.numel(), False))
+        segs.append(gsegs[-1])
     _launch("combine_bwd_reduce", calls)
     defer = training and _defer(dev)
     nofold = defer and cell_gw is not None and not EDGE_BWD
     if nofold:
-        cell_gw.extend(segs[1::2])
+        cell_gw.extend(gsegs)
     if not _selffold(dev) and not defer:
-        _fold(segs if FOLD else segs[1::2])
+        _fold(segs if FOLD else gsegs)
 
     r_early = REP if defer else _R
     r_late = REP if nofold else _R
@@ -472,13 +494,13 @@
         j = e.widx.index(k)
         return (dout, z, e.red[:C], e.red[(1 + j) * C:(2 + j) * C], e.bl[j], e.w, k, rep, e.nred)
 
-    gxs = [gx_of(e.i) for e in edges]
+    gxs = {e.i: gx_of(e.i) for e in edges}
 
     dils = [(e, k, p) for e in edges for k, p in enumerate(e.spec.prims) if p.startswith("dilated_convolution")]
     pwd, dd_of = [], {}
     for e, k, prim in dils:
         d, z = e.saved[prim]
-        dd = torch.empty(d.shape, device=dev)
+        dd = torch.empty(z.shape, device=dev)
         dd_of[(e.i, prim)] = dd
         g, gst = sink(e, prim + ".pw")
         pwd.append((src(e, k, z, r_early), e.P[prim + ".pw"], d, e.x, dd, None, g, 0, 0, gst))
@@ -493,7 +515,7 @@
         for n, (e, k, prim) in enumerate(seps):
             K = int(prim[-1])
             d1, z1, d2, z2 = e.saved[prim]
-            dd2 = torch.empty(d2.shape, device=dev)
+            dd2 = torch.empty(z2.shape, device=dev)
             g, gst = sink(e, prim + ".1.pw")
             pw2.append((src(e, k, z2, r_early), e.P[prim + ".1.pw"], d2, z1, dd2, None, g, 0, 0, gst))
             g1 = torch.empty(z1.shape, device=dev)
@@ -520,7 +542,7 @@
             g1, r1 = e.saved[prim + "/g1"]
             b1 = e.refs[e.spec.slots[prim][0]]
             gs1 = (g1, z1, r1[:C] if training else None, r1[C:2 * C] if training else None, b1, None, 0, r_late, 2 * C)
-            dd1 = torch.empty(d1.shape, device=dev)
+            dd1 = torch.empty(z1.shape, device=dev)
             e.saved[prim + "/dd1"] = dd1
             g, gst = sink(e, prim + ".0.pw")
             pw1.append((gs1, e.P[prim + ".0.pw"], d1, e.x, dd1, None, g, 0, 0, gst))
@@ -646,13 +668,13 @@
 class _MixedNode(torch.autograd.Function):
     @staticmethod
     def forward(ctx, meta, *flat):
-        specs, bns, training, momentum, eps, nparams = meta
+        specs, bns, training, momentum, eps, nparams, grad = meta
         E = len(specs)
         params, off = [], 2 * E
         for n in nparams:
             params.append(flat[off:off + n])
             off += n
-        out, edges = _node_forward(flat[:E], flat[E:2 * E], specs, bns, params, training, momentum, eps)
+        out, edges = _node_forward(flat[:E], flat[E:2 * E], specs, bns, params, training, momentum, eps, grad=grad)
         ctx.meta = (edges, training, out.shape[1])
         ctx.save_for_backward(*flat)
         return out
@@ -667,7 +689,9 @@
         for e in edges:
             pbase.append(acc)
             acc += len(e.spec.pnames)
-        gxs = [torch.empty_like(e.x) for e in edges]
+        need = ctx.needs_input_grad
+        live = [_edge_live(e, need[1 + e.i]) for e in edges]
+        gxs = [torch.empty_like(e.x) if lv else None for e, lv in zip(edges, live)]
         first = [True] * E
 
         def take_first(i):
@@ -676,14 +700,14 @@
             return f
 
         _node_backward(edges, training, C, dout, lambda i: gxs[i], take_first, sinks,
-                       lambda e, name: pbase[e.i] + e.spec.pidx[name])
+                       lambda e, name: pbase[e.i] + e.spec.pidx[name], None, live, any(need[1 + E:1 + 2 * E]))
         for i in range(E):
-            if first[i]:
+            if first[i] and live[i]:
                 gxs[i].zero_()
         grads = [None] * len(flat)
         for i, e in enumerate(edges):
-            grads[i] = gxs[i] if ctx.needs_input_grad[1 + i] else None
-            grads[E + i] = e.gw[:e.w.numel()].to(e.w.dtype) if ctx.needs_input_grad[1 + E + i] else None
+            grads[i] = gxs[i] if need[1 + i] else None
+            grads[E + i] = e.gw[:e.w.numel()].to(e.w.dtype) if need[1 + E + i] else None
         sinks.finish(grads)
         return (None, *grads)
 
@@ -691,7 +715,7 @@
 def mixed_node(xs: Sequence[torch.Tensor], ws: Sequence[torch.Tensor], specs: Sequence[EdgeSpec],
                bns: Sequence[List[Tuple[torch.Tensor, torch.Tensor]]], params: Sequence[Sequence[torch.Tensor]],
                training: bool, momentum: float = 0.1, eps: float = 1e-5):
-    meta = (list(specs), list(bns), training, momentum, eps, [len(p) for p in params])
+    meta = (list(specs), list(bns), training, momentum, eps, [len(p) for p in params], torch.is_grad_enabled())
     flat = list(xs) + list(ws) + [p for ps in params for p in ps]
     return _MixedNode.apply(meta, *flat)
 
@@ -790,7 +814,26 @@
         self.index = {n: i for i, n in enumerate(self.names)}
 
 
-def _cell_fwd(spec, s0, s1, wts, P, bn_of, training, momentum, eps):
+def needed_grads(spec: CellSpec, need0: bool, need1: bool, wreq, alpha: bool) -> List[bool]:
+    need = [need0 or any(wreq(n) for n in spec.pre0[1]), need1 or any(wreq(n) for n in spec.pre1[1])]
+    for node in spec.nodes:
+        need.append(any(alpha or need[src] or any(wreq(n) for n in pnames) for _, pnames, _, src, _ in node))
+    return need
+
+
+def network_needed_grads(spec: "NetSpec", wreq, alpha_n: bool, alpha_r: bool):
+    need = [any(wreq(n) for n in spec.stem[:3])]
+    i0 = i1 = 0
+    cells = []
+    for cspec, red in zip(spec.cells, spec.reduce):
+        c = needed_grads(cspec, need[i0], need[i1], wreq, alpha_r if red else alpha_n)
+        cells.append(c)
+        need.append(any(c[2:]))
+        i0, i1 = i1, len(need) - 1
+    return need[0], cells
+
+
+def _cell_fwd(spec, s0, s1, wts, P, bn_of, training, momentum, eps, grad=True):
     late = []
 
     def pre(x, p):
@@ -816,25 +859,36 @@
         bns = [[bn_of(b) for b in bnames] for _, _, bnames, _, _ in node]
         plist = [[P[n] for n in pnames] for _, pnames, _, _, _ in node]
         out, edges = _node_forward(xs, ws, specs, bns, plist, training, momentum, eps, out=O[i],
-                                   extra_fold=late if i == 0 else ())
+                                   extra_fold=late if i == 0 else (), grad=grad)
         states.append(out)
         node_states.append(edges)
-    return O, (spec, training, st0, st1, node_states, states, wts)
-
-
-def _cell_bwd(state, gO, sinks, pkey, gx0, first0, gx1, first1, need0, need1, alpha_rows=None):
-    spec, training, st0, st1, node_states, states, wts = state
+    return O, (spec, training, st0, st1, node_states, states, wts, P)
+
+
+def _edge_live(e, src_need: bool) -> bool:
+    return not NEEDED_GRADS or src_need or any(p.requires_grad for p in e.P.values())
+
+
+def _cell_bwd(state, gO, sinks, pkey, gx0, first0, gx1, first1, need0, need1, alpha_rows=None, alpha_need=True):
+    spec, training, st0, st1, node_states, states, wts, P = state
     nn_ = len(spec.nodes)
+    if NEEDED_GRADS:
+        need = needed_grads(spec, need0, need1, lambda n: P[n].requires_grad, alpha_need)
+    else:
+        need = [True] * (2 + nn_)
     gS = [None, None] + [gO[i] for i in range(nn_)]
     first = [True, True] + [False] * nn_
     ga_rows = [None] * nn_
     cell_gw = []
     for i in reversed(range(nn_)):
+        if not need[2 + i]:
+            continue
         node = spec.nodes[i]
         edges = node_states[i]
         srcs = [src for _, _, _, src, _ in node]
-        for src in srcs:
-            if gS[src] is None:
+        live = [_edge_live(e, need[src]) for e, src in zip(edges, srcs)]
+        for src, lv in zip(srcs, live):
+            if lv and gS[src] is None:
                 gS[src] = torch.empty_like(states[src])
 
         def take_first(k, srcs=srcs):
@@ -843,32 +897,36 @@
             return f
 
         _node_backward(edges, training, spec.C, gS[2 + i], lambda k, srcs=srcs: gS[srcs[k]], take_first, sinks,
-                       lambda e, name, node=node: pkey(node[e.i][1][e.spec.pidx[name]]), cell_gw)
+                       lambda e, name, node=node: pkey(node[e.i][1][e.spec.pidx[name]]), cell_gw, live, alpha_need)
         if alpha_rows is not None:
             for e, (_, _, _, _, row) in zip(edges, node):
-                alpha_rows.append((e.gw, e.w.numel(), wts[row], row))
-        else:
+                if e.gw is not None:
+                    alpha_rows.append((e.gw, e.w.numel(), wts[row], row))
+        elif alpha_need:
             ga_rows[i] = [e.gw[:wts.shape[1]] for e in edges]
-    for j in (0, 1):
+    gs = [None, None]
+    for j, (st, needx, gx, fst, pre) in enumerate(((st0, need0, gx0, first0, spec.pre0),
+                                                   (st1, need1, gx1, first1, spec.pre1))):
+        if not need[j]:
+            continue
         if first[j]:
             gS[j] = torch.zeros_like(states[j])
-    gs0 = _stdconv_backward(st0, gS[0], need0, sinks, tuple(pkey(n) for n in spec.pre0[1]) + (None,), gx0, first0)
-    gs1 = _stdconv_backward(st1, gS[1], need1, sinks, tuple(pkey(n) for n in spec.pre1[1]) + (None,), gx1, first1)
+        gs[j] = _stdconv_backward(st, gS[j], needx, sinks, tuple(pkey(n) for n in pre[1]) + (None,), gx, fst)
     gw = None
-    if alpha_rows is None:
+    if alpha_rows is None and alpha_need:
         if cell_gw:
             _K.fold_f64(cell_gw)
         gw = torch.cat([g for rows in ga_rows for g in rows]).view(wts.shape).to(torch.float32)
-    return gs0, gs1, gw
+    return gs[0], gs[1], gw
 
 
 class _Cell(torch.autograd.Function):
 
     @staticmethod
     def forward(ctx, meta, s0, s1, wts, *params):
-        spec, bn_of, training, momentum, eps = meta
+        spec, bn_of, training, momentum, eps, grad = meta
         P = dict(zip(spec.names, params))
-        O, state = _cell_fwd(spec, s0, s1, wts, P, bn_of, training, momentum, eps)
+        O, state = _cell_fwd(spec, s0, s1, wts, P, bn_of, training, momentum, eps, grad)
         nn_, N, C, Ho, Wo = O.shape
         y = O.permute(1, 0, 2, 3, 4).reshape(N, nn_ * C, Ho, Wo)
         ctx.cell = state
@@ -890,7 +948,7 @@
         need = ctx.needs_input_grad
         grads = [None] * (4 + len(params))
         gs0, gs1, gw = _cell_bwd(state, gO, sinks, lambda n: 4 + spec.index[n], None, True, None, True, need[1],
-                                 need[2])
+                                 need[2], None, need[3])
         grads[1], grads[2] = gs0, gs1
         if need[3]:
             grads[3] = gw
@@ -900,7 +958,7 @@
 
 def cell_forward(spec: CellSpec, s0, s1, wts, params: Sequence[torch.Tensor], bn_of, training: bool,
                  momentum: float = 0.1, eps: float = 1e-5):
-    return _Cell.apply((spec, bn_of, training, momentum, eps), s0, s1, wts, *params)
+    return _Cell.apply((spec, bn_of, training, momentum, eps, torch.is_grad_enabled()), s0, s1, wts, *params)
 
 
 def relu_conv_bn(x, w, rm, rv, training, momentum=0.1, eps=1e-5):
@@ -1124,7 +1182,7 @@
 
     @staticmethod
     def forward(ctx, meta, x, y, an, ar, *params):
-        spec, bn_of, training, momentum, eps = meta
+        spec, bn_of, training, momentum, eps, grad = meta
         P = dict(zip(spec.names, params))
         dev = x.device
         mats, outs = [an], [torch.empty_like(an)]
@@ -1147,7 +1205,8 @@
         cells = []
         i0 = i1 = 0
         for cspec, red in zip(spec.cells, spec.reduce):
-            O, st = _cell_fwd(cspec, tensors[i0], tensors[i1], wr if red else wn, P, bn_of, training, momentum, eps)
+            O, st = _cell_fwd(cspec, tensors[i0], tensors[i1], wr if red else wn, P, bn_of, training, momentum, eps,
+                              grad)
             tensors.append(O)
             cells.append((st, i0, i1, len(tensors) - 1, red))
             i0, i1 = i1, len(tensors) - 1
@@ -1179,21 +1238,35 @@
 
         def key(n):
             return 5 + spec.index[n]
-        g, first = {last: torch.empty_like(tensors[last])}, {last: False}
+        alpha = {False: bool(need[3]), True: ar is not None and bool(need[4])}
+        if NEEDED_GRADS:
+            stem_need, plans = network_needed_grads(spec, lambda n: P[n].requires_grad, alpha[False], alpha[True])
+            needT = [stem_need] + [any(c[2:]) for c in plans]
+        else:
+            needT = [True] * len(tensors)
+        g, first = {}, {}
+        if needT[last]:
+            g[last], first[last] = torch.empty_like(tensors[last]), False
         hw, hb = spec.head
         gw, sw = sinks.get(P[hw], key(hw)) if need[key(hw)] else (None, 0)
         gb, sb = sinks.get(P[hb], key(hb)) if need[key(hb)] else (None, 0)
-        _K.head_bwd(tensors[last], dl, pooled, P[hw], gloss.reshape(()).contiguous().float(), g[last], gw, sw, gb, sb)
+        if needT[last] or gw is not None or gb is not None:
+            _K.head_bwd(tensors[last], dl, pooled, P[hw], gloss.reshape(()).contiguous().float(), g.get(last), gw, sw,
+                        gb, sb)
         rows = []
         for st, i0, i1, io, red in reversed(cells):
+            if not needT[io]:
+                continue
             for i in (i0, i1):
-                if i not in g:
+                if needT[i] and i not in g:
                     g[i], first[i] = torch.empty_like(tensors[i]), True
-            f0 = first[i0]
-            f1 = first[i1] and i1 != i0
+            f0 = first.get(i0, False)
+            f1 = first.get(i1, False) and i1 != i0
             cell_rows = []
-            _cell_bwd(st, g[io], sinks, key, g[i0], f0, g[i1], f1, True, True, cell_rows)
-            first[i0] = first[i1] = False
+            _cell_bwd(st, g[io], sinks, key, g.get(i0), f0, g.get(i1), f1, needT[i0], needT[i1], cell_rows, alpha[red])
+            for i in (i0, i1):
+                if needT[i]:
+                    first[i] = False
             rows += [(r, red) for r in cell_rows]
         dst = {}
         for red, leaf, idx in ((False, an, 3), (True, ar, 4)):
@@ -1207,8 +1280,8 @@
         if ents:
             _alpha_grad(ents)
         conv, gamma, beta, _ = spec.stem
-        if training and st_stem is not None and 0 in g:
-            flags = (False, need[key(conv)], need[key(gamma)], need[key(beta)])
+        flags = (False, need[key(conv)], need[key(gamma)], need[key(beta)])
+        if training and st_stem is not None and 0 in g and (any(flags) or not NEEDED_GRADS):
             _stem_bwd(st_stem, g[0], sinks, (key(conv), key(gamma), key(beta)), flags)
         sinks.finish(grads)
         return tuple(grads)
@@ -1217,7 +1290,7 @@
 _MERGE_CAP = {"dwpw_fwd": 16, "pw_fwd": 32, "pool_fwd": 16, "combine_bwd_reduce": 8, "pw_bwd": 32, "dw_bwd": 40,
               "pool_bwd": 16, "dw_bwd_multi": 40, "dwpw_fwd_multi": 40, "pool_fwd_multi": 16,
               "pool_bwd_multi": 16, "fold_f64": 128, "alpha_grad": 128, "__sync_fold__": 64}
-_QUERIES = {"selffold_ready", "max_blocks", "stamps_compiled", "REP", "ZBF16", "OPTIM_MAX_PARTS"}
+_QUERIES = {"selffold_ready", "max_blocks", "stamps_compiled", "REP", "ZBF16", "OPTIM_MAX_PARTS", "dwpw_split_path"}
 
 
 class _Recorder:
@@ -1311,4 +1384,4 @@
 
 def network_loss(spec: NetSpec, x, y, params: Sequence[torch.Tensor], an, ar, bn_of, training: bool,
                  momentum: float = 0.1, eps: float = 1e-5):
-    return _Network.apply((spec, bn_of, training, momentum, eps), x, y, an, ar, *params)
+    return _Network.apply((spec, bn_of, training, momentum, eps, torch.is_grad_enabled()), x, y, an, ar, *params)
```

Result: faster. 2.016 s, median of 6 (-5.6%).
